# sinamalakouti/CDDMSL

Measured on AMD Instinct MI355X. Metric: images/sec (train step) VOC+Clipart RN50-C4, higher is better.
Workload: dtype bf16

## Files before the change

### cddmsl_amd/csrc/conv_fwd256.hip

```cpp
#include "gemm_common.h"
#include <type_traits>

namespace {

__device__ __forceinline__ unsigned pack4_e4m3(float a, float b, float c, float d) {
  a = __builtin_amdgcn_fmed3f(a, -448.f, 448.f); b = __builtin_amdgcn_fmed3f(b, -448.f, 448.f);
  c = __builtin_amdgcn_fmed3f(c, -448.f, 448.f); d = __builtin_amdgcn_fmed3f(d, -448.f, 448.f);
  int w = __builtin_amdgcn_cvt_pk_fp8_f32(a, b, 0, false);
  w = __builtin_amdgcn_cvt_pk_fp8_f32(c, d, w, true);
  return (unsigned)w;
}

struct fp8e4 { unsigned char v; };
template <> struct Mma<fp8e4> {
  static constexpr int ES = 2;
  __device__ static __forceinline__ void step2(f32x16& acc, const u32x4& a0, const u32x4& a1, const u32x4& b0, const u32x4& b1) {
    const i32x8 a = {(int)a0[0], (int)a0[1], (int)a0[2], (int)a0[3], (int)a1[0], (int)a1[1], (int)a1[2], (int)a1[3]};
    const i32x8 b = {(int)b0[0], (int)b0[1], (int)b0[2], (int)b0[3], (int)b1[0], (int)b1[1], (int)b1[2], (int)b1[3]};
    acc = __builtin_amdgcn_mfma_scale_f32_32x32x64_f8f6f4(a, b, acc, 0, 0, 0, 0x7f7f7f7f, 0, 0x7f7f7f7f);
  }
};
template <typename T> struct MmaQuad {
  __device__ static __forceinline__ void run(f32x16& c0, f32x16& c1, const u32x4 (*fa)[4], const u32x4* fb) {
#pragma unroll
// ... 172 lines not shown
        const u32x2 o8 = {pack4_e4m3(v[0] * q8s, v[1] * q8s, v[2] * q8s, v[3] * q8s), pack4_e4m3(v[4] * q8s, v[5] * q8s, v[6] * q8s, v[7] * q8s)};
        __builtin_amdgcn_raw_buffer_store_b64(o8, ry8, vy8, (unsigned)((a * 32 + 8 * i) * p.ldy), CDDMSL_STORE_AUX);
        asm volatile("s_nop 4" ::: "memory");
        asm volatile("" :: "v"(o8));
      }
      if (f32out) {
        const u32x4 o0 = {__builtin_bit_cast(unsigned, v[0]), __builtin_bit_cast(unsigned, v[1]), __builtin_bit_cast(unsigned, v[2]), __builtin_bit_cast(unsigned, v[3])};
        const u32x4 o1 = {__builtin_bit_cast(unsigned, v[4]), __builtin_bit_cast(unsigned, v[5]), __builtin_bit_cast(unsigned, v[6]), __builtin_bit_cast(unsigned, v[7])};
        __builtin_amdgcn_raw_buffer_store_b128(o0, ry, vy, so, CDDMSL_STORE_AUX);
        __builtin_amdgcn_raw_buffer_store_b128(o1, ry, vy, so + 16, CDDMSL_STORE_AUX);
        asm volatile("s_nop 4" ::: "memory");
        asm volatile("" :: "v"(o0), "v"(o1));
      } else {
        const u32x4 o = {pack2bf(v[0], v[1]), pack2bf(v[2], v[3]), pack2bf(v[4], v[5]), pack2bf(v[6], v[7])};
        if (p.nt_out) __builtin_amdgcn_raw_buffer_store_b128(o, ry, vy, so, CDDMSL_STORE_AUX);
        else __builtin_amdgcn_raw_buffer_store_b128(o, ry, vy, so, 0);
        asm volatile("s_nop 4" ::: "memory");
        asm volatile("" :: "v"(o));
      }
    }
    if (DEPTH == 2 && a + 2 < 4 && !rf32) fetch(a + 2, rresb[a % DEPTH], rmskb[a % DEPTH]);
  };
  put(std::integral_constant<int, 0>{});
  pass(std::integral_constant<int, 0>{});
  pass(std::integral_constant<int, 1>{});
  pass(std::integral_constant<int, 2>{});
  pass(std::integral_constant<int, 3>{});
  if (emit8 && p.amax8) {
    am8 = wave_max_u(am8);
    if (lane == 0) atomicMax(p.amax8 + (blockIdx.x & 63), am8);
  }
}

template <typename T, bool TAPS, bool RPOOL = false, int EPI = -1, bool PERSIST = false, bool SPLITK = false>
__global__ __launch_bounds__(512) void k_conv_fwd256(ConvArgs p) {
  __shared__ __attribute__((aligned(16))) u32x4 lds[2 * 2 * 2 * 128 * KCH];
  const int t_in = threadIdx.x;
  p.x += (long)blockIdx.y * p.bx; p.w += (long)blockIdx.y * p.bw; p.y += (long)blockIdx.y * p.by;
  const int ntn = p.Cout >> 8;
  const int ntiles = PERSIST ? (p.tile_limit ? p.tile_limit : ntn * ((p.M + 255) >> 8)) : 0;
  int lbid = PERSIST ? (int)((blockIdx.x & 7) * (gridDim.x >> 3) + (blockIdx.x >> 3))
           : SPLITK ? p.tile0 + (int)(blockIdx.x / (unsigned)p.ksplits) : xcd_remap(blockIdx.x, gridDim.x);
  const int kt0 = SPLITK ? (int)(blockIdx.x % (unsigned)p.ksplits) * p.kper : 0;
  if (PERSIST && lbid >= ntiles) return;
  for (;;) {
  int t = t_in;
  if (PERSIST) asm volatile("" : "+v"(t));
  const int lane = t & 63;
#ifdef CDDMSL_TILE_STAMPS
  const unsigned long long ts_entry = __builtin_amdgcn_s_memrealtime();
#endif
  const int wvu = __builtin_amdgcn_readfirstlane(t >> 6);
  const int wr = wvu >> 2, wc = wvu & 3;
  const int tile_n = lbid % ntn, tile_m = lbid / ntn;
  const int m0 = tile_m * 256, n0 = tile_n * 256;
  const int cl = (t & 7) ^ ((t >> 4) & 7);
  const int nkt = SPLITK ? min(p.kper, (p.Kc >> 3) - kt0) : (p.Kc >> 3);
  const int tpt = p.cpp >> 3;

  auto rowoff = [&](int m, int& iy0, int& ix0) {
    const unsigned tq = fdiv((unsigned)m, p.dWo), ox = m - tq * p.Wo;
    const unsigned img = fdiv(tq, p.dHo), oy = tq - img * p.Ho;
    iy0 = (int)oy * p.stride - p.pad; ix0 = (int)ox * p.stride - p.pad;
    return (((long)img * p.Hi + iy0) * p.Wi + ix0) * p.xrs * 16;
  };
  int iyb, ixb;
  const long base_a = rowoff(m0, iyb, ixb);
  const __amdgpu_buffer_rsrc_t ra_rsrc = __builtin_amdgcn_make_buffer_rsrc((void*)(p.x + base_a), 0, 0x7fffffff, 0x00020000);
  const __amdgpu_buffer_rsrc_t rb_rsrc = __builtin_amdgcn_make_buffer_rsrc((void*)(p.w + (long)n0 * p.wrs * 16), 0, 0x7fffffff, 0x00020000);
  unsigned va[2][2], vinv[2][2], vb[2][2];
  int iy0[2][2], ix0[2][2];
#pragma unroll
  for (int h = 0; h < 2; ++h)
#pragma unroll
    for (int i = 0; i < 2; ++i) {
      const int m = m0 + i * 128 + h * 64 + (t >> 3);
      const bool vm = m < p.M;
      const long ro = rowoff(vm ? m : m0, iy0[h][i], ix0[h][i]);
      va[h][i] = (unsigned)(ro - base_a) + cl * 16;
      if (!vm) { iy0[h][i] = -(1 << 20); if (!TAPS) va[h][i] |= 0x80000000u; }
      vinv[h][i] = 0;
      vb[h][i] = (unsigned)(((2 * i + (t >> 8)) * 64 + h * 32 + ((t >> 3) & 31)) * p.wrs + cl) * 16;
    }
  if (TAPS) {
    unsigned xm[2][2] = {{0, 0}, {0, 0}};
    for (int kx = 0; kx < p.KW; ++kx)
#pragma unroll
      for (int h = 0; h < 2; ++h)
#pragma unroll
        for (int i = 0; i < 2; ++i) xm[h][i] |= ((unsigned)(ix0[h][i] + kx) >= (unsigned)p.Wi ? 1u : 0u) << kx;
    const unsigned full = (1u << p.KW) - 1u;
    for (int ky = 0; ky < p.KH; ++ky)
#pragma unroll
      for (int h = 0; h < 2; ++h)
#pragma unroll
        for (int i = 0; i < 2; ++i) vinv[h][i] |= ((unsigned)(iy0[h][i] + ky) >= (unsigned)p.Hi ? full : xm[h][i]) << (ky * p.KW);
  }
  const int step_col = (p.xrs - (p.cpp - KCH)) * 16;
  const int step_row = ((p.Wi - (p.KW - 1)) * p.xrs - (p.cpp - KCH)) * 16;
  int left[2] = {tpt, tpt}, tap[2] = {0, 0}, kxs[2] = {0, 0};
  unsigned soa[2] = {0, 0}, sob[2] = {0, 0};
  if (SPLITK) {
    const int tap0 = TAPS ? kt0 / tpt : 0, within = TAPS ? kt0 - tap0 * tpt : kt0;
    const int ky0 = TAPS ? tap0 / p.KW : 0, kx0 = tap0 - ky0 * p.KW;
#pragma unroll
    for (int h = 0; h < 2; ++h) {
      left[h] = tpt - (TAPS ? within : 0); tap[h] = tap0; kxs[h] = kx0;
      soa[h] = (unsigned)((ky0 * p.Wi + kx0) * p.xrs * 16 + within * KCH * 16);
      sob[h] = (unsigned)(kt0 * KCH * 16);
    }
  }

  char* const L = (char*)lds;
  auto stageA = [&](auto H, int buf) {
    constexpr int h = decltype(H)::value;
    char* dst = L + (buf << 16) + (h << 14) + wvu * 1024;
#pragma unroll
    for (int i = 0; i < 2; ++i) {
      unsigned v = va[h][i];
      if (TAPS) v |= __builtin_amdgcn_ubfe(vinv[h][i], (unsigned)tap[h], 1u) << 31;
      blds16(ra_rsrc, v, soa[h], dst + i * 8192);
    }
    if (TAPS) {
      int step = KCH * 16;
      if (--left[h] == 0) {
        left[h] = tpt; ++tap[h];
        if (++kxs[h] == p.KW) { kxs[h] = 0; step = step_row; } else step = step_col;
      }
      soa[h] += step;
    } else soa[h] += KCH * 16;
  };
  auto stageB = [&](auto J, int buf) {
    constexpr int j = decltype(J)::value;
    char* dst = L + (buf << 16) + (1 << 15) + (j << 14) + wvu * 1024;
#pragma unroll
    for (int i = 0; i < 2; ++i) blds16(rb_rsrc, vb[j][i], sob[j], dst + i * 8192);
    sob[j] += KCH * 16;
  };
  using I0 = std::integral_constant<int, 0>;
  using I1 = std::integral_constant<int, 1>;

  f32x16 acc[4][2];
#pragma unroll
  for (int a = 0; a < 4; ++a)
#pragma unroll
    for (int b = 0; b < 2; ++b)
#pragma unroll
      for (int r = 0; r < 16; ++r) acc[a][b][r] = 0.f;

  const int r32 = lane & 31, hh = lane >> 5, sw = (r32 >> 1) & 7;
  unsigned ada[4], adb[4];
#pragma unroll
  for (int ks = 0; ks < 4; ++ks) {
    ada[ks] = (unsigned)(((wr * 64 + r32) * KCH + ((2 * ks + hh) ^ sw)) * 16);
    adb[ks] = (unsigned)(((wc * 32 + r32) * KCH + ((2 * ks + hh) ^ sw)) * 16 + (1 << 15));
  }
  u32x4 fa0[2][4], fa1[2][4], fb0[4], fb1[4];
  auto readA = [&](auto I, u32x4 (*fa)[4]) {
    constexpr int i = decltype(I)::value;
#pragma unroll
    for (int rt = 0; rt < 2; ++rt)
#pragma unroll
      for (int ks = 0; ks < 4; ++ks) fa[rt][ks] = *(const u32x4*)(L + ada[ks] + ((i << 14) + rt * 32 * KCH * 16));
  };
  auto readB = [&](auto J, u32x4* fb) {
    constexpr int j = decltype(J)::value;
#pragma unroll
    for (int ks = 0; ks < 4; ++ks) fb[ks] = *(const u32x4*)(L + adb[ks] + (j << 14));
  };
  auto flipA = [&]() {
// ... 313 lines not shown
    case 2: launch(std::integral_constant<int, 2>()); break;
    default: launch(std::integral_constant<int, 3>()); break;
  }
}

template <typename T, bool TAPS> void launch_fwd2(const ConvArgs& a, dim3 grid, hipStream_t st) {
  const int epi = epi_of(a);
  if constexpr (sizeof(T) == 2) {
    if (epi >= 0) {
      with_epi(epi, [&](auto e) { hipLaunchKernelGGL((k_conv_fwd2<T, TAPS, decltype(e)::value>), grid, dim3(256), 0, st, a); });
      return;
    }
  }
  hipLaunchKernelGGL((k_conv_fwd2<T, TAPS, -1>), grid, dim3(256), 0, st, a);
}

struct TailSplit { int rem, splits, kper; };
constexpr int TAIL_FRAC_DEFAULT = 8;
static TailSplit plan_tail_split(int tiles, int ncu, int nktot, long ws_bytes) {
  const int rem = ncu > 0 ? tiles % ncu : 0;
  long frac = env_int("CDDMSL_TAIL_FRAC", TAIL_FRAC_DEFAULT);
  if (frac <= 0) frac = 8;
  if (env_int("CDDMSL_TAIL_SPLIT", 1) == 0 || tiles <= ncu || rem <= 0 || rem * frac > ncu || nktot < 16) return {};
  long S = ncu / rem;
  if (S > nktot / 2) S = nktot / 2;
  const long maxs = env_int("CDDMSL_TAIL_MAXS", S);
  if (S > maxs) S = maxs;
  const int kper = (int)((nktot + S - 1) / S);
  S = (nktot + kper - 1) / kper;
  if (S < 2 || rem * S * 65536 * 4 > ws_bytes) return {};
  return {rem, (int)S, kper};
}

template <typename T, bool TAPS> void launch256_main(const ConvArgs& a, dim3 grid, hipStream_t st, int epi) {
  if constexpr (std::is_same<T, __bf16>::value && !TAPS) {
    const int nb = persistent_blocks();
    if (nb > 0 && grid.y == 1 && (int)grid.x > nb && (a.Kc >> 3) <= env_int("CDDMSL_PERSIST_MAXKT", 8)) {
      with_epi(epi, [&](auto e) { hipLaunchKernelGGL((k_conv_fwd256<T, false, false, decltype(e)::value, true>), dim3(nb), dim3(512), 0, st, a); });
      return;
    }
  }
  with_epi(epi, [&](auto e) { hipLaunchKernelGGL((k_conv_fwd256<T, TAPS, false, decltype(e)::value>), grid, dim3(512), 0, st, a); });
}

template <typename T, bool TAPS> void launch256(const ConvArgs& a, dim3 grid, hipStream_t st, void* ws, long ws_bytes) {
  const int epi = epi_of(a);
  if (sizeof(T) == 4 || epi < 0) { hipLaunchKernelGGL((k_conv_fwd256<T, TAPS, false, -1>), grid, dim3(512), 0, st, a); return; }
  if constexpr (sizeof(T) != 4) {
    if constexpr (std::is_same<T, __bf16>::value) {
      const int tiles = (int)grid.x;
      const TailSplit ts = grid.y == 1 ? plan_tail_split(tiles, persistent_blocks_raw(), a.Kc >> 3, ws ? ws_bytes : 0) : TailSplit{};
      if (ts.splits) {
        ConvArgs m = a, t = a;
        m.tile_limit = tiles - ts.rem;
        launch256_main<T, TAPS>(m, dim3((unsigned)(tiles - ts.rem), 1), st, epi);
        t.partial = (float*)ws; t.tile0 = tiles - ts.rem; t.ksplits = ts.splits; t.kper = ts.kper;
        hipLaunchKernelGGL((k_conv_fwd256<T, TAPS, false, -1, false, true>), dim3((unsigned)(ts.rem * ts.splits)), dim3(512), 0, st, t);
        hipLaunchKernelGGL(k_conv_split_reduce, dim3((unsigned)(ts.rem * 64)), dim3(256), 0, st, t);
        return;
      }
    }
    launch256_main<T, TAPS>(a, grid, st, epi);
  }
}

template <typename T> void launch_tile256(const ConvArgs& a, const Plan& p, hipStream_t st, void* ws, long ws_bytes) {
  const dim3 grid(p.gx, p.gy);
  const bool taps = !(a.KH == 1 && a.KW == 1 && a.pad == 0);
  if constexpr (std::is_same<T, fp8e4>::value) {
    if (taps) launch256<T, true>(a, grid, st, ws, ws_bytes);
    else launch256<T, false>(a, grid, st, ws, ws_bytes);
  } else if (p.kernel == 11) {
    if (taps) launch_fwd2<T, true>(a, grid, st);
    else launch_fwd2<T, false>(a, grid, st);
  } else {
    if (a.res_pool) hipLaunchKernelGGL((k_conv_fwd256<T, false, true>), grid, dim3(512), 0, st, a);
    else if (taps) launch256<T, true>(a, grid, st, ws, ws_bytes);
    else launch256<T, false>(a, grid, st, ws, ws_bytes);
  }
}

}

void launch_fwd_tile256(const ConvArgs& a, const Plan& p, Operand op, hipStream_t st, void* ws, long ws_bytes) {
  if (op == OP_BF16) launch_tile256<__bf16>(a, p, st, ws, ws_bytes);
  else if (op == OP_F32) launch_tile256<float>(a, p, st, ws, ws_bytes);
  else launch_tile256<fp8e4>(a, p, st, ws, ws_bytes);
}
```

### cddmsl_amd/csrc/conv_wgrad.hip

```cpp
#include "gemm_common.h"

namespace {

template <typename T> struct TrFrag;
template <> struct TrFrag<__bf16> {
  __device__ static __forceinline__ u32x4 read(const u32x4* base, int mrow0, int col0, int lane) {
    int g = lane >> 4, li = lane & 15, q = li >> 2, pp = li & 3;
    int hh = g >> 1;
    int col = col0 + 16 * (g & 1) + 4 * pp;
    const char* b = (const char*)base;
    const char* a0 = b + (long)(mrow0 + 8 * hh + q) * (WROW * 16) + col * 2;
    const char* a1 = a0 + 4 * (WROW * 16);
    i16x4 v0 = __builtin_amdgcn_ds_read_tr16_b64_v4i16((__attribute__((address_space(3))) i16x4*)a0);
    i16x4 v1 = __builtin_amdgcn_ds_read_tr16_b64_v4i16((__attribute__((address_space(3))) i16x4*)a1);
    u32x2 p0 = __builtin_bit_cast(u32x2, v0), p1 = __builtin_bit_cast(u32x2, v1);
    u32x4 r = {p0[0], p0[1], p1[0], p1[1]};
    return r;
  }
  static constexpr int MSTEP = 16;
};
template <> struct TrFrag<float> {
  __device__ static __forceinline__ u32x4 read(const u32x4* base, int mrow0, int col0, int lane) {
    int r = lane & 31, hh = lane >> 5;
    const char* b = (const char*)base;
// ... 170 lines not shown
  __shared__ __attribute__((aligned(16))) u32x4 lds[2][2][WM * 16];
  const int t = threadIdx.x, lane = t & 63, wv = t >> 6;
  p.x += (long)blockIdx.y * p.bx; p.dy += (long)blockIdx.y * p.bd;
  char* outp = (char*)p.dw + (long)blockIdx.y * p.bo;
  const int wvu = __builtin_amdgcn_readfirstlane(t >> 6);
  const int ntn = (p.Cout + COLS - 1) / COLS, ntk = (p.K + COLS - 1) / COLS;
  int bid = xcd_remap(blockIdx.x, gridDim.x);
  const int tile_k = bid % ntk; bid /= ntk;
  const int tile_n = bid % ntn; bid /= ntn;
  const int split = bid;
  const int n0 = tile_n * COLS, k0 = tile_k * COLS;
  const int mt0 = split * p.mtiles_per_split;
  const int total_mt = (p.M + WM - 1) / WM;
  const int mt1 = min(mt0 + p.mtiles_per_split, total_mt);

  const int cc = t & 15, rb = t >> 4;
  const int cl = cc ^ fsw(rb);
  const int kc = k0 * ES / 16 + cl;
  const bool vk = kc < p.Kc;
  const int pp = vk ? kc / p.cpp : 0, coff = vk ? kc - pp * p.cpp : 0;
  const int ky = pp / p.KW, kx = pp - ky * p.KW;
  const int nc = n0 * ES / 16 + cl;
  const bool vn = nc < p.ncc;
  const bool taps = !(p.KH == 1 && p.KW == 1);
  const char* zp = (const char*)g_zero_page;

  int m[4];
  const char* pd[4];
  const char* px[4];
#pragma unroll
  for (int i = 0; i < 4; ++i) {
    m[i] = mt0 * WM + rb + 16 * i;
    pd[i] = p.dy + ((long)m[i] * p.ldd) * ES + (long)nc * 16;
    px[i] = p.x + (((long)m[i] + (long)(ky - p.pad) * p.Wi + (kx - p.pad)) * p.xrs) * 16 + (long)coff * 16;
  }
  const long dstep = (long)WM * p.ldd * ES, xstep = (long)WM * p.xrs * 16;

  auto stage = [&](int buf) {
#pragma unroll
    for (int i = 0; i < 4; ++i) {
      bool vmm = m[i] < p.M;
      glds16((vmm && vn) ? pd[i] : zp, &lds[buf][0][(4 * wvu + 16 * i) * 16]);
    }
#pragma unroll
    for (int i = 0; i < 4; ++i) {
      bool ok = (m[i] < p.M) & vk;
      if (taps) {
        unsigned mm = min((unsigned)m[i], (unsigned)(p.M - 1));
        unsigned tq = fdiv(mm, p.dWo);
        unsigned ox = mm - tq * p.Wo;
        unsigned oy = tq - fdiv(tq, p.dHo) * p.Ho;
        ok = ok & ((unsigned)((int)oy - p.pad + ky) < (unsigned)p.Hi) & ((unsigned)((int)ox - p.pad + kx) < (unsigned)p.Wi);
      }
      glds16(ok ? px[i] : zp, &lds[buf][1][(4 * wvu + 16 * i) * 16]);
    }
#pragma unroll
    for (int i = 0; i < 4; ++i) { m[i] += WM; pd[i] += dstep; px[i] += xstep; }
  };

  constexpr int WT = COLS / 2;
  constexpr int NT = WT / 32;
  const int wn = wv >> 1, wk = wv & 1;
  f32x16 acc[NT][NT];
#pragma unroll
  for (int a = 0; a < NT; ++a)
#pragma unroll
    for (int b = 0; b < NT; ++b)
#pragma unroll
      for (int r = 0; r < 16; ++r) acc[a][b][r] = 0.f;

  typename TrFragS<T>::Off offa[NT], offb[NT];
#pragma unroll
  for (int i = 0; i < NT; ++i) {
    offa[i] = TrFragS<T>::prep(wn * WT + i * 32, lane);
    offb[i] = TrFragS<T>::prep(wk * WT + i * 32, lane);
  }

  if (mt0 < mt1) stage(0);
  for (int mt = mt0; mt < mt1; ++mt) {
    const int cur = (mt - mt0) & 1;
    if (mt + 1 < mt1) {
      stage(cur ^ 1);
      asm volatile("s_waitcnt vmcnt(8)" ::: "memory");
    } else {
      asm volatile("s_waitcnt vmcnt(0)" ::: "memory");
// ... 315 lines not shown
#pragma unroll
    for (int a = 0; a < NTN; ++a)
#pragma unroll
      for (int g = 0; g < 16; ++g) {
        if (a * 4 + (g >> 2) < NG) {
          const int n = a * 32 + (g & 3) + 8 * (g >> 2) + 4 * h;
          const float v = acc[a][g];
          const long o = (long)n * p.ldo + k;
          if (MODE == 0) atomicAdd((float*)outp + o, v);
          else if (MODE == 1) ((float*)outp)[o] = v;
          else Mma<__bf16>::store(outp + o * 2, v);
        }
        acc[a][g] = 0.f;
      }
  };
  {
    int it = 0;
    for (; it + 2 < nit; ++it) item(it, std::integral_constant<int, 2>{});
    if (it + 1 < nit) { item(it, std::integral_constant<int, 1>{}); ++it; }
    if (it < nit) item(it, std::integral_constant<int, 0>{});
  }
  if (MODE == 3 && p.gpos) {
    const int k = k0 + wvu * 32 + r;
#pragma unroll
    for (int a = 0; a < NTN; ++a)
#pragma unroll
      for (int g = 0; g < 16; ++g) {
        const int n = a * 32 + (g & 3) + 8 * (g >> 2) + 4 * h;
        if (a * 4 + (g >> 2) < NG && n <= P) atomicAdd(p.gpos + (long)n * p.K + k, gacc[a][g]);
      }
  }
}

__global__ __launch_bounds__(512) void k_wgrad256(WgradArgs p) {
  __shared__ __attribute__((aligned(16))) u32x4 lds[2 * 2 * 2 * 64 * 16];
  const int t = threadIdx.x, lane = t & 63;
#ifdef CDDMSL_TILE_STAMPS
  const unsigned long long ts_entry = __builtin_amdgcn_s_memrealtime();
  unsigned long long ts_loop = ts_entry;
#endif
  p.x += (long)blockIdx.y * p.bx; p.dy += (long)blockIdx.y * p.bd;
  char* outp = (char*)p.dw + (long)blockIdx.y * p.bo;
  const int wvu = __builtin_amdgcn_readfirstlane(t >> 6);
  const int wn = wvu >> 2, wk = wvu & 3;
  const int ntn = p.Cout >> 8, ntk = p.K >> 8;
  int bid = xcd_remap(blockIdx.x, gridDim.x);
  const int tile_k = bid % ntk; bid /= ntk;
  const int tile_n = bid % ntn; bid /= ntn;
  const int n0 = tile_n * 256, k0 = tile_k * 256;
  const int mt0 = bid * p.mtiles_per_split;
  const int nmt = min(p.mtiles_per_split, (p.M + WM - 1) / WM - mt0);
  const bool taps = !(p.KH == 1 && p.KW == 1);

  const int rb = t >> 4, cl = (t & 15) ^ fsw(rb);
  const int gd = (cl >> 3) * 16 + (cl & 7);
  const int gx = (cl >> 2) * 8 + (cl & 3);
  const int kc = (k0 >> 3) + gx;
  const int pp = kc / p.cpp, coff = kc - pp * p.cpp;
  const int ky = pp / p.KW, kx = pp - ky * p.KW;
  unsigned vd[2], vx[2];
#pragma unroll
  for (int i = 0; i < 2; ++i) {
    vd[i] = (unsigned)((i * 32 + rb) * p.ldd * 2 + gd * 16);
    vx[i] = (unsigned)((((i * 32 + rb) + ky * p.Wi + kx) * p.xrs + coff) * 16);
  }
  const __amdgpu_buffer_rsrc_t rd = __builtin_amdgcn_make_buffer_rsrc((void*)(p.dy + ((long)mt0 * WM * p.ldd + n0) * 2), 0, 0x80000000u, 0x00020000);
  const __amdgpu_buffer_rsrc_t rx = __builtin_amdgcn_make_buffer_rsrc((void*)(p.x + ((long)mt0 * WM - p.pad * p.Wi - p.pad) * p.xrs * 16), 0, 0x80000000u, 0x00020000);
  const unsigned dstep = (unsigned)(WM * p.ldd * 2), xstep = (unsigned)(WM * p.xrs * 16);
  const int mrow = mt0 * WM + rb;

  char* const L = (char*)lds;
  auto stageD = [&](auto H, int buf, int T) {
    constexpr int h = decltype(H)::value;
    char* dst = L + (buf << 16) + (h << 14) + wvu * 1024;
#pragma unroll
    for (int i = 0; i < 2; ++i) {
      const unsigned inv = (mrow + T * WM + i * 32 < p.M) ? 0u : 0x80000000u;
      __builtin_amdgcn_raw_ptr_buffer_load_lds(rd, (__attribute__((address_space(3))) void*)(dst + i * 8192 - h * 128), 16,
                                               (int)(vd[i] | inv), (int)(T * dstep), h * 128, 0);
    }
  };
  unsigned xinv[2];
  auto validX = [&](int T) {
#pragma unroll
    for (int i = 0; i < 2; ++i) {
      const int m = mrow + T * WM + i * 32;
      bool ok = m < p.M;
      if (taps) {
        const unsigned mm = min((unsigned)m, (unsigned)(p.M - 1));
        const unsigned tq = fdiv(mm, p.dWo);
        const unsigned ox = mm - tq * p.Wo;
        const unsigned oy = tq - fdiv(tq, p.dHo) * p.Ho;
        ok = ok & ((unsigned)((int)oy - p.pad + ky) < (unsigned)p.Hi) & ((unsigned)((int)ox - p.pad + kx) < (unsigned)p.Wi);
      }
      xinv[i] = ok ? 0u : 0x80000000u;
    }
  };
  auto stageX = [&](auto J, int buf, int T) {
    constexpr int j = decltype(J)::value;
    char* dst = L + (buf << 16) + (1 << 15) + (j << 14) + wvu * 1024;
#pragma unroll
    for (int i = 0; i < 2; ++i)
      __builtin_amdgcn_raw_ptr_buffer_load_lds(rx, (__attribute__((address_space(3))) void*)(dst + i * 8192 - j * 64), 16,
                                               (int)(vx[i] | xinv[i]), (int)(T * xstep), j * 64, 0);
  };
  using I0 = std::integral_constant<int, 0>;
  using I1 = std::integral_constant<int, 1>;

  f32x16 acc[4][2];
#pragma unroll
  for (int a = 0; a < 4; ++a)
#pragma unroll
    for (int b = 0; b < 2; ++b)
#pragma unroll
      for (int r = 0; r < 16; ++r) acc[a][b][r] = 0.f;

  const unsigned lbase = (unsigned)(size_t)(__attribute__((address_space(3))) char*)L;
  unsigned adA[2][2], adB[2];
  {
#pragma unroll
    for (int a = 0; a < 2; ++a) {
      const TrFragS<__bf16>::Off o = TrFragS<__bf16>::prep(wn * 64 + a * 32, lane);
      adA[a][0] = lbase + o.o0; adA[a][1] = lbase + o.o1;
    }
    const TrFragS<__bf16>::Off o = TrFragS<__bf16>::prep(wk * 32, lane);
    adB[0] = lbase + (1u << 15) + o.o0; adB[1] = lbase + (1u << 15) + o.o1;
  }
  u32x4 fa0[2][4], fa1[2][4], fb0[4], fb1[4];
#define CDDMSL_TR2(DST, A0, A1, IMM)                                                             \
// ... 5 lines not shown
  _Pragma("unroll") for (int a = 0; a < 2; ++a) {                                                \
    CDDMSL_TR2(FA[a][0], adA[a][0], adA[a][1], ((HALF) << 14) + 0 * 4096)                        \
    CDDMSL_TR2(FA[a][1], adA[a][0], adA[a][1], ((HALF) << 14) + 1 * 4096)                        \
    CDDMSL_TR2(FA[a][2], adA[a][0], adA[a][1], ((HALF) << 14) + 2 * 4096)                        \
    CDDMSL_TR2(FA[a][3], adA[a][0], adA[a][1], ((HALF) << 14) + 3 * 4096) }
#define CDDMSL_READ_B(HALF, FB)                                                                  \
  CDDMSL_TR2(FB[0], adB[0], adB[1], ((HALF) << 14) + 0 * 4096)                                   \
  CDDMSL_TR2(FB[1], adB[0], adB[1], ((HALF) << 14) + 1 * 4096)                                   \
  CDDMSL_TR2(FB[2], adB[0], adB[1], ((HALF) << 14) + 2 * 4096)                                   \
  CDDMSL_TR2(FB[3], adB[0], adB[1], ((HALF) << 14) + 3 * 4096)
#define CDDMSL_FLIP_A() { adA[0][0] ^= 1u << 16; adA[0][1] ^= 1u << 16; adA[1][0] ^= 1u << 16; adA[1][1] ^= 1u << 16; }
#define CDDMSL_FLIP_B() { adB[0] ^= 1u << 16; adB[1] ^= 1u << 16; }
#define CDDMSL_MMA_QUAD(I, J, FA, FB)                                               \
  _Pragma("unroll") for (int ms = 0; ms < 4; ++ms) {                                \
    Mma<__bf16>::step(acc[2 * (I)][J], FA[0][ms], FB[ms]);                          \
    Mma<__bf16>::step(acc[2 * (I) + 1][J], FA[1][ms], FB[ms]);                      \
  }
#define CDDMSL_WAIT4(F) asm volatile("s_waitcnt lgkmcnt(0)" : "+v"(F[0]), "+v"(F[1]), "+v"(F[2]), "+v"(F[3]) :: "memory");
#define CDDMSL_WAIT8(F) asm volatile("s_waitcnt lgkmcnt(0)" : "+v"(F[0][0]), "+v"(F[0][1]), "+v"(F[0][2]), "+v"(F[0][3]), \
                                     "+v"(F[1][0]), "+v"(F[1][1]), "+v"(F[1][2]), "+v"(F[1][3]) :: "memory");
#define CDDMSL_PHASE_SYNC_IN(WAIT)                                                  \
  __builtin_amdgcn_sched_barrier(0);                                                \
  __builtin_amdgcn_s_barrier();                                                     \
  WAIT                                                                              \
  __builtin_amdgcn_sched_barrier(0);                                                \
  __builtin_amdgcn_s_setprio(1);
#define CDDMSL_PHASE_SYNC_OUT(I, J)                                                 \
  asm volatile("" : "+v"(acc[2 * (I)][J]), "+v"(acc[2 * (I) + 1][J]));              \
  __builtin_amdgcn_s_setprio(0);                                                    \
  __builtin_amdgcn_sched_barrier(0);                                                \
  __builtin_amdgcn_s_barrier();                                                     \
  __builtin_amdgcn_sched_barrier(0);

  if (nmt > 0) {
    validX(0);
    stageD(I0{}, 0, 0); stageD(I1{}, 0, 0); stageX(I0{}, 0, 0); stageX(I1{}, 0, 0);
    if (nmt > 1) {
      validX(1);
      stageD(I0{}, 1, 1); stageX(I0{}, 1, 1); stageX(I1{}, 1, 1);
      asm volatile("s_waitcnt vmcnt(6)" ::: "memory");
    } else {
      asm volatile("s_waitcnt vmcnt(0)" ::: "memory");
    }
    __builtin_amdgcn_s_barrier();
    __builtin_amdgcn_sched_barrier(0);
    CDDMSL_READ_A(0, fa0)
    CDDMSL_WAIT8(fa0)
    if (wn == 1) __builtin_amdgcn_s_barrier();
    __builtin_amdgcn_sched_barrier(0);
#ifdef CDDMSL_TILE_STAMPS
    ts_loop = __builtin_amdgcn_s_memrealtime();
#endif

    for (int kt = 0; kt < nmt; ++kt) {
      const int d = kt & 1;
      const bool more1 = kt + 1 < nmt, more2 = kt + 2 < nmt;
      CDDMSL_READ_B(0, fb0)
      if (more1) stageD(I1{}, d ^ 1, kt + 1);
      CDDMSL_PHASE_SYNC_IN(CDDMSL_WAIT4(fb0))
      CDDMSL_MMA_QUAD(0, 0, fa0, fb0);
      CDDMSL_PHASE_SYNC_OUT(0, 0)
      CDDMSL_READ_B(1, fb1)
      CDDMSL_FLIP_B()
      if (more2) { stageD(I0{}, d, kt + 2); validX(kt + 2); }
      CDDMSL_PHASE_SYNC_IN(CDDMSL_WAIT4(fb1))
      CDDMSL_MMA_QUAD(0, 1, fa0, fb1);
      CDDMSL_PHASE_SYNC_OUT(0, 1)
      CDDMSL_READ_A(1, fa1)
      CDDMSL_FLIP_A()
      if (more2) {
        stageX(I0{}, d, kt + 2);
        asm volatile("s_waitcnt vmcnt(4)" ::: "memory");
      } else {
        asm volatile("s_waitcnt vmcnt(0)" ::: "memory");
      }
      CDDMSL_PHASE_SYNC_IN(CDDMSL_WAIT8(fa1))
      CDDMSL_MMA_QUAD(1, 1, fa1, fb1);
      CDDMSL_PHASE_SYNC_OUT(1, 1)
      if (more1) { CDDMSL_READ_A(0, fa0) }
      if (more2) stageX(I1{}, d, kt + 2);
      CDDMSL_PHASE_SYNC_IN(CDDMSL_WAIT8(fa0))
      CDDMSL_MMA_QUAD(1, 0, fa1, fb0);
      CDDMSL_PHASE_SYNC_OUT(1, 0)
    }
    if (wn == 0) __builtin_amdgcn_s_barrier();
  }
#undef CDDMSL_TR2
#undef CDDMSL_WAIT4
#undef CDDMSL_WAIT8
#undef CDDMSL_READ_A
#undef CDDMSL_READ_B
#undef CDDMSL_FLIP_A
#undef CDDMSL_FLIP_B
#undef CDDMSL_MMA_QUAD
#undef CDDMSL_PHASE_SYNC_IN
#undef CDDMSL_PHASE_SYNC_OUT

#ifdef CDDMSL_TILE_STAMPS
  const unsigned long long ts_epi = __builtin_amdgcn_s_memrealtime();
#endif
  const int r = lane & 31, h = lane >> 5;
  if (p.ws) {
    store_frags((f32x4*)p.ws + ((long)(bid * ntn + tile_n) * ntk + tile_k) * (8 * 32 * 64) + (wvu * 32) * 64 + lane, acc);
  } else
#pragma unroll
  for (int a = 0; a < 4; ++a)
#pragma unroll
    for (int b = 0; b < 2; ++b) {
      const int k = k0 + wk * 64 + b * 32 + r;
#pragma unroll
      for (int g = 0; g < 16; ++g) {
        const int n = n0 + wn * 128 + a * 32 + (g & 3) + 8 * (g >> 2) + 4 * h;
        const float v = acc[a][b][g] * (p.scale ? p.scale[n] : 1.f);
// ... 201 lines not shown
  }
  for (; s < splits; ++s) sum += src[s * ntiles * SLOTS];
  const int wv = q / (FR * 64), j = (q / 64) % FR, lane = q & 63, r = lane & 31, h = lane >> 5, g4 = j & 3;
  int a, b, wn, wk;
  if (WAVES == 8) { a = j >> 3; b = (j >> 2) & 1; wn = wv >> 2; wk = wv & 3; }
  else { a = j >> 3; b = (j >> 2) & 1; wn = wv >> 1; wk = wv & 1; }
  const int n = tile_n * TN + wn * (WAVES == 8 ? 128 : 64) + a * 32 + 8 * g4 + 4 * h;
  const int k = tile_k * TN + wk * 64 + b * 32 + r;
  if (k >= K) return;
#pragma unroll
  for (int e = 0; e < 4; ++e)
    if (n + e < Cout) dw[(long)(n + e) * ldo + k] += sum[e] * (scale ? scale[n + e] : 1.f);
}

static bool use_workspace(long blocks, long tile_floats, void* ws, long ws_bytes) {
  if (env_int("CDDMSL_WGRAD_WS", 1) == 0) return false;
  return ws != nullptr && blocks * tile_floats * 4 <= ws_bytes;
}

template <int WAVES, int FR>
static void launch_wgrad_split(void (*kernel)(WgradArgs), WgradArgs& a, const Plan& p, hipStream_t st, void* wsp, long ws_bytes) {
  constexpr int TN = WAVES == 8 ? 256 : 128, SLOTS = WAVES * FR * 64;
  const int ntn = (a.Cout + TN - 1) / TN, ntk = (a.K + TN - 1) / TN;
  const bool ws = p.splits > 1 && use_workspace((long)p.gx, SLOTS * 4, wsp, ws_bytes);
  if (ws) a.ws = (float*)wsp;
  hipLaunchKernelGGL(kernel, dim3(p.gx), dim3(WAVES * 64), 0, st, a);
  if (ws) hipLaunchKernelGGL((k_wgrad_reduce<WAVES, FR>), dim3((unsigned)(ntn * ntk * (SLOTS / 256))), dim3(256), 0, st, (const f32x4*)wsp, a.dw, a.scale,
                             ntn, ntk, p.splits, a.Cout, a.K, a.ldo);
}

void launch_wgrad(WgradArgs& a, const Plan& p, Operand op, hipStream_t st, void* ws, long ws_bytes) {
  switch (p.kernel) {
    case 12: launch_wgrad_split<8, 32>(k_wgrad256_f8, a, p, st, ws, ws_bytes); break;
    case 6: launch_wgrad_split<8, 32>(k_wgrad256, a, p, st, ws, ws_bytes); break;
    case 5:
      if (op == OP_BF16) launch_wgrad_split<4, 16>(k_conv_wgrad_dma<__bf16>, a, p, st, ws, ws_bytes);
      else hipLaunchKernelGGL(k_conv_wgrad_dma<float>, dim3(p.gx), dim3(256), 0, st, a);
      break;
    default:
      if (op == OP_BF16) hipLaunchKernelGGL(k_conv_wgrad<__bf16>, dim3(p.gx), dim3(256), 0, st, a);
      else hipLaunchKernelGGL(k_conv_wgrad<float>, dim3(p.gx), dim3(256), 0, st, a);
  }
}

void launch_gemm_tn(const WgradArgs& p, Operand op, const Plan& pl, int batch, int mode, hipStream_t st) {
  const dim3 grid(pl.gx, pl.gy);
  if (pl.kernel == 9) {
#define CDDMSL_TNS(NG)                                                                                              \
  case NG:                                                                                                          \
    if (mode == 0) hipLaunchKernelGGL((k_gemm_tn_small<NG, 0>), grid, dim3(256), 0, st, p, batch, pl.bpb);      \
    else if (mode == 1) hipLaunchKernelGGL((k_gemm_tn_small<NG, 1>), grid, dim3(256), 0, st, p, batch, pl.bpb); \
    else hipLaunchKernelGGL((k_gemm_tn_small<NG, 2>), grid, dim3(256), 0, st, p, batch, pl.bpb);                \
    break;
    switch (p.Cout / 8) { CDDMSL_TNS(1) CDDMSL_TNS(2) CDDMSL_TNS(3) CDDMSL_TNS(4) CDDMSL_TNS(5) CDDMSL_TNS(6) CDDMSL_TNS(7) CDDMSL_TNS(8) }
#undef CDDMSL_TNS
  } else if (pl.kernel == 7) {
    if (op == OP_BF16) hipLaunchKernelGGL(k_gemm_tn_stream<__bf16>, grid, dim3(256), 0, st, p, batch, pl.bpb);
    else hipLaunchKernelGGL(k_gemm_tn_stream<float>, grid, dim3(256), 0, st, p, batch, pl.bpb);
  } else {
    if (op == OP_BF16) hipLaunchKernelGGL(k_conv_wgrad_dma<__bf16>, grid, dim3(256), 0, st, p);
    else hipLaunchKernelGGL(k_conv_wgrad_dma<float>, grid, dim3(256), 0, st, p);
  }
}

void launch_attnpool_dx(const WgradArgs& p, unsigned gx, unsigned gy, int nbatch, int bpb, hipStream_t st) {
  hipLaunchKernelGGL((k_gemm_tn_small<7, 3, 49>), dim3(gx, gy), dim3(256), 0, st, p, nbatch, bpb);
}
// ... 1 lines not shown
```

### cddmsl_amd/csrc/elementwise.hip

```cpp
#include "common.h"
#include <stdlib.h>

namespace {

template <typename T> struct Elt;
template <> struct Elt<__bf16> {
  static constexpr int ES = 2, VEC = 8;
  __device__ static __forceinline__ void unpack(const u32x4& v, float* f) {
#pragma unroll
    for (int j = 0; j < 4; ++j) { f[2 * j] = bf2f(v[j] & 0xffff); f[2 * j + 1] = bf2f(v[j] >> 16); }
  }
  __device__ static __forceinline__ u32x4 pack(const float* f) {
    u32x4 v;
#pragma unroll
    for (int j = 0; j < 4; ++j) v[j] = pack2bf(f[2 * j], f[2 * j + 1]);
    return v;
  }
  __device__ static __forceinline__ float ld(const char* p) { return bf2f(*(const unsigned short*)p); }
  __device__ static __forceinline__ void st(char* p, float v) { *(unsigned short*)p = f2bf(v); }
};
template <> struct Elt<float> {
  static constexpr int ES = 4, VEC = 4;
  __device__ static __forceinline__ void unpack(const u32x4& v, float* f) {
    const f32x4 x = __builtin_bit_cast(f32x4, v);
// ... 110 lines not shown
    float a0[8], a1[8], a2[8], a3[8], o[8];
    Elt<T>::unpack(b[0], a0); Elt<T>::unpack(b[cch], a1);
    Elt<T>::unpack(b[(long)W * cch], a2); Elt<T>::unpack(b[(long)W * cch + cch], a3);
#pragma unroll
    for (int j = 0; j < Elt<T>::VEC; ++j) o[j] = ((a0[j] + a1[j]) + (a2[j] + a3[j])) * 0.25f;
    ((u32x4*)y)[i] = Elt<T>::pack(o);
  }
}

template <typename T>
__global__ void k_avgpool2_bwd(const char* dy, const char* mask, const char* add, char* dx, int N, int H, int W, int cch) {
  int Ho = H / 2, Wo = W / 2;
  long total = (long)N * H * W * cch;
  for (long i = (long)blockIdx.x * blockDim.x + threadIdx.x; i < total; i += (long)gridDim.x * blockDim.x) {
    int c = i % cch; long q = i / cch;
    int xx = q % W; q /= W;
    int yy = q % H; int n = q / H;
    float g[8], m[8], a[8], o[8];
    bool in = (yy >> 1) < Ho && (xx >> 1) < Wo;
    if (in) Elt<T>::unpack(((const u32x4*)dy)[(((long)n * Ho + (yy >> 1)) * Wo + (xx >> 1)) * cch + c], g);
    if (mask) Elt<T>::unpack(((const u32x4*)mask)[i], m);
    if (add) Elt<T>::unpack(((const u32x4*)add)[i], a);
#pragma unroll
    for (int j = 0; j < Elt<T>::VEC; ++j) {
      float v = in ? g[j] * 0.25f : 0.f;
      if (add) v += a[j];
      if (mask && !(m[j] > 0.f)) v = 0.f;
      o[j] = v;
    }
    ((u32x4*)dx)[i] = Elt<T>::pack(o);
  }
}

__global__ __launch_bounds__(256) void k_avgpool2_bwd_q8(const char* dy, const char* mask, const char* add, char* dx, int N, int H, int W, int cch,
                                                         char* y8, const float* q8, unsigned* amax8) {
  using T = __bf16;
  const int Ho = H / 2, Wo = W / 2;
  const long total = (long)N * H * W * cch;
  const float s = q8[0];
  unsigned mx = 0u;
  for (long i = (long)blockIdx.x * blockDim.x + threadIdx.x; i < total; i += (long)gridDim.x * blockDim.x) {
    int c = i % cch; long q = i / cch;
    int xx = q % W; q /= W;
    int yy = q % H; int n = q / H;
    float g[8], m[8], a[8], o[8];
    bool in = (yy >> 1) < Ho && (xx >> 1) < Wo;
    if (in) Elt<T>::unpack(((const u32x4*)dy)[(((long)n * Ho + (yy >> 1)) * Wo + (xx >> 1)) * cch + c], g);
    if (mask) Elt<T>::unpack(((const u32x4*)mask)[i], m);
    if (add) Elt<T>::unpack(((const u32x4*)add)[i], a);
#pragma unroll
    for (int j = 0; j < 8; ++j) {
      float v = in ? g[j] * 0.25f : 0.f;
      if (add) v += a[j];
      if (mask && !(m[j] > 0.f)) v = 0.f;
      o[j] = v;
      mx = absmax_bits(mx, v);
    }
    ((u32x4*)dx)[i] = Elt<T>::pack(o);
    const u32x2 o8 = {e4m3x4(o[0] * s, o[1] * s, o[2] * s, o[3] * s), e4m3x4(o[4] * s, o[5] * s, o[6] * s, o[7] * s)};
    ((u32x2*)y8)[i] = o8;
  }
  __shared__ unsigned sm[4];
  mx = wave_max_u(mx);
  if ((threadIdx.x & 63) == 0) sm[threadIdx.x >> 6] = mx;
  __syncthreads();
  if (threadIdx.x == 0) {
// ... 416 lines not shown
  hipStream_t st = (hipStream_t)stream;
  for (int n0 = 0; n0 < N; n0 += PRE_MAX) {
    const int c = N - n0 < PRE_MAX ? N - n0 : PRE_MAX;
    PreBatch b;
    for (int j = 0; j < PRE_MAX; ++j) { const int q = j < c ? j : 0; b.img[j] = imgs[n0 + q]; b.h[j] = hs[n0 + q]; b.w[j] = ws[n0 + q]; }
    DISPATCH(dtype, k_preprocess224_batch, <<<dim3((unsigned)((S * S + 255) / 256), (unsigned)c), dim3(256), 0, st>>>(
        b, (char*)out, n0, Hp, Wp, RH, RW, top, left, S, Cp, mean3[0], mean3[1], mean3[2], std3[0], std3[1], std3[2]));
  }
  return launch_status();
}

extern "C" int cddmsl_avgpool2_fwd(const void* x, void* y, int N, int H, int W, int C, int dtype, void* stream) {
  int es = dtype == 0 ? 2 : 4;
  if ((C * es) % 16 || H < 2 || W < 2) return CDDMSL_ERR_ARG;
  int cch = C * es / 16;
  long total = (long)N * (H / 2) * (W / 2) * cch;
  if (total == 0) return CDDMSL_OK;
  DISPATCH(dtype, k_avgpool2_fwd, <<<dim3(gsz(total)), dim3(256), 0, (hipStream_t)stream>>>((const char*)x, (char*)y, N, H, W, cch));
  return launch_status();
}

extern "C" int cddmsl_avgpool2_bwd(const void* dy, const void* mask, const void* add, void* dx, int N, int H, int W,
                                   int C, int dtype, void* stream) {
  int es = dtype == 0 ? 2 : 4;
  if ((C * es) % 16 || H < 2 || W < 2) return CDDMSL_ERR_ARG;
  int cch = C * es / 16;
  long total = (long)N * H * W * cch;
  if (total == 0) return CDDMSL_OK;
  DISPATCH(dtype, k_avgpool2_bwd, <<<dim3(gsz(total)), dim3(256), 0, (hipStream_t)stream>>>(
      (const char*)dy, (const char*)mask, (const char*)add, (char*)dx, N, H, W, cch));
  return launch_status();
}

extern "C" int cddmsl_avgpool2_bwd_q8(const void* dy, const void* mask, const void* add, void* dx, int N, int H, int W, int C, void* y8,
                                      const float* q8, float* amax8, void* stream) {
  if ((C * 2) % 16 || !y8 || !q8 || !amax8) return CDDMSL_ERR_ARG;
  const int cch = C * 2 / 16;
  const long total = (long)N * H * W * cch;
  if (total == 0) return CDDMSL_OK;
  hipLaunchKernelGGL(k_avgpool2_bwd_q8, dim3(gsz(total, 256, 8192)), dim3(256), 0, (hipStream_t)stream, (const char*)dy, (const char*)mask, (const char*)add,
                     (char*)dx, N, H, W, cch, (char*)y8, q8, (unsigned*)amax8);
  return launch_status();
}

extern "C" int cddmsl_maxpool3s2_fwd(const void* x, void* y, int N, int H, int W, int C, int dtype, void* stream) {
  int es = dtype == 0 ? 2 : 4;
  if ((C * es) % 16 || H < 1 || W < 1) return CDDMSL_ERR_ARG;
  int cch = C * es / 16, Ho = (H - 1) / 2 + 1, Wo = (W - 1) / 2 + 1;
  long total = (long)N * Ho * Wo * cch;
  if (total == 0) return CDDMSL_OK;
  DISPATCH(dtype, k_maxpool3s2, <<<dim3(gsz(total)), dim3(256), 0, (hipStream_t)stream>>>((const char*)x, (char*)y, N, H, W, Ho, Wo, cch));
  return launch_status();
}
extern "C" int cddmsl_upsample_zero2(const void* t, const void* mask, const void* add, void* dx, int N, int H, int W, int C,
                                     int dtype, void* stream) {
  int es = dtype == 0 ? 2 : 4;
  if ((C * es) % 16 || H < 1 || W < 1) return CDDMSL_ERR_ARG;
  int cch = C * es / 16, Ho = (H - 1) / 2 + 1, Wo = (W - 1) / 2 + 1;
  long total = (long)N * H * W * cch;
  if (total == 0) return CDDMSL_OK;
  DISPATCH(dtype, k_upsample_zero2, <<<dim3(gsz(total)), dim3(256), 0, (hipStream_t)stream>>>(
      (const char*)t, (const char*)mask, (const char*)add, (char*)dx, N, H, W, Ho, Wo, cch));
  return launch_status();
}
extern "C" int cddmsl_meanpool_fwd(const void* x, float* y, long K, int P, int C, int dtype, void* stream) {
  if (K < 0 || P <= 0 || C <= 0) return CDDMSL_ERR_ARG;
// ... 122 lines not shown
```

### cddmsl_amd/csrc/gemm_common.h

```cpp
#pragma once
#include "common.h"
#include <cstdlib>

namespace {

constexpr int BM = 128, BN = 128, KCH = 8;

struct FastDiv {
  unsigned mul, shr, d;
};
static inline FastDiv make_fastdiv(unsigned d) {
  FastDiv f;
  f.d = d;
  unsigned s = 0;
  while ((1ull << s) < d) ++s;
  f.shr = s;
  f.mul = (unsigned)(((1ull << 32) * ((1ull << s) - d)) / d + 1);
  return f;
}
__device__ __forceinline__ unsigned fdiv(unsigned n, const FastDiv& f) { return (__umulhi(n, f.mul) + n) >> f.shr; }

template <typename T> __device__ __forceinline__ float affine(float v, float sc, float bi) {
  return sizeof(T) <= 2 ? __builtin_fmaf(v, sc, bi) : v * sc + bi;
}

#ifndef CDDMSL_STORE_AUX
#define CDDMSL_STORE_AUX 2
#endif
#ifndef CDDMSL_LOAD_AUX
#define CDDMSL_LOAD_AUX 0
#endif

struct ConvArgs {
  const char* x;
  const char* w;
  char* y;
  const float* scale;
  const float* bias;
  const char* residual;
  const char* relu_mask;
  int Nimg, Hi, Wi, Cin, Ho, Wo, Cout, KH, KW, stride, pad;
  int ldy, ldr, ldm;
  int relu, out_f32, pool;
  int res_f32;
  int res_pool;
  int M, Kc, cpp;
  FastDiv dWo, dHo, dcpp, dKW;
  int xrs, wrs;
  long bx, bw, by;
  char* y8 = nullptr;
  const float* q8 = nullptr;
  unsigned* amax8 = nullptr;
  float* partial = nullptr;
  int tile0 = 0, ksplits = 1, kper = 0, tile_limit = 0;
  int nt_out = 1;
#ifdef CDDMSL_TILE_STAMPS
  unsigned long long* tstamps = nullptr;
#endif
};

template <typename T> struct Mma;
template <> struct Mma<__bf16> {
  static constexpr int ES = 2;
  __device__ static __forceinline__ void step(f32x16& acc, const u32x4& a, const u32x4& b) {
    acc = __builtin_amdgcn_mfma_f32_32x32x16_bf16(__builtin_bit_cast(bf16x8, a), __builtin_bit_cast(bf16x8, b), acc, 0, 0, 0);
  }
  __device__ static __forceinline__ float load(const char* p) { return bf2f(*(const unsigned short*)p); }
  __device__ static __forceinline__ void store(char* p, float v) { *(unsigned short*)p = f2bf(v); }
};
template <> struct Mma<float> {
  static constexpr int ES = 4;
  __device__ static __forceinline__ void step(f32x16& acc, const u32x4& a, const u32x4& b) {
    const f32x4 fa = __builtin_bit_cast(f32x4, a), fb = __builtin_bit_cast(f32x4, b);
    acc = __builtin_amdgcn_mfma_f32_32x32x2f32(fa[0], fb[0], acc, 0, 0, 0);
    acc = __builtin_amdgcn_mfma_f32_32x32x2f32(fa[1], fb[1], acc, 0, 0, 0);
    acc = __builtin_amdgcn_mfma_f32_32x32x2f32(fa[2], fb[2], acc, 0, 0, 0);
    acc = __builtin_amdgcn_mfma_f32_32x32x2f32(fa[3], fb[3], acc, 0, 0, 0);
  }
  __device__ static __forceinline__ float load(const char* p) { return *(const float*)p; }
  __device__ static __forceinline__ void store(char* p, float v) { *(float*)p = v; }
};
typedef __attribute__((ext_vector_type(8))) int i32x8;

__device__ __forceinline__ int xcd_remap(int bid, int nblk) {
  const int q = nblk >> 3, rem = nblk & 7, x = bid & 7, j = bid >> 3;
  return (x < rem ? x * (q + 1) : rem * (q + 1) + (x - rem) * q) + j;
}

// ... 8 lines not shown
  u32x4 r;
#pragma unroll
  for (int j = 0; j < 4; ++j) {
    float lo = (bf2f(a[j] & 0xffff) + bf2f(b[j] & 0xffff)) + (bf2f(c[j] & 0xffff) + bf2f(d[j] & 0xffff));
    float hi = (bf2f(a[j] >> 16) + bf2f(b[j] >> 16)) + (bf2f(c[j] >> 16) + bf2f(d[j] >> 16));
    r[j] = pack2bf(lo * 0.25f, hi * 0.25f);
  }
  return r;
}

__device__ __attribute__((aligned(16))) unsigned int g_zero_page[4] = {0u, 0u, 0u, 0u};

__device__ __forceinline__ void glds16(const void* g, void* l) {
  __builtin_amdgcn_global_load_lds((const __attribute__((address_space(1))) void*)g,
                                   (__attribute__((address_space(3))) void*)l, 16, 0, 0);
}

struct WgradArgs {
  const char* x;
  const char* dy;
  float* dw;
  const float* scale;
  int Nimg, Hi, Wi, Cin, Ho, Wo, Cout, KH, KW, stride, pad, ldd, pool;
  int M, Kc, cpp, K, ncc;
  int mtiles_per_split;
  FastDiv dWo, dHo;
  int xrs;
  int ldo;
  int direct;
  long bx, bd, bo;
  const float* g0 = nullptr;
  const unsigned long long* mbits = nullptr;
  float* gpos = nullptr;
  float* ws = nullptr;
#ifdef CDDMSL_TILE_STAMPS
  unsigned long long* tstamps = nullptr;
#endif
};

constexpr int WM = 64;
constexpr int WROW = 16 + 4;

__device__ __forceinline__ int fsw(int row) { return ((row & 3) << 2) | ((row >> 2) & 3); }

__device__ __forceinline__ void store_frags(f32x4* dst, const f32x16 (&acc)[4][2]) {
#pragma unroll
  for (int a = 0; a < 4; ++a)
#pragma unroll
    for (int b = 0; b < 2; ++b)
#pragma unroll
      for (int g4 = 0; g4 < 4; ++g4) {
        const f32x4 v = {acc[a][b][4 * g4], acc[a][b][4 * g4 + 1], acc[a][b][4 * g4 + 2], acc[a][b][4 * g4 + 3]};
        dst[((a * 2 + b) * 4 + g4) * 64] = v;
      }
}

static long env_int(const char* name, long dflt, bool* set = nullptr) {
  const char* e = getenv(name);
  if (set) *set = e != nullptr;
  return e ? atol(e) : dflt;
}

enum Operand { OP_BF16 = 0, OP_F32 = 1, OP_FP8 = 2 };
static int elem_size(Operand op) { return op == OP_BF16 ? 2 : op == OP_F32 ? 4 : 1; }

struct Plan {
// ... 28 lines not shown
```

### cddmsl_amd/csrc/gemm_conv.hip

```cpp
#include "gemm_common.h"

namespace {

template <typename T>
__device__ __forceinline__ void weight_prep_body(const float* w, const float* scale, char* wf, char* wd, int Cout, int KH, int KW, int Cin,
                                                 long first, long stride) {
  __shared__ float tile[32][33];
  const int taps = KH * KW, nit = (Cin + 31) / 32, nct = (Cout + 31) / 32;
  const long ntiles = (long)nct * taps * nit;
  const int tx = threadIdx.x & 31, ty = threadIdx.x >> 5;
  constexpr int ES = Mma<T>::ES;
  for (long tl = first; tl < ntiles; tl += stride) {
    const int it = (int)(tl % nit); const long q = tl / nit;
    const int tap = (int)(q % taps), ct = (int)(q / taps);
    const int ky = tap / KW, kx = tap % KW;
    __syncthreads();
#pragma unroll
    for (int r = 0; r < 4; ++r) {
      const int co = ct * 32 + ty + 8 * r, ci = it * 32 + tx;
      float v = 0.f;
      if (co < Cout && ci < Cin) {
        const long i = ((long)co * taps + tap) * Cin + ci;
        v = w[i];
        if (wf) Mma<T>::store(wf + i * ES, v);
// ... 161 lines not shown
extern "C" int cddmsl_conv_fwd(const void* x, const void* w, void* y, const float* scale, const float* bias,
                               const void* residual, const void* relu_mask, int Nimg, int Hi, int Wi, int Cin,
                               int Cout, int KH, int KW, int stride, int pad, int pool, int ldy, int ldr, int ldm,
                               int relu, int out_f32, int dtype, void* stream) {
  if (dtype != 0 && dtype != 1) return CDDMSL_ERR_ARG;
  return conv_fwd_any((Operand)dtype, x, w, y, scale, bias, residual, relu_mask, Nimg, Hi, Wi, Cin, Cout, KH, KW, stride, pad, pool, ldy, ldr, ldm,
                      relu, out_f32, nullptr, nullptr, nullptr, stream);
}

extern "C" int cddmsl_conv_fwd_q8(const void* x, const void* w, void* y, const float* scale, const float* bias,
                                  const void* residual, const void* relu_mask, int Nimg, int Hi, int Wi, int Cin,
                                  int Cout, int KH, int KW, int stride, int pad, int relu, void* y8, const float* q8, float* amax8,
                                  void* stream) {
  if (!y8) return CDDMSL_ERR_ARG;
  return conv_fwd_any(OP_BF16, x, w, y, scale, bias, residual, relu_mask, Nimg, Hi, Wi, Cin, Cout, KH, KW, stride, pad, 0, Cout, Cout, Cout,
                      relu, 0, y8, q8, amax8, stream);
}

extern "C" int cddmsl_conv_fwd_fp8(const void* x, const void* w, void* y, const float* scale, const float* bias,
                                   const void* residual, const void* relu_mask, int Nimg, int Hi, int Wi, int Cin, int Cout, int KH,
                                   int KW, int pad, int relu, int out_f32, void* y8, const float* q8, float* amax8, void* stream) {
  if (Cin % 128 != 0 || (out_f32 & ~1)) return CDDMSL_ERR_ARG;
  return conv_fwd_any(OP_FP8, x, w, y, scale, bias, residual, relu_mask, Nimg, Hi, Wi, Cin, Cout, KH, KW, 1, pad, 0, Cout, Cout, Cout,
                      relu, out_f32, y8, q8, amax8, stream);
}

static bool wgrad256_ok(const WgradArgs& a, int batch) {
  const long mode = env_int("CDDMSL_GEMM256", 1);
  if (mode == 0) return false;
  if ((a.Cout & 255) || (a.K & 255) || (a.cpp & 7) || (a.ldd & 7)) return false;
  if (mode == 2) return true;
  return (long)(a.Cout / 256) * (a.K / 256) * batch * ((a.M + WM - 1) / WM) >= env_int("CDDMSL_WGRAD256_MIN", 4000);
}
static bool wgrad256_span_ok(int mtiles_per_split, int Wi, long row_bytes) {
  return ((long)mtiles_per_split * WM + WM + 2L * Wi + 2) * row_bytes + (1L << 20) < (1L << 31);
}

static int even_split(int total_mt, long* splits) {
  const int mps = (int)((total_mt + *splits - 1) / *splits);
  *splits = (total_mt + mps - 1) / mps;
  return mps;
}

static long split_512_rounds(long tiles, int total_mt, bool taps) {
  bool forced;
  const long target = env_int("CDDMSL_WGRAD_BLOCKS", taps ? 1024 : 512, &forced);
  const long maxs = (total_mt + 7) / 8;
  long splits = 1;
  const long r0 = (target + 511) / 512;
  double best = -1.0;
  for (long r = r0; r <= r0 + 1; ++r) {
    long c = (512 * r) / tiles;
    if (c < 1) c = 1;
    if (c > maxs) c = maxs;
    long real = c;
    even_split(total_mt, &real);
    const long blocks = tiles * real, rounds = (blocks + 511) / 512;
    const double eff = (double)blocks / (512.0 * rounds);
    if (eff > best + 0.03) { best = eff; splits = c; }
    if (c == maxs) break;
  }
  if (forced) { splits = (target + tiles - 1) / tiles; if (splits > maxs) splits = maxs; }
  return splits < 1 ? 1 : splits;
}

static long split_256_rounds(long tiles, int total_mt) {
  const long maxs = (total_mt + 15) / 16;
  long sp = 1;
  double best = -1.0;
  for (int r = 1; r <= 6; ++r) {
    long c = (256L * r) / tiles;
    if (c < 1) continue;
    if (c > maxs) c = maxs;
    const long blocks = tiles * c, rounds = (blocks + 255) / 256;
    const double eff = (double)blocks / (256.0 * rounds);
    if (eff > best + 0.02) { best = eff; sp = c; }
    if (c == maxs) break;
  }
  return sp;
}

static Plan plan_wgrad(const WgradArgs& a, Operand op, int batch) {
  const int es = elem_size(op), total_mt = (a.M + WM - 1) / WM;
  const long tiles256 = (long)(a.Cout / 256) * (a.K / 256);
  const long row_bytes = (long)a.ldd * es > a.xrs * 16L ? (long)a.ldd * es : a.xrs * 16L;
  if (op == OP_FP8) {
    long sp = split_256_rounds(tiles256, total_mt);
    const int mps = even_split(total_mt, &sp);
    if (!wgrad256_span_ok(mps, a.Wi, row_bytes)) return {};
    return {12, (unsigned)(tiles256 * sp), 1, (int)sp, mps};
  }
  const int cols = 256 / es;
  const long tiles = (long)((a.Cout + cols - 1) / cols) * ((a.K + cols - 1) / cols);
  long splits = split_512_rounds(tiles, total_mt, !(a.KH == 1 && a.KW == 1));
  const int mps = even_split(total_mt, &splits);
  if (tiles * splits > 0x7fffffffL) return {};
  const bool same = !a.pool && a.stride == 1 && a.Ho == a.Hi && a.Wo == a.Wi;
  if (same && op == OP_BF16 && wgrad256_ok(a, batch)) {
    bool forced;
    const long want = env_int("CDDMSL_WGRAD256_BLOCKS", 0, &forced);
    const long maxs = (total_mt + 15) / 16;
    long sp = forced ? (want + tiles256 - 1) / tiles256 : split_256_rounds(tiles256, total_mt);
    if (sp > maxs) sp = maxs;
    if (sp < 1) sp = 1;
    const int mps256 = even_split(total_mt, &sp);
    if (wgrad256_span_ok(mps256, a.Wi, row_bytes)) return {6, (unsigned)(tiles256 * sp), 1, (int)sp, mps256};
  }
  return {same ? 5 : 4, (unsigned)(tiles * splits), 1, (int)splits, mps};
}

extern "C" int cddmsl_set_workspace(void* ptr, long bytes) {
  if (bytes < 0 || (ptr == nullptr && bytes != 0) || ((size_t)ptr & 15)) return CDDMSL_ERR_ARG;
  g_ws = ptr; g_ws_bytes = bytes;
  return CDDMSL_OK;
}

static int run_wgrad(WgradArgs& a, Operand op, const Plan& p, void* stream) {
  if (p.kernel == 0) return CDDMSL_ERR_ARG;
  g_last_kernel = p.kernel;
  if (g_plan_only) return CDDMSL_OK;
  a.mtiles_per_split = p.mtiles_per_split;
  launch_wgrad(a, p, op, (hipStream_t)stream, g_ws, g_ws_bytes);
  return launch_status();
}

static int fill_wgrad(WgradArgs& a, Operand op, const void* x, const void* dy, float* dw, const float* scale, int Nimg, int Hi,
                      int Wi, int Cin, int Cout, int KH, int KW, int stride, int pad, int pool, int ldd) {
  const int es = elem_size(op);
  if (Nimg < 0 || Hi <= 0 || Wi <= 0 || Cin <= 0 || Cout <= 0 || KH <= 0 || KW <= 0 || stride <= 0) return CDDMSL_ERR_ARG;
  if ((Cin * es) % 16 != 0 || (Cout * es) % 16 != 0 || (ldd * es) % 16 != 0) return CDDMSL_ERR_ARG;
  if (pool && (KH != 1 || KW != 1 || pad != 0 || stride != 1)) return CDDMSL_ERR_ARG;
  a.x = (const char*)x; a.dy = (const char*)dy; a.dw = dw; a.scale = scale;
  a.Nimg = Nimg; a.Hi = Hi; a.Wi = Wi; a.Cin = Cin; a.Cout = Cout; a.KH = KH; a.KW = KW; a.stride = stride; a.pad = pad;
  a.ldd = ldd; a.pool = pool;
  if (pool) { a.Ho = Hi / 2; a.Wo = Wi / 2; }
  else { a.Ho = (Hi + 2 * pad - KH) / stride + 1; a.Wo = (Wi + 2 * pad - KW) / stride + 1; }
  if (a.Ho <= 0 || a.Wo <= 0) return CDDMSL_ERR_ARG;
  long M = (long)Nimg * a.Ho * a.Wo;
  if (M > 0x7fffff00L) return CDDMSL_ERR_ARG;
  a.M = (int)M; a.cpp = Cin * es / 16; a.Kc = KH * KW * a.cpp; a.K = KH * KW * Cin; a.ncc = Cout * es / 16;
  a.mtiles_per_split = 0;
  a.dWo = make_fastdiv((unsigned)a.Wo); a.dHo = make_fastdiv((unsigned)a.Ho);
  a.xrs = a.cpp; a.ldo = a.K; a.direct = 0; a.bx = a.bd = a.bo = 0;
#ifdef CDDMSL_TILE_STAMPS
  a.tstamps = g_tile_stamps;
#endif
  return CDDMSL_OK;
}

extern "C" int cddmsl_conv_wgrad(const void* x, const void* dy, float* dw, const float* scale, int Nimg, int Hi,
                                 int Wi, int Cin, int Cout, int KH, int KW, int stride, int pad, int pool, int ldd,
                                 int dtype, void* stream) {
  if (dtype != 0 && dtype != 1) return CDDMSL_ERR_ARG;
  WgradArgs a;
  const int st = fill_wgrad(a, (Operand)dtype, x, dy, dw, scale, Nimg, Hi, Wi, Cin, Cout, KH, KW, stride, pad, pool, ldd);
  if (st != CDDMSL_OK || a.M == 0) return st;
  return run_wgrad(a, (Operand)dtype, plan_wgrad(a, (Operand)dtype, 1), stream);
}

extern "C" int cddmsl_conv_wgrad_fp8_ok(int Cin, int Cout, int KH, int KW, int pad, int ldd) {
  return (Cin % 256 == 0 && Cout % 256 == 0 && KH == KW && (KH & 1) && 2 * pad == KH - 1 && ldd % 16 == 0) ? 1 : 0;
}
extern "C" int cddmsl_conv_wgrad_fp8(const void* x8, const void* dy8, float* dw, const float* scale, int Nimg, int Hi, int Wi, int Cin,
                                     int Cout, int KH, int KW, int pad, int ldd, void* stream) {
  if (!cddmsl_conv_wgrad_fp8_ok(Cin, Cout, KH, KW, pad, ldd) || ldd < Cout) return CDDMSL_ERR_ARG;
  WgradArgs a;
  const int st = fill_wgrad(a, OP_FP8, x8, dy8, dw, scale, Nimg, Hi, Wi, Cin, Cout, KH, KW, 1, pad, 0, ldd);
  if (st != CDDMSL_OK || a.M == 0) return st;
  return run_wgrad(a, OP_FP8, plan_wgrad(a, OP_FP8, 1), stream);
}

extern "C" int cddmsl_gemm_nt_batched(const void* a, const void* w, void* c, const float* bias, int M, int N, int K, int lda,
                                      int ldb, int ldc, int batch, long sa, long sw, long sc, int out_f32, int dtype, void* stream) {
  int es = dtype == 0 ? 2 : 4;
  if (dtype != 0 && dtype != 1) return CDDMSL_ERR_ARG;
  if (M < 0 || N <= 0 || K <= 0 || batch < 0 || batch > 65535) return CDDMSL_ERR_ARG;
  if ((K * es) % 16 || (lda * es) % 16 || (ldb * es) % 16 || (sa * es) % 16 || (sw * es) % 16) return CDDMSL_ERR_ARG;
  if (M == 0 || batch == 0) return CDDMSL_OK;
  const Operand op = (Operand)dtype;
  ConvArgs p;
  const int st = fill_conv(p, op, a, w, c, nullptr, bias, nullptr, nullptr, 1, 1, M, K, N, 1, 1, 1, 0, 0, ldc, 0, 0, 0, out_f32 ? 1 : 0,
                           nullptr, nullptr, nullptr);
  if (st != CDDMSL_OK) return st;
  p.xrs = lda * es / 16; p.wrs = ldb * es / 16;
  p.bx = sa * es; p.bw = sw * es; p.by = sc * (out_f32 ? 4 : es);
  p.nt_out = 1;
  return run_fwd(p, op, plan_fwd(p, op, batch), stream);
}

static unsigned tn_small_grid(long kt, long batch, int* bpb) {
  long b = (kt * batch + 4095) / 4096;
  if (b < 8) b = 8;
// ... 89 lines not shown
```

### cddmsl_amd/csrc/roi_align.hip

```cpp
#include "common.h"

namespace {

template <typename T> struct Vec;
template <> struct Vec<__bf16> {
  static constexpr int ES = 2, VEC = 8;
  __device__ static __forceinline__ void unpack(const u32x4& v, float* f) {
#pragma unroll
    for (int j = 0; j < 4; ++j) { f[2 * j] = bf2f(v[j] & 0xffff); f[2 * j + 1] = bf2f(v[j] >> 16); }
  }
  __device__ static __forceinline__ u32x4 pack(const float* f) {
    u32x4 v;
#pragma unroll
    for (int j = 0; j < 4; ++j) v[j] = pack2bf(f[2 * j], f[2 * j + 1]);
    return v;
  }
};
template <> struct Vec<float> {
  static constexpr int ES = 4, VEC = 4;
  __device__ static __forceinline__ void unpack(const u32x4& v, float* f) {
    const f32x4 x = __builtin_bit_cast(f32x4, v);
    f[0] = x[0]; f[1] = x[1]; f[2] = x[2]; f[3] = x[3];
  }
  __device__ static __forceinline__ u32x4 pack(const float* f) {
// ... 150 lines not shown
    if (RP == 2) {
      float a0[8], a1[8], a2[8], a3[8], o[8];
      Vec<T>::unpack(outp[0][0], a0); Vec<T>::unpack(outp[0][RP - 1], a1);
      Vec<T>::unpack(outp[RP - 1][0], a2); Vec<T>::unpack(outp[RP - 1][RP - 1], a3);
#pragma unroll
      for (int q = 0; q < VEC; ++q) o[q] = ((a0[q] + a1[q]) + (a2[q] + a3[q])) * 0.25f;
      if (esc && !y) {
#pragma unroll
        for (int q = 0; q < VEC; ++q) {
          const float sq = esc[c * VEC + q], bq = ebi[c * VEC + q];
          o[q] = sizeof(T) == 2 ? __builtin_fmaf(o[q], sq, bq) : o[q] * sq + bq;
        }
      }
      ((u32x4*)yp)[(((long)k * (ph / 2) + i0 / 2) * (pw / 2) + j0 / 2) * cch + c] = Vec<T>::pack(o);
    }
  }
  }
  if (sizeof(T) == 2 && y8 && amax8) {
    __shared__ unsigned sm8[4];
    am8 = wave_max_u(am8);
    if ((threadIdx.x & 63) == 0) sm8[threadIdx.x >> 6] = am8;
    __syncthreads();
    if (threadIdx.x == 0) {
      unsigned m = sm8[0];
      for (int wv = 1; wv < (int)(blockDim.x >> 6); ++wv) m = sm8[wv] > m ? sm8[wv] : m;
      atomicMax(amax8 + (blockIdx.x & 63), m);
    }
  }
}

constexpr int ROW_MAXY = 32;
template <int RP>
__global__ __launch_bounds__(256) void k_roi_align_fwd_rows(const char* x, const float* rois, char* y, int N, int H, int W, int cch, int ph, int pw,
                                                            float scale, int sampling_ratio, int aligned, const float* esc, const float* ebi, int relu) {
  const int nrb = ph / RP;
  const int i0 = (blockIdx.x % nrb) * RP, k = blockIdx.x / nrb;
  const RoiGeom g = roi_geom(rois + 5 * (long)k, scale, ph, pw, sampling_ratio, aligned);
  __shared__ int s_xl[ROI_MAXS], s_py[ROW_MAXY], s_n[2];
  __shared__ float s_xwl[ROI_MAXS], s_xwh[ROI_MAXS], s_wy[ROW_MAXY];
  __shared__ int s_ylo[ROW_MAXY], s_yhi[ROW_MAXY];
  __shared__ float s_ywl[ROW_MAXY], s_ywh[ROW_MAXY];
  const int ny = RP * g.gh, nx = pw * g.gw;
  const int opw = pw / RP;
  const int c = blockIdx.y * blockDim.x + threadIdx.x;
  const bool inb = g.b >= 0 && g.b < N;
  float sq[8], bq[8];
#pragma unroll
  for (int q = 0; q < 8; ++q) { sq[q] = 1.f; bq[q] = 0.f; }
  if (esc) {
    const int cl = min(c, cch - 1);
#pragma unroll
    for (int q = 0; q < 8; ++q) { sq[q] = esc[cl * 8 + q]; bq[q] = ebi[cl * 8 + q]; }
  }
  if (nx > ROI_MAXS || 2 * ny > ROW_MAXY || g.bw < 0.f) {
    if (c >= cch) return;
    const u32x4* xb = (const u32x4*)x + (long)(inb ? g.b : 0) * H * W * cch + c;
    const float inv = 1.0f / ((float)max(g.gh * g.gw, 1) * (float)(RP * RP));
    for (int jo = 0; jo < opw; ++jo) {
      float acc[8] = {0, 0, 0, 0, 0, 0, 0, 0};
      for (int rr = 0; rr < RP && inb; ++rr)
        for (int cc = 0; cc < RP; ++cc)
          for (int iy = 0; iy < g.gh; ++iy) {
            int yl, yh; float wyl, wyh;
            const float yy = g.y0 + (float)(i0 + rr) * g.bh + ((float)iy + 0.5f) * g.bh / (float)g.gh;
            if (!axis_tap(yy, H, yl, yh, wyl, wyh)) continue;
            for (int ix = 0; ix < g.gw; ++ix) {
              int xl, xh; float wxl, wxh;
              const float xx = g.x0 + (float)(jo * RP + cc) * g.bw + ((float)ix + 0.5f) * g.bw / (float)g.gw;
              if (!axis_tap(xx, W, xl, xh, wxl, wxh)) continue;
              float v1[8], v2[8], v3[8], v4[8];
              Vec<__bf16>::unpack(xb[((long)yl * W + xl) * cch], v1); Vec<__bf16>::unpack(xb[((long)yl * W + xh) * cch], v2);
              Vec<__bf16>::unpack(xb[((long)yh * W + xl) * cch], v3); Vec<__bf16>::unpack(xb[((long)yh * W + xh) * cch], v4);
#pragma unroll
              for (int q = 0; q < 8; ++q) acc[q] += wyl * (wxl * v1[q] + wxh * v2[q]) + wyh * (wxl * v3[q] + wxh * v4[q]);
            }
          }
      float o[8];
#pragma unroll
      for (int q = 0; q < 8; ++q) {
        o[q] = acc[q] * inv;
        if (esc) { o[q] = __builtin_fmaf(o[q], sq[q], bq[q]); if (relu) o[q] = fmaxf(o[q], 0.f); }
      }
      ((u32x4*)y)[(((long)k * nrb + i0 / RP) * opw + jo) * cch + c] = Vec<__bf16>::pack(o);
    }
    return;
  }
  for (int s = threadIdx.x; s < ny + nx; s += blockDim.x) {
    int lo = -1, hi = -1; float wl = 0.f, wh = 0.f;
    if (s < ny) {
      const int rr = s / g.gh, iy = s - rr * g.gh;
      const float yy = g.y0 + (float)(i0 + rr) * g.bh + ((float)iy + 0.5f) * g.bh / (float)g.gh;
      if (!axis_tap(yy, H, lo, hi, wl, wh)) lo = -1;
      s_ylo[s] = lo; s_yhi[s] = hi; s_ywl[s] = wl; s_ywh[s] = wh;
    } else {
      const int sx = s - ny, j = sx / g.gw, ix = sx - j * g.gw;
      const float xx = g.x0 + (float)j * g.bw + ((float)ix + 0.5f) * g.bw / (float)g.gw;
      if (!axis_tap(xx, W, lo, hi, wl, wh)) lo = -1;
      s_xl[sx] = lo; s_xwl[sx] = wl; s_xwh[sx] = wh;
    }
  }
  __syncthreads();
  if (threadIdx.x == 0) {
    int n = 0;
    for (int s = 0; s < ny; ++s) {
      if (s_ylo[s] < 0) continue;
      const int r2[2] = {s_ylo[s], s_yhi[s]};
      const float w2[2] = {s_ywl[s], s_ywh[s]};
      for (int e = 0; e < 2; ++e) {
        int f = -1;
        for (int q = 0; q < n; ++q) if (s_py[q] == r2[e]) f = q;
        if (f < 0) { f = n++; s_py[f] = r2[e]; s_wy[f] = 0.f; }
        s_wy[f] += w2[e];
      }
    }
    int first = -1;
    for (int s = 0; s < nx && first < 0; ++s) if (s_xl[s] >= 0) first = s_xl[s];
// ... 32 lines not shown
  for (int q = 0; q < 8; ++q) { R0[q] = R1[q] = acc[q] = 0.f; }
  int cur = first;
  const bool any = inb && nrow > 0 && first >= 0;
  constexpr int PF = 4;
  const bool ahead = nrow <= PF;
  int pyr[PF]; float wyr[PF];
#pragma unroll
  for (int e = 0; e < PF; ++e) {
    pyr[e] = __builtin_amdgcn_readfirstlane(s_py[e < nrow ? e : 0]);
    wyr[e] = e < nrow ? __builtin_bit_cast(float, __builtin_amdgcn_readfirstlane(__builtin_bit_cast(int, s_wy[e]))) : 0.f;
  }
  u32x4 raw[PF];
  auto issue = [&](int px) {
#pragma unroll
    for (int e = 0; e < PF; ++e) if (e < nrow) raw[e] = xb[((long)pyr[e] * W + px) * cch];
  };
  auto finish = [&](float* R) {
#pragma unroll
    for (int q = 0; q < 8; ++q) R[q] = 0.f;
#pragma unroll
    for (int e = 0; e < PF; ++e) if (e < nrow) {
      float v[8];
      Vec<__bf16>::unpack(raw[e], v);
#pragma unroll
      for (int q = 0; q < 8; ++q) R[q] = __builtin_fmaf(wyr[e], v[q], R[q]);
    }
  };
  __builtin_amdgcn_s_waitcnt(0x0F70);
  if (any) {
    rload(cur, R0); rload(min(cur + 1, W - 1), R1);
    if (ahead) issue(min(cur + 2, W - 1));
  }
  const int spo = RP * g.gw;
  u32x4* yo = (u32x4*)y + ((long)k * nrb + i0 / RP) * opw * cch + c;
  if (nx == 0) {
    float o[8];
#pragma unroll
    for (int q = 0; q < 8; ++q) { o[q] = 0.f; if (esc) { o[q] = bq[q]; if (relu) o[q] = fmaxf(o[q], 0.f); } }
    for (int jo = 0; jo < opw; ++jo) yo[(long)jo * cch] = Vec<__bf16>::pack(o);
    return;
  }
  int left = spo, j = 0;
#pragma unroll
  for (int q = 0; q < ROI_MAXS / 64; ++q) {
  const int lim = min(64, nx - q * 64);
  for (int l = 0; l < lim; ++l) {
    const int xl = __builtin_amdgcn_readlane(xlr[q], l);
    if (any && xl >= 0) {
      while (cur < xl) {
        ++cur;
#pragma unroll
        for (int q = 0; q < 8; ++q) R0[q] = R1[q];
        if (ahead) { finish(R1); issue(min(cur + 2, W - 1)); }
        else rload(min(cur + 1, W - 1), R1);
      }
      const float wl = __builtin_bit_cast(float, __builtin_amdgcn_readlane(xwlr[q], l));
      const float wh = __builtin_bit_cast(float, __builtin_amdgcn_readlane(xwhr[q], l));
#pragma unroll
      for (int q = 0; q < 8; ++q) acc[q] = __builtin_fmaf(wl, R0[q], __builtin_fmaf(wh, R1[q], acc[q]));
    }
    if (--left == 0) {
      float o[8];
#pragma unroll
      for (int q = 0; q < 8; ++q) { o[q] = acc[q] * inv; acc[q] = 0.f; }
      if (esc) {
#pragma unroll
        for (int q = 0; q < 8; ++q) o[q] = __builtin_fmaf(o[q], sq[q], bq[q]);
        if (relu) {
#pragma unroll
          for (int q = 0; q < 8; ++q) o[q] = fmaxf(o[q], 0.f);
        }
      }
      __builtin_nontemporal_store(Vec<__bf16>::pack(o), &yo[(long)j * cch]);
      ++j; left = spo;
    }
  }
  }
}

__global__ void k_roi_tables(const float* rois, float* ay, float* ax, int* fp, int K, int H, int W, int ph, int pw,
                             float scale, int sampling_ratio, int aligned, int fold) {
  int k = blockIdx.x;
  RoiGeom g = roi_geom(rois + 5 * (long)k, scale, ph * fold, pw * fold, sampling_ratio, aligned);
  float* ayk = ay + (long)k * H * ph;
  float* axk = ax + (long)k * W * pw;
  for (int i = threadIdx.x; i < H * ph; i += blockDim.x) ayk[i] = 0.f;
  for (int i = threadIdx.x; i < W * pw; i += blockDim.x) axk[i] = 0.f;
  __shared__ int lim[4];
  if (threadIdx.x == 0) { lim[0] = H; lim[1] = -1; lim[2] = W; lim[3] = -1; }
  __syncthreads();
  const float fw = 1.0f / (float)fold;
  if (threadIdx.x < ph) {
    int lo_min = H, hi_max = -1;
    for (int i = threadIdx.x * fold; i < (threadIdx.x + 1) * fold; ++i)
    for (int iy = 0; iy < g.gh; ++iy) {
      float yy = g.y0 + (float)i * g.bh + ((float)iy + 0.5f) * g.bh / (float)g.gh;
      int yl, yh; float wl, wh;
      if (!axis_tap(yy, H, yl, yh, wl, wh)) continue;
      ayk[yl * ph + threadIdx.x] += fw * (wl / (float)g.gh);
      ayk[yh * ph + threadIdx.x] += fw * (wh / (float)g.gh);
      lo_min = min(lo_min, yl); hi_max = max(hi_max, yh);
    }
    atomicMin(&lim[0], lo_min); atomicMax(&lim[1], hi_max);
  } else if (threadIdx.x >= 64 && threadIdx.x < 64 + pw) {
    const int jc = threadIdx.x - 64;
    int lo_min = W, hi_max = -1;
    for (int j = jc * fold; j < (jc + 1) * fold; ++j)
    for (int ix = 0; ix < g.gw; ++ix) {
      float xx = g.x0 + (float)j * g.bw + ((float)ix + 0.5f) * g.bw / (float)g.gw;
      int xl, xh; float wl, wh;
      if (!axis_tap(xx, W, xl, xh, wl, wh)) continue;
      axk[xl * pw + jc] += fw * (wl / (float)g.gw);
      axk[xh * pw + jc] += fw * (wh / (float)g.gw);
      lo_min = min(lo_min, xl); hi_max = max(hi_max, xh);
    }
    atomicMin(&lim[2], lo_min); atomicMax(&lim[3], hi_max);
  }
  __syncthreads();
  if (threadIdx.x == 0) {
    bool ok = g.b >= 0;
    fp[4 * k] = ok ? lim[0] : 1; fp[4 * k + 1] = ok ? lim[1] : 0; fp[4 * k + 2] = lim[2]; fp[4 * k + 3] = lim[3];
  }
}

constexpr int MAXP = 16;
template <typename T, int NC, int TS>
__global__ __launch_bounds__(256) void k_roi_align_bwd(const char* dy, const float* ay, const float* ax, const int* fp, const int* roi_start,
                                char* dx, int H, int W, int cch, int ph, int pw) {
  const int tiles_x = (W + TS - 1) / TS, tiles_y = (H + TS - 1) / TS;
  const long tile = blockIdx.x;
  const int tx = tile % tiles_x, ty = (tile / tiles_x) % tiles_y, n = tile / ((long)tiles_x * tiles_y);
  const int py0 = TS * ty, px0 = TS * tx;
  const int k0 = roi_start[n], k1 = roi_start[n + 1];
  constexpr int VEC = Vec<T>::VEC;
  float acc[NC][TS * TS][8];
#pragma unroll
  for (int u = 0; u < NC; ++u)
#pragma unroll
    for (int q4 = 0; q4 < TS * TS; ++q4)
#pragma unroll
      for (int q = 0; q < 8; ++q) acc[u][q4][q] = 0.f;
  const int lane_ = threadIdx.x & 63;
  for (int kb = k0; kb < k1; kb += 64) {
    bool hit = false;
    if (kb + lane_ < k1) {
      const int* f = fp + 4 * (kb + lane_);
      hit = !(py0 + TS - 1 < f[0] || py0 > f[1] || px0 + TS - 1 < f[2] || px0 > f[3]);
    }
    unsigned long long hits = __ballot(hit);
  while (hits) {
    const int k = kb + __builtin_ctzll(hits);
    hits &= hits - 1;
    const float* ayr = ay + ((long)k * H + py0) * ph;
    const float* axr = ax + ((long)k * W + px0) * pw;
    const int lane = threadIdx.x & 63;
    float wyv[TS], wxv[TS];
    bool nzy = false, nzx = false;
#pragma unroll
    for (int a = 0; a < TS; ++a) {
      wyv[a] = (lane < ph && py0 + a < H) ? ayr[a * ph + lane] : 0.f;
      wxv[a] = (lane < pw && px0 + a < W) ? axr[a * pw + lane] : 0.f;
      nzy |= wyv[a] != 0.f; nzx |= wxv[a] != 0.f;
    }
    unsigned long long ym = __ballot(nzy);
    const unsigned long long xm0 = __ballot(nzx);
    if (xm0 == 0ull) continue;
    while (ym) {
      const int i = __builtin_ctzll(ym);
      ym &= ym - 1;
      float wyi[TS];
#pragma unroll
      for (int a = 0; a < TS; ++a) wyi[a] = __builtin_bit_cast(float, __builtin_amdgcn_readlane(__builtin_bit_cast(int, wyv[a]), i));
      unsigned long long xm = xm0;
      while (xm) {
        const int j = __builtin_ctzll(xm);
        xm &= xm - 1;
        float wxj[TS];
#pragma unroll
        for (int a = 0; a < TS; ++a) wxj[a] = __builtin_bit_cast(float, __builtin_amdgcn_readlane(__builtin_bit_cast(int, wxv[a]), j));
        const u32x4* src = (const u32x4*)dy + (((long)k * ph + i) * pw + j) * cch;
        float v[NC][8];
#pragma unroll
        for (int u = 0; u < NC; ++u) {
          const int c = threadIdx.x + u * blockDim.x;
          if (c < cch) Vec<T>::unpack(src[c], v[u]);
        }
#pragma unroll
        for (int a = 0; a < TS; ++a)
#pragma unroll
          for (int b = 0; b < TS; ++b) {
            const float w = wyi[a] * wxj[b];
            if (w == 0.f) continue;
#pragma unroll
            for (int u = 0; u < NC; ++u)
#pragma unroll
              for (int q = 0; q < VEC; ++q) acc[u][a * TS + b][q] += w * v[u][q];
          }
      }
    }
  }
  }
#pragma unroll
  for (int u = 0; u < NC; ++u) {
    const int c = threadIdx.x + u * blockDim.x;
    if (c < cch) {
#pragma unroll
      for (int a = 0; a < TS; ++a)
#pragma unroll
        for (int b = 0; b < TS; ++b)
          if (py0 + a < H && px0 + b < W) ((u32x4*)dx)[(((long)n * H + py0 + a) * W + px0 + b) * cch + c] = Vec<T>::pack(acc[u][a * TS + b]);
    }
  }
}

}

static int roi_align_forward_impl(const void* x, const float* rois, void* y, void* y_pooled, int* dbg_grid, const float* esc,
                                  const float* ebi, int relu, int N, int C, int H, int W, int K, int ph, int pw, float spatial_scale,
                                  int sampling_ratio, int aligned, int dtype, void* stream, void* y8 = nullptr, const float* q8 = nullptr,
                                  float* amax8 = nullptr) {
  int es = dtype == 0 ? 2 : 4;
  if ((dtype != 0 && dtype != 1) || (C * es) % 16 || H <= 0 || W <= 0 || ph <= 0 || pw <= 0 || K < 0 || N < 0)
    return CDDMSL_ERR_ARG;
  if ((esc == nullptr) != (ebi == nullptr)) return CDDMSL_ERR_ARG;
  if (!y && y_pooled && relu) return CDDMSL_ERR_ARG;
  if (K == 0) return CDDMSL_OK;
  if (!y && !y_pooled) return CDDMSL_ERR_ARG;
  if (y8 && (dtype != 0 || !y)) return CDDMSL_ERR_ARG;
  int cch = C * es / 16;
  if (y_pooled && ((ph & 1) || (pw & 1))) return CDDMSL_ERR_ARG;
  long grid = (long)K * (y_pooled ? ph / 2 : ph);
  if (grid > 0x7fffffffL) return CDDMSL_ERR_ARG;
  int threads = cch >= 256 ? 256 : ((cch + 63) / 64) * 64;
  hipStream_t st = (hipStream_t)stream;
  const char* rows_env = getenv("CDDMSL_ROI_ROWS");
  const bool rows_off = rows_env && rows_env[0] == '0';
  if (dtype == 0 && !y8 && !dbg_grid && ((y != nullptr) != (y_pooled != nullptr)) && cch <= 256 && !rows_off) {
    const int rthreads = 64;
    const unsigned gy = (unsigned)((cch + rthreads - 1) / rthreads);
    if (y) k_roi_align_fwd_rows<1><<<dim3((unsigned)((long)K * ph), gy), dim3(rthreads), 0, st>>>((const char*)x, rois, (char*)y, N, H, W, cch, ph, pw, spatial_scale, sampling_ratio, aligned, esc, ebi, relu);
    else k_roi_align_fwd_rows<2><<<dim3((unsigned)((long)K * (ph / 2)), gy), dim3(rthreads), 0, st>>>((const char*)x, rois, (char*)y_pooled, N, H, W, cch, ph, pw, spatial_scale, sampling_ratio, aligned, esc, ebi, relu);
    return launch_status();
  }
#define CDDMSL_RAF(TT, RPP) k_roi_align_fwd<TT, RPP><<<dim3((unsigned)grid), dim3(threads), 0, st>>>((const char*)x, rois, (char*)y, (char*)y_pooled, dbg_grid, N, H, W, cch, ph, pw, spatial_scale, sampling_ratio, aligned, esc, ebi, relu, (char*)y8, q8, (unsigned*)amax8)
  if (dtype == 0) { if (y_pooled) CDDMSL_RAF(__bf16, 2); else CDDMSL_RAF(__bf16, 1); }
  else { if (y_pooled) CDDMSL_RAF(float, 2); else CDDMSL_RAF(float, 1); }
#undef CDDMSL_RAF
  return launch_status();
}

extern "C" int cddmsl_roi_align_forward(const void* x, const float* rois, void* y, void* y_pooled, int* dbg_grid, int N, int C,
                                        int H, int W, int K, int ph, int pw, float spatial_scale, int sampling_ratio,
                                        int aligned, int dtype, void* stream) {
  if (!y && K > 0) return CDDMSL_ERR_ARG;
  return roi_align_forward_impl(x, rois, y, y_pooled, dbg_grid, nullptr, nullptr, 0, N, C, H, W, K, ph, pw, spatial_scale,
                                sampling_ratio, aligned, dtype, stream);
}

extern "C" int cddmsl_roi_align_forward_affine(const void* x, const float* rois, void* y, void* y_pooled, const float* scale,
                                               const float* bias, int relu, int N, int C, int H, int W, int K, int ph, int pw,
                                               float spatial_scale, int sampling_ratio, int aligned, int dtype, void* y8,
                                               const float* q8, float* amax8, void* stream) {
  return roi_align_forward_impl(x, rois, y, y_pooled, nullptr, scale, bias, relu, N, C, H, W, K, ph, pw, spatial_scale,
                                sampling_ratio, aligned, dtype, stream, y8, q8, amax8);
}

static int roi_align_backward_impl(const void* dy, const float* rois, const int* roi_start, void* dx, float* ws_ay,
                                   float* ws_ax, int* ws_fp, int N, int C, int H, int W, int K, int ph, int pw,
                                   float spatial_scale, int sampling_ratio, int aligned, int dtype, int fold, void* stream) {
  int es = dtype == 0 ? 2 : 4;
  if ((dtype != 0 && dtype != 1) || (C * es) % 16 || H <= 0 || W <= 0 || ph <= 0 || pw <= 0 || K < 0 || N < 0)
    return CDDMSL_ERR_ARG;
  if (ph > MAXP || pw > MAXP || ph > 64 || pw > 64) return CDDMSL_ERR_ARG;
  int cch = C * es / 16;
  if (cch > 1024) return CDDMSL_ERR_ARG;
  hipStream_t st = (hipStream_t)stream;
  if (N == 0) return CDDMSL_OK;
  if (K > 0) k_roi_tables<<<dim3((unsigned)K), dim3(128), 0, st>>>(rois, ws_ay, ws_ax, ws_fp, K, H, W, ph, pw, spatial_scale, sampling_ratio, aligned, fold);
  int threads = cch >= 256 ? 256 : ((cch + 63) / 64) * 64;
  const int ncpt = (cch + threads - 1) / threads;
  const int ts = 2;
  long grid = (long)N * ((H + ts - 1) / ts) * ((W + ts - 1) / ts);
  if (grid > 0x7fffffffL) return CDDMSL_ERR_ARG;
#define CDDMSL_RAB(TT, NCC, TSS) k_roi_align_bwd<TT, NCC, TSS><<<dim3((unsigned)grid), dim3(threads), 0, st>>>((const char*)dy, ws_ay, ws_ax, ws_fp, roi_start, (char*)dx, H, W, cch, ph, pw)
  if (dtype == 0) { if (ncpt <= 1) CDDMSL_RAB(__bf16, 1, 2); else if (ncpt == 2) CDDMSL_RAB(__bf16, 2, 2); else CDDMSL_RAB(__bf16, 4, 2); }
  else { if (ncpt <= 1) CDDMSL_RAB(float, 1, 2); else if (ncpt == 2) CDDMSL_RAB(float, 2, 2); else CDDMSL_RAB(float, 4, 2); }
#undef CDDMSL_RAB
  return launch_status();
}

extern "C" int cddmsl_roi_align_backward(const void* dy, const float* rois, const int* roi_start, void* dx, float* ws_ay,
                                         float* ws_ax, int* ws_fp, int N, int C, int H, int W, int K, int ph, int pw,
                                         float spatial_scale, int sampling_ratio, int aligned, int dtype, void* stream) {
  return roi_align_backward_impl(dy, rois, roi_start, dx, ws_ay, ws_ax, ws_fp, N, C, H, W, K, ph, pw, spatial_scale,
                                 sampling_ratio, aligned, dtype, 1, stream);
}

extern "C" int cddmsl_roi_align_backward_pooled(const void* dy, const float* rois, const int* roi_start, void* dx, float* ws_ay,
                                                float* ws_ax, int* ws_fp, int N, int C, int H, int W, int K, int ph, int pw,
                                                float spatial_scale, int sampling_ratio, int aligned, int dtype, void* stream) {
  return roi_align_backward_impl(dy, rois, roi_start, dx, ws_ay, ws_ax, ws_fp, N, C, H, W, K, ph, pw, spatial_scale,
                                 sampling_ratio, aligned, dtype, 2, stream);
}

namespace {
template <typename T>
__global__ void k_nchw_to_nhwc(const T* x, T* y, long N, int C, long HW, int Cp) {
  const long i = (long)blockIdx.x * blockDim.x + threadIdx.x;
  if (i >= N * HW * Cp) return;
  const int c = (int)(i % Cp);
  const long p = (i / Cp) % HW, n = i / ((long)Cp * HW);
  y[i] = c < C ? x[(n * C + c) * HW + p] : (T)0.f;
}
template <typename T>
__global__ void k_nhwc_to_nchw(const T* x, T* y, long K, int C, long HW, int Cp, const int* perm) {
  const long i = (long)blockIdx.x * blockDim.x + threadIdx.x;
  if (i >= K * C * HW) return;
  const long p = i % HW, k = i / ((long)C * HW);
  const int c = (int)((i / HW) % C);
  const long ks = perm ? perm[k] : k;
  y[i] = x[(ks * HW + p) * Cp + c];
}
template <typename T>
__global__ void k_nchw_rows_to_ranked_nhwc(const T* x, T* y, long K, int C, long HW, int Cp, const int* rank) {
  const long i = (long)blockIdx.x * blockDim.x + threadIdx.x;
  if (i >= K * HW * Cp) return;
  const int c = (int)(i % Cp);
  const long p = (i / Cp) % HW, k = i / ((long)Cp * HW);
// ... 78 lines not shown
```

### cddmsl_amd/hip.py

```python
import ctypes
import os
from ctypes import c_float, c_int, c_long, c_void_p

import torch

from ._lib import check, lib, ptr, require_cuda, stream_ptr

DT = {torch.bfloat16: 0, torch.float32: 1}

_sigs_done = False


def _L():
    global _sigs_done
    L = lib()
    if not _sigs_done:
        vp, ci, cf = c_void_p, c_int, c_float
        L.cddmsl_last_kernel.argtypes = []
        L.cddmsl_plan_only.argtypes = [ci]
        L.cddmsl_conv_fwd.argtypes = [vp] * 7 + [ci] * 16 + [vp]
        L.cddmsl_bottleneck64_ok.argtypes = [ci] * 4
        L.cddmsl_bottleneck64_fwd.argtypes = [vp] * 17 + [ci] * 4 + [vp]
        L.cddmsl_conv_wgrad.argtypes = [vp] * 4 + [ci] * 12 + [vp]
        L.cddmsl_set_workspace.argtypes = [vp, c_long]
# ... 42 lines not shown
        L.cddmsl_l2norm_bwd.argtypes = [vp, vp, vp, vp, c_long, ci, vp]
        L.cddmsl_cosine_logits_fwd.argtypes = [vp] * 4 + [c_long, ci, ci, cf, cf, vp]
        L.cddmsl_cosine_logits_bwd.argtypes = [vp] * 5 + [c_long, ci, ci, cf, ci, vp]
        L.cddmsl_layernorm_fwd.argtypes = [vp] * 6 + [c_long, ci, cf, ci, vp]
        L.cddmsl_layernorm_bwd.argtypes = [vp] * 6 + [c_long, ci, ci, ci, vp]
        L.cddmsl_focal_ce_fwd.argtypes = [vp] * 4 + [c_long, ci, cf, ci, cf, vp]
        L.cddmsl_focal_ce_bwd.argtypes = [vp] * 5 + [c_long, ci, cf, ci, cf, vp]
        L.cddmsl_attn_small_fwd.argtypes = [vp] * 4 + [ci] * 8 + [cf, ci, vp]
        L.cddmsl_attn_small_bwd.argtypes = [vp] * 7 + [ci] * 8 + [cf, ci, vp]
        L.cddmsl_attn_tokens_fwd_mask.argtypes = [vp] * 4 + [ci] * 5 + [vp]
        L.cddmsl_attnpool_dx.argtypes = [vp] * 6 + [ci] * 6 + [vp]
        L.cddmsl_rpn_losses.argtypes = [vp, vp, vp, ci, vp, ci, vp, vp, vp, vp, c_long, cf, cf, cf, cf, cf, vp, vp, vp, vp, vp]
        L.cddmsl_box_l1.argtypes = [vp, ci, vp, ci, vp, vp, vp, cf, cf, cf, cf, cf, vp, vp, vp, vp]
        L.cddmsl_attn_last_fwd.argtypes = [vp] * 4 + [ci] * 8 + [cf, ci, vp]
        L.cddmsl_attn_last_bwd.argtypes = [vp] * 6 + [ci] * 8 + [cf, ci, vp]
        L.cddmsl_contrastive_fwd.argtypes = [vp] * 4 + [ci, ci, vp]
        L.cddmsl_contrastive_bwd.argtypes = [vp] * 5 + [ci, ci, vp]
        L.cddmsl_instance_boxes.argtypes = [vp] + [ci] * 4 + [vp, ci, vp, vp, vp, vp]
        L.cddmsl_text_embed.argtypes = [vp] * 4 + [c_long, ci, ci, ci, ci, vp]
        L.cddmsl_attn_causal_fwd.argtypes = [vp, vp] + [ci] * 6 + [cf, ci, vp]
        L.cddmsl_quick_gelu.argtypes = [vp, c_long, ci, vp]
        L.cddmsl_text_pool.argtypes = [vp] * 5 + [c_long, ci, ci, ci, cf, ci, vp]
        L.cddmsl_skinny_gemm_workspace.argtypes = [ci] * 3
        L.cddmsl_skinny_gemm.argtypes = [vp] * 6 + [c_long] + [ci] * 4 + [vp]
        L.cddmsl_lm_head_workspace.argtypes = [ci, ci]
        L.cddmsl_lm_head_argmax.argtypes = [vp, vp, vp, ci, vp, vp, c_long, ci, ci, ci, vp]
        L.cddmsl_decode_attn.argtypes = [vp] * 4 + [ci] * 6 + [cf, ci, vp]
        L.cddmsl_pos_embed.argtypes = [vp, ci] + [vp] * 4 + [c_long] + [ci] * 6 + [vp]
        L.cddmsl_gelu_new.argtypes = [vp, c_long, ci, vp]
        L.cddmsl_lm_head_topk_workspace.argtypes = [ci, ci]
        L.cddmsl_lm_head_topk.argtypes = [vp] * 7 + [c_long] + [ci] * 4 + [vp]
        L.cddmsl_beam_step.argtypes = [vp] * 15 + [ci] * 5 + [vp]
        L.cddmsl_decode_attn_beam.argtypes = [vp] * 7 + [ci] * 9 + [cf, ci, vp]
        _sigs_done = True
    return L


class _Profiler:

    def __init__(self):
        self.on = False
        self.only = None
        self.events = []
        self.shapes = []

    def enable(self, only=None):
        self.on, self.only, self.events, self.shapes = True, (set(only) if only else None), [], []

    def begin(self, name=None, plan=None):
        if not self.on:
            return None
        if self.only is not None:
            if name is None and plan is not None:
                L = _L()
                L.cddmsl_plan_only(1)
                try:
                    plan()
                finally:
                    L.cddmsl_plan_only(0)
                name = _CONV_KERNEL.get(L.cddmsl_last_kernel())
            if name not in self.only:
                return None
        e = torch.cuda.Event(enable_timing=True)
        e.record()
        return e

# ... 96 lines not shown
    if residual_pooled:
        assert residual is not None and not res_f32 and residual.dtype == x.dtype and residual.is_contiguous()
        assert tuple(residual.shape) == (N, Ho // 2, Wo // 2, Cout) and pooled_residual_ok(residual), residual.shape
    for v in (residual, relu_mask):
        assert v is None or (v is residual and residual_pooled) or (
            (v.dtype == x.dtype or (v is residual and res_f32)) and v.is_contiguous() and v.numel() == y.numel())
    y8 = None
    if emit8 is not None:
        assert x.dtype == torch.bfloat16 and not out_f32 and not pool and not residual_pooled and not res_f32
        y8 = torch.empty(y.shape, device=x.device, dtype=torch.uint8)

    def launch():
        if y8 is not None:
            return _L().cddmsl_conv_fwd_q8(ptr(x), ptr(w), ptr(y), ptr(scale), ptr(bias), ptr(residual), ptr(relu_mask),
                                           N, H, W, Cin, Cout, KH, KW, stride, pad, int(relu), ptr(y8), ptr(emit8[0]), ptr(emit8[1]), stream_ptr())
        return _L().cddmsl_conv_fwd(ptr(x), ptr(w), ptr(y), ptr(scale), ptr(bias), ptr(residual), ptr(relu_mask),
                                    N, H, W, Cin, Cout, KH, KW, stride, pad, int(pool), Cout, Cout, Cout,
                                    int(relu), int(out_f32) | (2 if res_f32 else 0) | (4 if residual_pooled else 0), _dt(x), stream_ptr())
    e0 = PROFILE.begin(plan=launch) if PROFILE.on else None
    st = launch()
    check(st, "cddmsl_conv_fwd")
    PROFILE.end(e0, _CONV_KERNEL.get(_L().cddmsl_last_kernel(), "conv_fwd") if e0 is not None else "conv_fwd",
                2.0 * N * Ho * Wo * Cout * KH * KW * Cin,
                (N * Ho * Wo, Cout, KH * KW * Cin, KH, int(pool), stride),
                nbytes=float(_conv_input_pixels(N, H, W, Ho, Wo, KH, KW, stride, bool(pool)) * Cin * x.element_size()
                             + w.numel() * w.element_size() + y.numel() * y.element_size()
                             + (residual.numel() * residual.element_size() if residual is not None else 0)
                             + (relu_mask.numel() * relu_mask.element_size() if relu_mask is not None else 0)))
    if y8 is not None:
        y._fp8 = (y8, emit8[0].data_ptr())
    return y


def bottleneck64_ok(o1, w2, w3, wd=None, w1n=None):
    if not (o1.is_cuda and o1.dtype == torch.bfloat16 and o1.dim() == 4 and o1.is_contiguous() and o1.shape[3] == 64):
        return False
    want = ((w2, (64, 3, 3, 64)), (w3, (256, 1, 1, 64)), (wd, (256, 1, 1, 64)), (w1n, (64, 1, 1, 256)))
    if any(w is not None and (tuple(w.shape) != s or w.dtype != torch.bfloat16 or not w.is_contiguous()) for w, s in want):
        return False
    N, H, W, _ = o1.shape
    return N > 0 and bool(_L().cddmsl_bottleneck64_ok(N, H, W, 0))


def bottleneck64_fwd(o1, w2, bn2, w3, bn3, residual=None, x0=None, wd=None, bnd=None, w1n=None, bn1n=None):
    require_cuda(o1, w2, w3, residual, x0, wd, w1n)
    assert bottleneck64_ok(o1, w2, w3, wd, w1n) and (residual is None) != (wd is None)
    N, H, W, _ = o1.shape
    for t, c in ((residual, 256), (x0 if wd is not None else None, 64)):
        assert t is None or (t.dtype == torch.bfloat16 and t.is_contiguous() and tuple(t.shape) == (N, H, W, c))
    for bn, c in ((bn2, 64), (bn3, 256), (bnd, 256), (bn1n, 64)):
        assert bn is None or all(v.dtype == torch.float32 and v.numel() == c and v.is_contiguous() and v.is_cuda for v in bn)
    assert (wd is None) == (bnd is None) and (w1n is None) == (bn1n is None) and (wd is None or x0 is not None)
    out = torch.empty((N, H, W, 256), device=o1.device, dtype=o1.dtype)
    o1n = torch.empty((N, H, W, 64), device=o1.device, dtype=o1.dtype) if w1n is not None else None
    sd, bd = bnd if bnd is not None else (None, None)
    s1n, b1n = bn1n if bn1n is not None else (None, None)
    e0 = PROFILE.begin(name="k_bottleneck64") if PROFILE.on else None
    check(_L().cddmsl_bottleneck64_fwd(ptr(o1), ptr(w2), ptr(bn2[0]), ptr(bn2[1]), ptr(w3), ptr(bn3[0]), ptr(bn3[1]), ptr(residual),
                                       ptr(x0 if wd is not None else None), ptr(wd), ptr(sd), ptr(bd), ptr(w1n), ptr(s1n), ptr(b1n),
                                       ptr(out), ptr(o1n), N, H, W, 0, stream_ptr()), "cddmsl_bottleneck64_fwd")
    M = N * H * W
    kn = 576 * 64 + 64 * 256 + (64 * 256 if wd is not None else 0) + (256 * 64 if w1n is not None else 0)
    PROFILE.end(e0, "k_bottleneck64", 2.0 * M * kn, (M, 256, 576, 3, int(wd is not None), int(w1n is not None)),
                nbytes=float(2 * M * (64 + (64 if wd is not None else 256) + 256 + (64 if w1n is not None else 0)) + 2 * kn))
    return out, o1n

# ... 184 lines not shown
    check(_L().cddmsl_preprocess_batch(ptrs, hs, ws, len(images_u8), ptr(out), Hp, Wp, Cp, m, s, int(div255), DT[dtype], stream_ptr()),
          "cddmsl_preprocess_batch")
    return out


@_timed("preprocess224")
def preprocess224(images_u8, Hp, Wp, mean, std, dtype, size=224, Cp=None):
    require_cuda(*images_u8)
    Cp = Cp or (8 if dtype == torch.bfloat16 else 4)
    if Wp <= Hp:
        RW, RH = size, int(size * Hp / Wp)
    else:
        RH, RW = size, int(size * Wp / Hp)
    top, left = int(round((RH - size) / 2.0)), int(round((RW - size) / 2.0))
    out = torch.empty((len(images_u8), size, size, Cp), device=images_u8[0].device, dtype=dtype)
    m, s = _f3(mean), _f3(std)
    for im in images_u8:
        assert im.dtype == torch.uint8 and im.dim() == 3 and im.is_contiguous()
    ptrs, hs, ws = _image_table(images_u8)
    check(_L().cddmsl_preprocess224_batch(ptrs, hs, ws, len(images_u8), ptr(out), Hp, Wp, RH, RW, top, left, size, Cp,
                                           m, s, DT[dtype], stream_ptr()), "cddmsl_preprocess224_batch")
    return out


@_timed("avgpool2_fwd")
def avgpool2_fwd(x):
    require_cuda(x)
    N, H, W, C = x.shape
    y = torch.empty((N, H // 2, W // 2, C), device=x.device, dtype=x.dtype)
    check(_L().cddmsl_avgpool2_fwd(ptr(x), ptr(y), N, H, W, C, _dt(x), stream_ptr()), "cddmsl_avgpool2_fwd")
    return y


@_timed("avgpool2_bwd")
def avgpool2_bwd(dy, in_shape, mask=None, add=None, emit8=None):
    require_cuda(dy, mask, add)
    N, H, W, C = in_shape
    assert dy.is_contiguous() and tuple(dy.shape) == (N, H // 2, W // 2, C)
    dx = torch.empty(in_shape, device=dy.device, dtype=dy.dtype)
    if emit8 is not None and dy.dtype == torch.bfloat16:
        y8 = torch.empty(in_shape, device=dy.device, dtype=torch.uint8)
        check(_L().cddmsl_avgpool2_bwd_q8(ptr(dy), ptr(mask), ptr(add), ptr(dx), N, H, W, C, ptr(y8), ptr(emit8[0]), ptr(emit8[1]), stream_ptr()),
              "cddmsl_avgpool2_bwd_q8")
        dx._fp8 = (y8, emit8[0].data_ptr())
        return dx
    check(_L().cddmsl_avgpool2_bwd(ptr(dy), ptr(mask), ptr(add), ptr(dx), N, H, W, C, _dt(dy), stream_ptr()), "cddmsl_avgpool2_bwd")
    return dx


@_timed("attn_tokens_fwd")
def attn_tokens_fwd(x, pos, tp=None):
    require_cuda(x, pos)
    K, P, C = x.shape
    tp = tp or P + 1
    assert pos.dtype == torch.float32 and tuple(pos.shape) == (P + 1, C) and x.is_contiguous() and pos.is_contiguous()
    tok = torch.empty((K, tp, C), device=x.device, dtype=x.dtype)
    check(_L().cddmsl_attn_tokens_fwd(ptr(x), ptr(pos), ptr(tok), K, P, tp, C, _dt(x), stream_ptr()), "cddmsl_attn_tokens_fwd")
    return tok


@_timed("attn_tokens_fwd")
def attn_tokens_fwd_mask(x, pos, tp=None):
    require_cuda(x, pos)
    K, P, C = x.shape
    tp = tp or P + 1
    assert pos.dtype == torch.float32 and tuple(pos.shape) == (P + 1, C) and x.is_contiguous() and pos.is_contiguous() and P <= 64
# ... 170 lines not shown
    N, H, W, C = x.shape
    K = rois.shape[0]
    y = torch.empty((K + extra_rows, ph, pw, C), device=x.device, dtype=x.dtype)
    yp = torch.empty((K + extra_rows, ph // 2, pw // 2, C), device=x.device, dtype=x.dtype) if with_pooled else None
    check(_L().cddmsl_roi_align_forward(ptr(x), ptr(rois), ptr(y), ptr(yp), ptr(dbg_grid), N, C, H, W, K, ph, pw, spatial_scale,
                                         sampling_ratio, int(aligned), _dt(x), stream_ptr()), "cddmsl_roi_align_forward")
    return (y, yp) if with_pooled else y


@_timed("roi_align_forward")
def roi_align_forward_affine(x, rois, ph, pw, spatial_scale, sampling_ratio, aligned, scale=None, bias=None, relu=False,
                             pooled_only=False, extra_rows=0, emit8=None):
    require_cuda(x, rois)
    assert rois.dim() == 2 and rois.size(1) == 5 and rois.dtype == torch.float32 and rois.is_contiguous()
    assert (scale is None) == (bias is None)
    N, H, W, C = x.shape
    K = rois.shape[0]
    if pooled_only:
        y, yp = None, torch.empty((K + extra_rows, ph // 2, pw // 2, C), device=x.device, dtype=x.dtype)
    else:
        y, yp = torch.empty((K + extra_rows, ph, pw, C), device=x.device, dtype=x.dtype), None
    assert scale is None or (scale.dtype == torch.float32 and scale.numel() == C and bias.numel() == C and scale.is_contiguous() and bias.is_contiguous())
    y8 = None
    if emit8 is not None:
        assert not pooled_only and x.dtype == torch.bfloat16
        y8 = torch.empty(y.shape, device=x.device, dtype=torch.uint8)
    check(_L().cddmsl_roi_align_forward_affine(ptr(x), ptr(rois), ptr(y), ptr(yp), ptr(scale), ptr(bias), int(relu), N, C, H, W, K,
                                                ph, pw, spatial_scale, sampling_ratio, int(aligned), _dt(x), ptr(y8),
                                                ptr(emit8[0]) if emit8 else c_void_p(0), ptr(emit8[1]) if emit8 else c_void_p(0), stream_ptr()),
          "cddmsl_roi_align_forward_affine")
    if y8 is not None:
        y._fp8 = (y8, emit8[0].data_ptr())
    return yp if pooled_only else y


@_timed("roi_align_backward")
def roi_align_backward(dy, rois, roi_start, in_shape, spatial_scale, sampling_ratio, aligned, pooled=False):
    require_cuda(dy, rois, roi_start)
    N, H, W, C = in_shape
    K, ph, pw, _ = dy.shape
    assert roi_start.dtype == torch.int32 and roi_start.numel() == N + 1 and dy.is_contiguous()
    dx = torch.empty(in_shape, device=dy.device, dtype=dy.dtype)
    ay = workspace("roi_ay", max(K, 1) * H * ph * 4, dy.device)
    ax = workspace("roi_ax", max(K, 1) * W * pw * 4, dy.device)
    fp = workspace("roi_fp", max(K, 1) * 16, dy.device)
    fn = _L().cddmsl_roi_align_backward_pooled if pooled else _L().cddmsl_roi_align_backward
    check(fn(ptr(dy), ptr(rois), ptr(roi_start), ptr(dx), ptr(ay), ptr(ax), ptr(fp), N, C, H, W, K,
             ph, pw, spatial_scale, sampling_ratio, int(aligned), _dt(dy), stream_ptr()), "cddmsl_roi_align_backward")
    return dx


def roi_align_nchw(input, rois, output_size, spatial_scale, sampling_ratio, aligned):
    require_cuda(input, rois)
    assert rois.dim() == 2 and rois.size(1) == 5 and rois.dtype == torch.float32 and rois.is_contiguous() and input.is_contiguous()
    N, C, H, W = input.shape
    ph, pw = (output_size, output_size) if isinstance(output_size, int) else output_size
    K = rois.shape[0]
    out = torch.zeros((K, C, ph, pw), device=input.device, dtype=input.dtype)
    nbytes = ctypes.c_size_t(0)
    args = (N, C, H, W, K, ph, pw, spatial_scale, sampling_ratio, int(aligned), _dt(input))
    check(_L().cddmsl_roi_align_nchw_anyorder(ptr(input), ptr(rois), ptr(out), *args, None, ctypes.byref(nbytes), stream_ptr()), "cddmsl_roi_align_nchw_anyorder(size)")
    ws = workspace("roi_nchw", max(nbytes.value, 1), input.device)
    check(_L().cddmsl_roi_align_nchw_anyorder(ptr(input), ptr(rois), ptr(out), *args, ptr(ws), ctypes.byref(nbytes), stream_ptr()), "cddmsl_roi_align_nchw_anyorder")
    return out


# ... 610 lines not shown
```

### cddmsl_amd/layers.py

```python
import os
import weakref

import torch

from . import hip

_STEP = [0]


def bump_weight_version():
    _STEP[0] += 1


_LOAD_GEN = [0]


def note_weights_loaded(*_):
    _LOAD_GEN[0] += 1
    _STEP[0] += 1


def load_generation():
    return _LOAD_GEN[0]

# ... 579 lines not shown
class StackHalvesFn(torch.autograd.Function):

    @staticmethod
    def forward(ctx, a, b, full):
        n = a.shape[0]
        assert a.data_ptr() == full.data_ptr() and b.data_ptr() == full[n:].data_ptr() and full.shape[0] == 2 * n and a.shape == b.shape
        ctx.n = n
        return full.view(full.shape)

    @staticmethod
    def backward(ctx, g):
        return g[:ctx.n], g[ctx.n:], None


def stack_halves(a, b, full):
    return StackHalvesFn.apply(a, b, full)


def res_stage_attnpool(x, blocks, frozen, ap):
    fuse = not frozen and torch.is_grad_enabled()
    y = res_stage(x, blocks, frozen, out_grad_premasked=fuse)
    return AttnPoolFn.apply(y, None if ap.frozen else ap.q_w, ap, fuse)


def roi_downsample_on_map(K, out_size, N, H, W):
    if os.environ.get("CDDMSL_ROI_COMMUTE", "1") == "0":
        return False
    v = os.environ.get("CDDMSL_ROI_COMMUTE_DOWN", "")
    if v in ("0", "1"):
        return v == "1"
    return K * (out_size // 2) ** 2 > N * H * W


def _roi_block0_forward(feat, rois, bp, out_size, scale, sr, extra, next_pw=None, on_map=None):
    T = feat.dtype
    (s1, b1), (s2, b2), (s3, b3), bnd = bp.bn
    w1, _ = bp.pw[0].get(T, False)
    f8 = bp.fp8
    K, E = rois.shape[0], (0 if extra is None else extra.shape[0])
    N, H, W, _ = feat.shape
    z = hip.conv_fwd(feat, w1)
    o1_shape = (K + E, out_size, out_size, z.shape[-1])
    e8 = fp8_emit_for(bp.pw[1], o1_shape, 1, f8) if E == 0 else None
    o1 = hip.roi_align_forward_affine(z, rois, out_size, out_size, scale, sr, True, s1, b1, relu=True, extra_rows=E, emit8=e8)
    del z
    if on_map is None:
        on_map = roi_downsample_on_map(K, out_size, N, H, W)
    if on_map:
        wd, _ = bp.pw[3].get(T, False)
        zd = hip.conv_fwd(feat, wd)
        idn = hip.roi_align_forward_affine(zd, rois, out_size, out_size, scale, sr, True, bnd[0], bnd[1], pooled_only=True, extra_rows=E)
        del zd
        px = None
        if E:
            px = hip.avgpool2_fwd(extra)
            idn[K:].copy_(hip.conv_fwd(px, wd, bnd[0], bnd[1]))
    else:
        px = hip.roi_align_forward_affine(feat, rois, out_size, out_size, scale, sr, True, pooled_only=True, extra_rows=E)
        idn = None
    if E:
        o1[K:].copy_(hip.conv_fwd(extra, w1, s1, b1, relu=True))
        if idn is None:
            px[K:].copy_(hip.avgpool2_fwd(extra))
    o2 = conv_fwd_auto(o1, bp.pw[1], s2, b2, f8, relu=True, pad=1)
    p2 = hip.avgpool2_fwd(o2)
    if idn is None:
        idn = conv_fwd_auto(px, bp.pw[3], bnd[0], bnd[1], f8)
    out_shape = (p2.shape[0], p2.shape[1], p2.shape[2], _ohwi(bp.w[2]).shape[0])
    out = conv_fwd_auto(p2, bp.pw[2], s3, b3, f8, emit8=fp8_emit_for(next_pw, out_shape, 0, f8), residual=idn, relu=True)
    return o1, o2, p2, px, out, (_fp8_made_for(o1, bp.pw[1]) if f8 else None)


class RoIStageFn(torch.autograd.Function):

    @staticmethod
    def forward(ctx, feat, anchor, rois, roi_start, blocks, out_size, scale, sr, out_grad_premasked, extra):
        feat = feat.contiguous()
        nxt = lambda i: blocks[i + 1].pw[0] if i + 1 < len(blocks) else None
        on_map = roi_downsample_on_map(rois.shape[0], out_size, feat.shape[0], feat.shape[1], feat.shape[2])
        o1, o2, p2, px, cur, o1_8 = _roi_block0_forward(feat, rois, blocks[0], out_size, scale, sr, extra, nxt(0), on_map)
        saved, o1_8s = [feat, rois, roi_start, extra, o1, o2, p2, px, cur], [None, o1_8, None]
        for bi, bp in enumerate(blocks[1:], start=1):
            cur, mids = _block_forward(cur, bp, True, None, nxt(bi))
            saved += [mids[0], mids[1], mids[2], mids[3], cur]
            o1_8s += list(mids[4])
        ctx.blocks, ctx.meta = blocks, (out_size, scale, sr, out_grad_premasked, on_map)
        ctx.save_for_backward(*saved, *o1_8s)
        return cur

    @staticmethod
    def backward(ctx, g):
        blocks = ctx.blocks
        saved, o1_8s = ctx.saved_tensors[:-3 * len(blocks)], ctx.saved_tensors[-3 * len(blocks):]
        out_size, scale, sr, premasked, on_map = ctx.meta
        feat, rois, roi_start, extra = saved[:4]
        st = saved[4:]
        gs = g.contiguous() if premasked else hip.relu_bwd(g.contiguous(), st[-1])
        for i in range(len(blocks) - 1, 0, -1):
            o1, o2, p2, px = st[5 * i: 5 * i + 4]
            gs = _block_backward(gs, st[5 * i - 1], o1, o2, p2, px, blocks[i], True, mask_x=True, prev_bp=blocks[i - 1], c8=tuple(o1_8s[3 * i: 3 * i + 3]))
        bp = blocks[0]
        o1, o2, p2, px = st[0:4]
        T = o1.dtype
        (s1, _), (s2, _), (s3, _), bnd = bp.bn
        w1p, w2p, w3p, wdp = bp.w
        shp = lambda w: _ohwi(w).shape
        K, E = rois.shape[0], (0 if extra is None else extra.shape[0])
        f8 = bp.fp8 and T == torch.bfloat16
        gs_slot = fp8_slot_of(bp, "_fp8_gs") if f8 else None
        d2_slot = fp8_slot_of(bp.pw[1], "_fp8_g") if f8 else None
        hip.conv_wgrad(p2, gs, shp(w3p), s3, out=_ohwi(_grad_buf(w3p)))
        e8 = d2_slot.emit() if f8 and _fp8_dgrad_wanted(bp.pw[1], o2.shape, 1, f8) else None
        dpre2 = hip.avgpool2_bwd(dgrad_auto(gs, bp.pw[2], f8, gs_slot), tuple(o2.shape), mask=o2, emit8=e8)
        dpre1 = dgrad_auto(dpre2, bp.pw[1], f8, d2_slot, pad=1, relu_mask=o1)
        wgrad_auto(o1, dpre2, bp.pw[1], s2, 1, _ohwi(_grad_buf(w2p)), f8, o1_8s[1], d2_slot)
        N, H, W, C = feat.shape
        _, w1d = bp.pw[0].get(T, True)
        dfeat = dextra = dzd = wdd = None
        if on_map:
            _, wdd = bp.pw[3].get(T, True)
            dzd = hip.roi_align_backward(gs[:K], rois, roi_start, (N, H, W, gs.shape[-1]), scale, sr, True, pooled=True)
            hip.conv_wgrad(feat, dzd, shp(wdp), bnd[0], out=_ohwi(_grad_buf(wdp)))
            if E:
                hip.conv_wgrad(px, gs[K:], shp(wdp), bnd[0], out=_ohwi(_grad_buf(wdp)))
        else:
            hip.conv_wgrad(px, gs, shp(wdp), bnd[0], out=_ohwi(_grad_buf(wdp)))
            dxb = dgrad_auto(gs, bp.pw[3], f8, gs_slot)
        dz = hip.roi_align_backward(dpre1[:K], rois, roi_start, (N, H, W, dpre1.shape[-1]), scale, sr, True)
        hip.conv_wgrad(feat, dz, shp(w1p), s1, out=_ohwi(_grad_buf(w1p)))
        if E:
            hip.conv_wgrad(extra, dpre1[K:], shp(w1p), s1, out=_ohwi(_grad_buf(w1p)))
            if ctx.needs_input_grad[9]:
                dxe = hip.conv_fwd(gs[K:], wdd) if on_map else dxb[K:].contiguous()
                dextra = hip.conv_fwd(dpre1[K:], w1d, residual=hip.avgpool2_bwd(dxe, tuple(extra.shape)))
        if ctx.needs_input_grad[0]:
            r = hip.conv_fwd(dzd, wdd) if on_map else hip.roi_align_backward(dxb[:K], rois, roi_start, (N, H, W, C), scale, sr, True, pooled=True)
            dfeat = hip.conv_fwd(dz, w1d, residual=r)
        return dfeat, None, None, None, None, None, None, None, None, dextra


def roi_stage_supported(blocks):
    bp = blocks[0]
    return bp.stride == 2 and bp.w[3] is not None and tuple(bp.w[0].shape[2:]) == (1, 1) and tuple(bp.w[3].shape[2:]) == (1, 1)


def roi_stage(feat, rois, roi_start, blocks, frozen, out_size, scale, sr, extra=None, out_grad_premasked=False):
    assert rois.dim() == 2 and rois.size(1) == 5 and out_size % 2 == 0
    assert extra is None or tuple(extra.shape[1:]) == (out_size, out_size, feat.shape[3])
    if frozen or not torch.is_grad_enabled():
        nxt = lambda i: blocks[i + 1].pw[0] if i + 1 < len(blocks) else None
        cur = _roi_block0_forward(feat.contiguous(), rois, blocks[0], out_size, scale, sr, extra, nxt(0))[4]
        for bi, bp in enumerate(blocks[1:], start=1):
            cur, _ = _block_forward(cur, bp, False, None, nxt(bi))
        return cur
    return RoIStageFn.apply(feat, blocks[0].w[0], rois, roi_start, blocks, out_size, scale, sr, out_grad_premasked, extra)


def roi_stage_attnpool(feat, rois, roi_start, blocks, frozen, ap, out_size, scale, sr, extra=None):
    fuse = not frozen and torch.is_grad_enabled()
    y = roi_stage(feat, rois, roi_start, blocks, frozen, out_size, scale, sr, extra, out_grad_premasked=fuse)
    return AttnPoolFn.apply(y, None if ap.frozen else ap.q_w, ap, fuse)


class RoIAlignFn(torch.autograd.Function):
    @staticmethod
    def forward(ctx, x, rois, roi_start, out_size, scale, sampling_ratio, aligned, with_pooled=False, extra=None):
        K, E = rois.shape[0], (0 if extra is None else extra.shape[0])
# ... 419 lines not shown
```

### include/cddmsl_hip.h

```cpp
#ifndef CDDMSL_HIP_H
#define CDDMSL_HIP_H
#include <stddef.h>

#ifdef __cplusplus
extern "C" {
#endif

int cddmsl_abi_version(void);

int cddmsl_conv_fwd(const void* x, const void* w, void* y, const float* scale, const float* bias, const void* residual,
                    const void* relu_mask, int Nimg, int Hi, int Wi, int Cin, int Cout, int KH, int KW, int stride, int pad,
                    int pool, int ldy, int ldr, int ldm, int relu, int out_f32, int dtype, void* stream);
int cddmsl_bottleneck64_ok(int Nimg, int H, int W, int dtype);
int cddmsl_bottleneck64_fwd(const void* o1, const void* w2, const float* s2, const float* b2, const void* w3, const float* s3,
                            const float* b3, const void* residual, const void* x0, const void* wd, const float* sd,
                            const float* bd, const void* w1n, const float* s1n, const float* b1n, void* out, void* o1n,
                            int Nimg, int H, int W, int dtype, void* stream);
int cddmsl_set_workspace(void* ptr, long bytes);
int cddmsl_conv_wgrad(const void* x, const void* dy, float* dw, const float* scale, int Nimg, int Hi, int Wi, int Cin,
                      int Cout, int KH, int KW, int stride, int pad, int pool, int ldd, int dtype, void* stream);
int cddmsl_gemm_nt_batched(const void* a, const void* w, void* c, const float* bias, int M, int N, int K, int lda, int ldb, int ldc,
                           int batch, long sa, long sw, long sc, int out_f32, int dtype, void* stream);
int cddmsl_gemm_tn_batched(const void* a, const void* b, void* out, int M, int N, int K, int lda, int ldb, int ldo, int batch, long sa,
                           long sb, long so, int mode, int dtype, void* stream);
int cddmsl_last_kernel(void);
int cddmsl_plan_only(int on);
int cddmsl_weight_prep(const float* w, const float* scale, void* w_fwd, void* w_dgrad, int Cout, int KH, int KW, int Cin,
                       int dtype, void* stream);
int cddmsl_weight_prep_multi(const long long* table, int count, int dtype, void* stream);

int cddmsl_quantize_fp8(const void* x, void* y, const float* scale, float* amax, long numel, int src_dtype, void* stream);
int cddmsl_conv_fwd_fp8(const void* x, const void* w, void* y, const float* scale, const float* bias, const void* residual,
                        const void* relu_mask, int Nimg, int Hi, int Wi, int Cin, int Cout, int KH, int KW, int pad, int relu,
                        int out_f32, void* y8, const float* q8, float* amax8, void* stream);
int cddmsl_conv_fwd_q8(const void* x, const void* w, void* y, const float* scale, const float* bias, const void* residual,
                       const void* relu_mask, int Nimg, int Hi, int Wi, int Cin, int Cout, int KH, int KW, int stride, int pad,
                       int relu, void* y8, const float* q8, float* amax8, void* stream);
int cddmsl_fp8_dot_nt(const void* a, const void* b, float* c, const float* alpha, int R, int N, int K, int ldc, void* stream);
int cddmsl_conv_wgrad_fp8_ok(int Cin, int Cout, int KH, int KW, int pad, int ldd);
int cddmsl_conv_wgrad_fp8(const void* x8, const void* dy8, float* dw, const float* scale, int Nimg, int Hi, int Wi, int Cin, int Cout,
                          int KH, int KW, int pad, int ldd, void* stream);

int cddmsl_roi_align_forward(const void* x, const float* rois, void* y, void* y_pooled, int* dbg_grid, int N, int C, int H, int W,
                             int K, int ph, int pw, float spatial_scale, int sampling_ratio, int aligned, int dtype, void* stream);
int cddmsl_roi_align_backward(const void* dy, const float* rois, const int* roi_start, void* dx, float* ws_ay, float* ws_ax,
                              int* ws_fp, int N, int C, int H, int W, int K, int ph, int pw, float spatial_scale,
                              int sampling_ratio, int aligned, int dtype, void* stream);
int cddmsl_roi_align_forward_affine(const void* x, const float* rois, void* y, void* y_pooled, const float* scale,
                                    const float* bias, int relu, int N, int C, int H, int W, int K, int ph, int pw,
                                    float spatial_scale, int sampling_ratio, int aligned, int dtype, void* y8, const float* q8,
                                    float* amax8, void* stream);
int cddmsl_roi_align_backward_pooled(const void* dy, const float* rois, const int* roi_start, void* dx, float* ws_ay,
                                     float* ws_ax, int* ws_fp, int N, int C, int H, int W, int K, int ph, int pw,
                                     float spatial_scale, int sampling_ratio, int aligned, int dtype, void* stream);
int cddmsl_roi_align_nchw_anyorder(const void* input, const float* rois, void* output, int N, int C, int H, int W, int K, int ph, int pw,
                                   float spatial_scale, int sampling_ratio, int aligned, int dtype, void* temp, size_t* temp_bytes,
                                   void* stream);
int cddmsl_roi_align_backward_nchw_anyorder(const void* grad, const float* rois, void* grad_input, int N, int C, int H, int W, int K,
                                            int ph, int pw, float spatial_scale, int sampling_ratio, int aligned, int dtype, void* temp,
                                            size_t* temp_bytes, void* stream);

int cddmsl_anchors(const float* cell, float* out, int Hf, int Wf, int A, float stride, float offset, void* stream);
int cddmsl_sort_desc(const float* keys_in, float* keys_out, int* idx_scratch, int* order_out, const int* offsets, int N,
                     int total, void* temp, size_t* temp_bytes, void* stream);
int cddmsl_rpn_decode(const int* order, const float* deltas, const float* cell, const int* img_hw, float* boxes,
                      unsigned char* valid, int N, int Hf, int Wf, int A, int topk, float stride, float offset, float wx,
                      float wy, float ww, float wh, float scale_clamp, float min_size, void* stream);
int cddmsl_nms(const float* boxes, const unsigned char* valid, unsigned long long* mask_ws, int* keep, int* nkeep, int N,
               int n, float thr, int max_keep, void* stream);
int cddmsl_nms_anyorder(const float* boxes, const float* scores, long* keep, int* nkeep, int K, float iou_threshold, void* temp,
                        size_t* temp_bytes, void* stream);
int cddmsl_iou_match(const float* gt, int G, const float* preds, int P, long* matches, signed char* labels,
                     unsigned int* best_ws, int nthr, float t0, float t1, int l0, int l1, int l2, int allow_low_quality,
                     void* stream);

int cddmsl_iou_match_batched(const float* gt, const int* gt_off, const float* preds, const int* pred_off, long* matches,
                             signed char* labels, unsigned int* best_ws, int N, int P, int maxG, int totalG, int nthr, float t0,
                             float t1, int l0, int l1, int l2, int allow_low_quality, void* stream);

int cddmsl_attn_tokens_fwd(const void* x, const float* pos, void* tok, int K, int P, int TP, int C, int dtype, void* stream);
int cddmsl_attn_tokens_fwd_mask(const void* x, const float* pos, void* tok, unsigned long long* mbits, int K, int P, int TP, int C,
                                int dtype, void* stream);
int cddmsl_attnpool_dx(const void* pds, const void* zu, const float* g0, const unsigned long long* mbits, void* dx, float* gpos, int K,
                       int H2, int P, int TP, int C, int dtype, void* stream);
int cddmsl_attn_tokens_bwd(const void* dtok, const void* relu_mask, void* dx, float* gpos, int K, int P, int TP, int C, int dtype,
                           void* stream);
// ... 43 lines not shown
int cddmsl_l2norm_bwd(const float* dy, const float* y, const float* inv, float* dx, long R, int D, void* stream);
int cddmsl_cosine_logits_fwd(const float* x, const float* wn, float* scores, float* inv, long R, int D, int Kc,
                             float temperature, float eps, void* stream);
int cddmsl_cosine_logits_bwd(const float* ds, const float* x, const float* wn, const float* inv, float* dx, long R, int D,
                             int Kc, float temperature, int accumulate, void* stream);
int cddmsl_layernorm_fwd(const float* x, const float* gamma, const float* beta, void* y, float* mean, float* rstd, long R, int D,
                         float eps, int dtype, void* stream);
int cddmsl_layernorm_bwd(const void* dy, const float* x, const float* gamma, const float* mean, const float* rstd, float* dx,
                         long R, int D, int accumulate, int dtype, void* stream);
int cddmsl_focal_ce_fwd(const float* logits, const long* target, float* row_loss, float* probs, long R, int C, float gamma,
                        int bg_class, float bg_weight, void* stream);
int cddmsl_focal_ce_bwd(const float* logits, const long* target, const float* probs, const float* gscale, float* dlogits, long R,
                        int C, float gamma, int bg_class, float bg_weight, void* stream);
int cddmsl_contrastive_fwd(const float* S, float* rlse, float* clse, float* loss, int n, int ld, void* stream);
int cddmsl_contrastive_bwd(const float* S, const float* rlse, const float* clse, const float* gloss, float* dS, int n, int ld,
                           void* stream);
int cddmsl_rpn_losses(const float* logits, const float* deltas, const long* pos, int npos, const long* neg, int nneg, const long* midx,
                      const float* gt, const long* gt_off, const float* anchors, long A, float wx, float wy, float ww, float wh, float inv_norm,
                      float* out2, const float* gout2, float* dlogits, float* ddeltas, void* stream);
int cddmsl_box_l1(const float* deltas, int ld, const long* fg, int nfg, const long* cls, const float* src, const float* tgt, float wx, float wy,
                  float ww, float wh, float inv_norm, float* out1, const float* gout1, float* ddeltas, void* stream);

int cddmsl_preprocess(const unsigned char* img, void* out, int n, int h, int w, int Hp, int Wp, int Cp, const float* mean3,
                      const float* std3, int div255, int dtype, void* stream);
int cddmsl_preprocess224(const unsigned char* img, void* out, int n, int h, int w, int Hp, int Wp, int RH, int RW, int top,
                         int left, int S, int Cp, const float* mean3, const float* std3, int dtype, void* stream);
int cddmsl_preprocess_batch(const unsigned char* const* imgs, const int* hs, const int* ws, int N, void* out, int Hp, int Wp, int Cp,
                            const float* mean3, const float* std3, int div255, int dtype, void* stream);
int cddmsl_preprocess224_batch(const unsigned char* const* imgs, const int* hs, const int* ws, int N, void* out, int Hp, int Wp, int RH,
                               int RW, int top, int left, int S, int Cp, const float* mean3, const float* std3, int dtype, void* stream);
int cddmsl_avgpool2_fwd(const void* x, void* y, int N, int H, int W, int C, int dtype, void* stream);
int cddmsl_avgpool2_bwd(const void* dy, const void* mask, const void* add, void* dx, int N, int H, int W, int C, int dtype,
                        void* stream);
int cddmsl_avgpool2_bwd_q8(const void* dy, const void* mask, const void* add, void* dx, int N, int H, int W, int C, void* y8,
                           const float* q8, float* amax8, void* stream);
int cddmsl_maxpool3s2_fwd(const void* x, void* y, int N, int H, int W, int C, int dtype, void* stream);
int cddmsl_upsample_zero2(const void* t, const void* mask, const void* add, void* dx, int N, int H, int W, int C, int dtype,
                          void* stream);
int cddmsl_meanpool_fwd(const void* x, float* y, long K, int P, int C, int dtype, void* stream);
int cddmsl_meanpool_bwd(const float* dy, void* dx, long K, int P, int C, int dtype, void* stream);
int cddmsl_relu_bwd(const void* g, const void* y, void* dx, long numel, int g_f32, int dtype, void* stream);
int cddmsl_colsum(const void* x, float* out, long rows, int cols, int period, int dtype, void* stream);
int cddmsl_sgd_clip_step(float** params, const float** grads, float** moms, const long* sizes, int count, float* norm_ws,
                         float lr, float momentum, float wd, float clip, int first_step, void* stream);

int cddmsl_instance_boxes(const void* maps, int B, int H, int W, int dtype, int* records, int max_records, int* counts, void* ws,
                          size_t* ws_bytes, void* stream);

#ifdef __cplusplus
}
#endif
#endif
```

Baseline: 167.9.

## Add planar ROI-head layout path with dilated conv kernels and tap skipping

Introduces a 'planes' layout for the ROI head's first block, where pooled ROI features are stored position-major across all ROIs, so the 3x3 conv runs as a dilated conv over a wide plane instead of a batch of tiny images. The forward and wgrad kernels gain a dilation template path, and the forward path skips taps that are fully out of bounds for the whole tile. Matching avgpool, ROI-align forward/backward and wgrad plane kernels and the Python dispatch are added. The aim is to cut per-ROI tiling overhead and wasted padding work on small 7x7/14x14 maps. In exchange it adds extra permute copies and runs the fp8 paths in bf16 only when planes are used.

```diff
diff --git a/cddmsl_amd/csrc/conv_fwd256.hip b/cddmsl_amd/csrc/conv_fwd256.hip
--- a/cddmsl_amd/csrc/conv_fwd256.hip
+++ b/cddmsl_amd/csrc/conv_fwd256.hip
@@ -228,7 +228,7 @@
   }
 }
 
-template <typename T, bool TAPS, bool RPOOL = false, int EPI = -1, bool PERSIST = false, bool SPLITK = false>
+template <typename T, bool TAPS, bool RPOOL = false, int EPI = -1, bool PERSIST = false, bool SPLITK = false, bool DIL = false>
 __global__ __launch_bounds__(512) void k_conv_fwd256(ConvArgs p) {
   __shared__ __attribute__((aligned(16))) u32x4 lds[2 * 2 * 2 * 128 * KCH];
   const int t_in = threadIdx.x;
@@ -251,13 +251,14 @@
   const int tile_n = lbid % ntn, tile_m = lbid / ntn;
   const int m0 = tile_m * 256, n0 = tile_n * 256;
   const int cl = (t & 7) ^ ((t >> 4) & 7);
-  const int nkt = SPLITK ? min(p.kper, (p.Kc >> 3) - kt0) : (p.Kc >> 3);
+  int nkt = SPLITK ? min(p.kper, (p.Kc >> 3) - kt0) : (p.Kc >> 3);
   const int tpt = p.cpp >> 3;
+  const int dil = DIL ? p.dil : 1;
 
   auto rowoff = [&](int m, int& iy0, int& ix0) {
     const unsigned tq = fdiv((unsigned)m, p.dWo), ox = m - tq * p.Wo;
     const unsigned img = fdiv(tq, p.dHo), oy = tq - img * p.Ho;
-    iy0 = (int)oy * p.stride - p.pad; ix0 = (int)ox * p.stride - p.pad;
+    iy0 = (int)oy * p.stride - p.pad; ix0 = (int)ox * p.stride - p.pad * dil;
     return (((long)img * p.Hi + iy0) * p.Wi + ix0) * p.xrs * 16;
   };
   int iyb, ixb;
@@ -284,7 +285,7 @@
 #pragma unroll
       for (int h = 0; h < 2; ++h)
 #pragma unroll
-        for (int i = 0; i < 2; ++i) xm[h][i] |= ((unsigned)(ix0[h][i] + kx) >= (unsigned)p.Wi ? 1u : 0u) << kx;
+        for (int i = 0; i < 2; ++i) xm[h][i] |= ((unsigned)(ix0[h][i] + kx * dil) >= (unsigned)p.Wi ? 1u : 0u) << kx;
     const unsigned full = (1u << p.KW) - 1u;
     for (int ky = 0; ky < p.KH; ++ky)
 #pragma unroll
@@ -296,13 +297,42 @@
   const int step_row = ((p.Wi - (p.KW - 1)) * p.xrs - (p.cpp - KCH)) * 16;
   int left[2] = {tpt, tpt}, tap[2] = {0, 0}, kxs[2] = {0, 0};
   unsigned soa[2] = {0, 0}, sob[2] = {0, 0};
+  unsigned keep = (1u << (p.KH * p.KW)) - 1u;
+  int leftb[2] = {tpt, tpt}, tapb[2] = {0, 0};
+  auto tap_off = [&](int tp) {
+    const unsigned ky = fdiv((unsigned)tp, p.dKW), kx = (unsigned)tp - ky * p.KW;
+    return (unsigned)((ky * p.Wi + kx * dil) * p.xrs * 16);
+  };
+  auto next_tap = [&](int tp) {
+    const unsigned r = keep >> (tp + 1);
+    return tp + 1 + (r ? __builtin_ctz(r) : 0);
+  };
+  if (DIL && !SPLITK) {
+    unsigned inv = vinv[0][0] & vinv[0][1] & vinv[1][0] & vinv[1][1];
+#pragma unroll
+    for (int o = 32; o > 0; o >>= 1) inv &= (unsigned)__shfl_xor((int)inv, o);
+    unsigned* red = (unsigned*)lds;
+    if (lane == 0) red[wvu] = inv;
+    __syncthreads();
+    unsigned all = red[0];
+#pragma unroll
+    for (int w = 1; w < 8; ++w) all &= red[w];
+    __syncthreads();
+    keep &= ~(unsigned)__builtin_amdgcn_readfirstlane((int)all);
+    if (keep == 0) keep = 1u;
+    nkt = __builtin_popcount(keep) * tpt;
+    const int t0 = __builtin_ctz(keep);
+#pragma unroll
+    for (int h = 0; h < 2; ++h) { tap[h] = tapb[h] = t0; soa[h] = tap_off(t0); sob[h] = (unsigned)(t0 * p.cpp * 16); }
+  }
   if (SPLITK) {
     const int tap0 = TAPS ? kt0 / tpt : 0, within = TAPS ? kt0 - tap0 * tpt : kt0;
     const int ky0 = TAPS ? tap0 / p.KW : 0, kx0 = tap0 - ky0 * p.KW;
 #pragma unroll
     for (int h = 0; h < 2; ++h) {
       left[h] = tpt - (TAPS ? within : 0); tap[h] = tap0; kxs[h] = kx0;
-      soa[h] = (unsigned)((ky0 * p.Wi + kx0) * p.xrs * 16 + within * KCH * 16);
+      leftb[h] = left[h]; tapb[h] = tap0;
+      soa[h] = (unsigned)((ky0 * p.Wi + kx0 * dil) * p.xrs * 16 + within * KCH * 16);
       sob[h] = (unsigned)(kt0 * KCH * 16);
     }
   }
@@ -317,7 +347,10 @@
       if (TAPS) v |= __builtin_amdgcn_ubfe(vinv[h][i], (unsigned)tap[h], 1u) << 31;
       blds16(ra_rsrc, v, soa[h], dst + i * 8192);
     }
-    if (TAPS) {
+    if (DIL) {
+      soa[h] += KCH * 16;
+      if (--left[h] == 0) { left[h] = tpt; tap[h] = next_tap(tap[h]); soa[h] = tap_off(tap[h]); }
+    } else if (TAPS) {
       int step = KCH * 16;
       if (--left[h] == 0) {
         left[h] = tpt; ++tap[h];
@@ -332,6 +365,9 @@
 #pragma unroll
     for (int i = 0; i < 2; ++i) blds16(rb_rsrc, vb[j][i], sob[j], dst + i * 8192);
     sob[j] += KCH * 16;
+    if (DIL) {
+      if (--leftb[j] == 0) { leftb[j] = tpt; tapb[j] = next_tap(tapb[j]); sob[j] = (unsigned)(tapb[j] * p.cpp * 16); }
+    }
   };
   using I0 = std::integral_constant<int, 0>;
   using I1 = std::integral_constant<int, 1>;
@@ -711,7 +747,7 @@
   return {rem, (int)S, kper};
 }
 
-template <typename T, bool TAPS> void launch256_main(const ConvArgs& a, dim3 grid, hipStream_t st, int epi) {
+template <typename T, bool TAPS, bool DIL = false> void launch256_main(const ConvArgs& a, dim3 grid, hipStream_t st, int epi) {
   if constexpr (std::is_same<T, __bf16>::value && !TAPS) {
     const int nb = persistent_blocks();
     if (nb > 0 && grid.y == 1 && (int)grid.x > nb && (a.Kc >> 3) <= env_int("CDDMSL_PERSIST_MAXKT", 8)) {
@@ -719,12 +755,14 @@
       return;
     }
   }
-  with_epi(epi, [&](auto e) { hipLaunchKernelGGL((k_conv_fwd256<T, TAPS, false, decltype(e)::value>), grid, dim3(512), 0, st, a); });
-}
-
-template <typename T, bool TAPS> void launch256(const ConvArgs& a, dim3 grid, hipStream_t st, void* ws, long ws_bytes) {
+  with_epi(epi, [&](auto e) { hipLaunchKernelGGL((k_conv_fwd256<T, TAPS, false, decltype(e)::value, false, false, DIL>), grid, dim3(512), 0, st, a); });
+}
+
+template <typename T, bool TAPS, bool DIL = false> void launch256(const ConvArgs& a, dim3 grid, hipStream_t st, void* ws, long ws_bytes) {
   const int epi = epi_of(a);
-  if (sizeof(T) == 4 || epi < 0) { hipLaunchKernelGGL((k_conv_fwd256<T, TAPS, false, -1>), grid, dim3(512), 0, st, a); return; }
+  if constexpr (!DIL) {
+    if (sizeof(T) == 4 || epi < 0) { hipLaunchKernelGGL((k_conv_fwd256<T, TAPS, false, -1>), grid, dim3(512), 0, st, a); return; }
+  }
   if constexpr (sizeof(T) != 4) {
     if constexpr (std::is_same<T, __bf16>::value) {
       const int tiles = (int)grid.x;
@@ -732,14 +770,14 @@
       if (ts.splits) {
         ConvArgs m = a, t = a;
         m.tile_limit = tiles - ts.rem;
-        launch256_main<T, TAPS>(m, dim3((unsigned)(tiles - ts.rem), 1), st, epi);
+        launch256_main<T, TAPS, DIL>(m, dim3((unsigned)(tiles - ts.rem), 1), st, epi);
         t.partial = (float*)ws; t.tile0 = tiles - ts.rem; t.ksplits = ts.splits; t.kper = ts.kper;
-        hipLaunchKernelGGL((k_conv_fwd256<T, TAPS, false, -1, false, true>), dim3((unsigned)(ts.rem * ts.splits)), dim3(512), 0, st, t);
+        hipLaunchKernelGGL((k_conv_fwd256<T, TAPS, false, -1, false, true, DIL>), dim3((unsigned)(ts.rem * ts.splits)), dim3(512), 0, st, t);
         hipLaunchKernelGGL(k_conv_split_reduce, dim3((unsigned)(ts.rem * 64)), dim3(256), 0, st, t);
         return;
       }
     }
-    launch256_main<T, TAPS>(a, grid, st, epi);
+    launch256_main<T, TAPS, DIL>(a, grid, st, epi);
   }
 }
 
@@ -753,6 +791,9 @@
     if (taps) launch_fwd2<T, true>(a, grid, st);
     else launch_fwd2<T, false>(a, grid, st);
   } else {
+    if constexpr (std::is_same<T, __bf16>::value) {
+      if (a.dil != 1) { launch256<T, true, true>(a, grid, st, ws, ws_bytes); return; }
+    }
     if (a.res_pool) hipLaunchKernelGGL((k_conv_fwd256<T, false, true>), grid, dim3(512), 0, st, a);
     else if (taps) launch256<T, true>(a, grid, st, ws, ws_bytes);
     else launch256<T, false>(a, grid, st, ws, ws_bytes);
diff --git a/cddmsl_amd/csrc/conv_wgrad.hip b/cddmsl_amd/csrc/conv_wgrad.hip
--- a/cddmsl_amd/csrc/conv_wgrad.hip
+++ b/cddmsl_amd/csrc/conv_wgrad.hip
@@ -226,7 +226,7 @@
   for (int i = 0; i < 4; ++i) {
     m[i] = mt0 * WM + rb + 16 * i;
     pd[i] = p.dy + ((long)m[i] * p.ldd) * ES + (long)nc * 16;
-    px[i] = p.x + (((long)m[i] + (long)(ky - p.pad) * p.Wi + (kx - p.pad)) * p.xrs) * 16 + (long)coff * 16;
+    px[i] = p.x + (((long)m[i] + (long)(ky - p.pad) * p.Wi + (long)(kx - p.pad) * p.dil) * p.xrs) * 16 + (long)coff * 16;
   }
   const long dstep = (long)WM * p.ldd * ES, xstep = (long)WM * p.xrs * 16;
 
@@ -244,7 +244,7 @@
         unsigned tq = fdiv(mm, p.dWo);
         unsigned ox = mm - tq * p.Wo;
         unsigned oy = tq - fdiv(tq, p.dHo) * p.Ho;
-        ok = ok & ((unsigned)((int)oy - p.pad + ky) < (unsigned)p.Hi) & ((unsigned)((int)ox - p.pad + kx) < (unsigned)p.Wi);
+        ok = ok & ((unsigned)((int)oy - p.pad + ky) < (unsigned)p.Hi) & ((unsigned)((int)ox + (kx - p.pad) * p.dil) < (unsigned)p.Wi);
       }
       glds16(ok ? px[i] : zp, &lds[buf][1][(4 * wvu + 16 * i) * 16]);
     }
@@ -626,6 +626,7 @@
   }
 }
 
+template <bool DIL>
 __global__ __launch_bounds__(512) void k_wgrad256(WgradArgs p) {
   __shared__ __attribute__((aligned(16))) u32x4 lds[2 * 2 * 2 * 64 * 16];
   const int t = threadIdx.x, lane = t & 63;
@@ -645,6 +646,7 @@
   const int mt0 = bid * p.mtiles_per_split;
   const int nmt = min(p.mtiles_per_split, (p.M + WM - 1) / WM - mt0);
   const bool taps = !(p.KH == 1 && p.KW == 1);
+  const int dil = DIL ? p.dil : 1;
 
   const int rb = t >> 4, cl = (t & 15) ^ fsw(rb);
   const int gd = (cl >> 3) * 16 + (cl & 7);
@@ -656,10 +658,10 @@
 #pragma unroll
   for (int i = 0; i < 2; ++i) {
     vd[i] = (unsigned)((i * 32 + rb) * p.ldd * 2 + gd * 16);
-    vx[i] = (unsigned)((((i * 32 + rb) + ky * p.Wi + kx) * p.xrs + coff) * 16);
+    vx[i] = (unsigned)((((i * 32 + rb) + ky * p.Wi + kx * dil) * p.xrs + coff) * 16);
   }
   const __amdgpu_buffer_rsrc_t rd = __builtin_amdgcn_make_buffer_rsrc((void*)(p.dy + ((long)mt0 * WM * p.ldd + n0) * 2), 0, 0x80000000u, 0x00020000);
-  const __amdgpu_buffer_rsrc_t rx = __builtin_amdgcn_make_buffer_rsrc((void*)(p.x + ((long)mt0 * WM - p.pad * p.Wi - p.pad) * p.xrs * 16), 0, 0x80000000u, 0x00020000);
+  const __amdgpu_buffer_rsrc_t rx = __builtin_amdgcn_make_buffer_rsrc((void*)(p.x + ((long)mt0 * WM - p.pad * p.Wi - p.pad * dil) * p.xrs * 16), 0, 0x80000000u, 0x00020000);
   const unsigned dstep = (unsigned)(WM * p.ldd * 2), xstep = (unsigned)(WM * p.xrs * 16);
   const int mrow = mt0 * WM + rb;
 
@@ -685,10 +687,28 @@
         const unsigned tq = fdiv(mm, p.dWo);
         const unsigned ox = mm - tq * p.Wo;
         const unsigned oy = tq - fdiv(tq, p.dHo) * p.Ho;
-        ok = ok & ((unsigned)((int)oy - p.pad + ky) < (unsigned)p.Hi) & ((unsigned)((int)ox - p.pad + kx) < (unsigned)p.Wi);
+        ok = ok & ((unsigned)((int)oy - p.pad + ky) < (unsigned)p.Hi) & ((unsigned)((int)ox + (kx - p.pad) * dil) < (unsigned)p.Wi);
       }
       xinv[i] = ok ? 0u : 0x80000000u;
     }
+  };
+  const int btap = __builtin_amdgcn_readfirstlane((k0 >> 3) / p.cpp);
+  const int bky = btap / p.KW, bkx = btap - bky * p.KW;
+  auto next_tile = [&](int T) {
+    if (!DIL) return T;
+    while (T < nmt) {
+      const unsigned mlo = (unsigned)(mt0 + T) * WM, mhi = min(mlo + WM - 1, (unsigned)(p.M - 1));
+      const unsigned qlo = fdiv(mlo, p.dWo), qhi = fdiv(mhi, p.dWo);
+      if (qlo != qhi) break;
+      const int oxlo = (int)(mlo - qlo * p.Wo), oxhi = (int)(mhi - qlo * p.Wo);
+      const int oy = (int)(qlo - fdiv(qlo, p.dHo) * p.Ho), dxo = (bkx - p.pad) * dil;
+      unsigned mend;
+      if ((unsigned)(oy - p.pad + bky) >= (unsigned)p.Hi || (dxo > 0 && oxlo + dxo >= p.Wi)) mend = (qlo + 1) * p.Wo;
+      else if (dxo < 0 && oxhi + dxo < 0) mend = qlo * p.Wo + (unsigned)(-dxo);
+      else break;
+      T = max(T + 1, (int)(mend / WM) - mt0);
+    }
+    return T;
   };
   auto stageX = [&](auto J, int buf, int T) {
     constexpr int j = decltype(J)::value;
@@ -760,12 +780,13 @@
   __builtin_amdgcn_s_barrier();                                                     \
   __builtin_amdgcn_sched_barrier(0);
 
-  if (nmt > 0) {
-    validX(0);
-    stageD(I0{}, 0, 0); stageD(I1{}, 0, 0); stageX(I0{}, 0, 0); stageX(I1{}, 0, 0);
-    if (nmt > 1) {
-      validX(1);
-      stageD(I0{}, 1, 1); stageX(I0{}, 1, 1); stageX(I1{}, 1, 1);
+  int Tc = next_tile(0), T1 = next_tile(Tc + 1), T2 = next_tile(T1 + 1);
+  if (Tc < nmt) {
+    validX(Tc);
+    stageD(I0{}, 0, Tc); stageD(I1{}, 0, Tc); stageX(I0{}, 0, Tc); stageX(I1{}, 0, Tc);
+    if (T1 < nmt) {
+      validX(T1);
+      stageD(I0{}, 1, T1); stageX(I0{}, 1, T1); stageX(I1{}, 1, T1);
       asm volatile("s_waitcnt vmcnt(6)" ::: "memory");
     } else {
       asm volatile("s_waitcnt vmcnt(0)" ::: "memory");
@@ -780,24 +801,24 @@
     ts_loop = __builtin_amdgcn_s_memrealtime();
 #endif
 
-    for (int kt = 0; kt < nmt; ++kt) {
+    for (int kt = 0; Tc < nmt; ++kt, Tc = T1, T1 = T2, T2 = next_tile(T2 + 1)) {
       const int d = kt & 1;
-      const bool more1 = kt + 1 < nmt, more2 = kt + 2 < nmt;
+      const bool more1 = T1 < nmt, more2 = T2 < nmt;
       CDDMSL_READ_B(0, fb0)
-      if (more1) stageD(I1{}, d ^ 1, kt + 1);
+      if (more1) stageD(I1{}, d ^ 1, T1);
       CDDMSL_PHASE_SYNC_IN(CDDMSL_WAIT4(fb0))
       CDDMSL_MMA_QUAD(0, 0, fa0, fb0);
       CDDMSL_PHASE_SYNC_OUT(0, 0)
       CDDMSL_READ_B(1, fb1)
       CDDMSL_FLIP_B()
-      if (more2) { stageD(I0{}, d, kt + 2); validX(kt + 2); }
+      if (more2) { stageD(I0{}, d, T2); validX(T2); }
       CDDMSL_PHASE_SYNC_IN(CDDMSL_WAIT4(fb1))
       CDDMSL_MMA_QUAD(0, 1, fa0, fb1);
       CDDMSL_PHASE_SYNC_OUT(0, 1)
       CDDMSL_READ_A(1, fa1)
       CDDMSL_FLIP_A()
       if (more2) {
-        stageX(I0{}, d, kt + 2);
+        stageX(I0{}, d, T2);
         asm volatile("s_waitcnt vmcnt(4)" ::: "memory");
       } else {
         asm volatile("s_waitcnt vmcnt(0)" ::: "memory");
@@ -806,7 +827,7 @@
       CDDMSL_MMA_QUAD(1, 1, fa1, fb1);
       CDDMSL_PHASE_SYNC_OUT(1, 1)
       if (more1) { CDDMSL_READ_A(0, fa0) }
-      if (more2) stageX(I1{}, d, kt + 2);
+      if (more2) stageX(I1{}, d, T2);
       CDDMSL_PHASE_SYNC_IN(CDDMSL_WAIT8(fa0))
       CDDMSL_MMA_QUAD(1, 0, fa1, fb0);
       CDDMSL_PHASE_SYNC_OUT(1, 0)
@@ -1074,7 +1095,7 @@
 void launch_wgrad(WgradArgs& a, const Plan& p, Operand op, hipStream_t st, void* ws, long ws_bytes) {
   switch (p.kernel) {
     case 12: launch_wgrad_split<8, 32>(k_wgrad256_f8, a, p, st, ws, ws_bytes); break;
-    case 6: launch_wgrad_split<8, 32>(k_wgrad256, a, p, st, ws, ws_bytes); break;
+    case 6: launch_wgrad_split<8, 32>(a.dil != 1 ? k_wgrad256<true> : k_wgrad256<false>, a, p, st, ws, ws_bytes); break;
     case 5:
       if (op == OP_BF16) launch_wgrad_split<4, 16>(k_conv_wgrad_dma<__bf16>, a, p, st, ws, ws_bytes);
       else hipLaunchKernelGGL(k_conv_wgrad_dma<float>, dim3(p.gx), dim3(256), 0, st, a);
diff --git a/cddmsl_amd/csrc/elementwise.hip b/cddmsl_amd/csrc/elementwise.hip
--- a/cddmsl_amd/csrc/elementwise.hip
+++ b/cddmsl_amd/csrc/elementwise.hip
@@ -166,6 +166,46 @@
   }
 }
 
+template <typename T>
+__global__ void k_avgpool2_fwd_planes(const char* x, char* y, int N, int H, int W, int cch) {
+  int Ho = H / 2, Wo = W / 2;
+  long total = (long)N * Ho * Wo * cch;
+  const long px = (long)N * cch;
+  for (long i = (long)blockIdx.x * blockDim.x + threadIdx.x; i < total; i += (long)gridDim.x * blockDim.x) {
+    int c = i % cch; long q = i / cch;
+    int ox = q % Wo; q /= Wo;
+    int oy = q % Ho; int n = q / Ho;
+    const u32x4* b = (const u32x4*)x + ((long)(2 * oy) * W + 2 * ox) * px + (long)n * cch + c;
+    float a0[8], a1[8], a2[8], a3[8], o[8];
+    Elt<T>::unpack(b[0], a0); Elt<T>::unpack(b[px], a1);
+    Elt<T>::unpack(b[(long)W * px], a2); Elt<T>::unpack(b[(long)W * px + px], a3);
+#pragma unroll
+    for (int j = 0; j < Elt<T>::VEC; ++j) o[j] = ((a0[j] + a1[j]) + (a2[j] + a3[j])) * 0.25f;
+    ((u32x4*)y)[i] = Elt<T>::pack(o);
+  }
+}
+template <typename T>
+__global__ void k_avgpool2_bwd_planes(const char* dy, const char* mask, char* dx, int N, int H, int W, int cch) {
+  int Ho = H / 2, Wo = W / 2;
+  long total = (long)N * H * W * cch;
+  for (long i = (long)blockIdx.x * blockDim.x + threadIdx.x; i < total; i += (long)gridDim.x * blockDim.x) {
+    int c = i % cch; long q = i / cch;
+    int n = q % N; q /= N;
+    int xx = q % W; int yy = q / W;
+    float g[8], m[8], o[8];
+    bool in = (yy >> 1) < Ho && (xx >> 1) < Wo;
+    if (in) Elt<T>::unpack(((const u32x4*)dy)[(((long)n * Ho + (yy >> 1)) * Wo + (xx >> 1)) * cch + c], g);
+    if (mask) Elt<T>::unpack(((const u32x4*)mask)[i], m);
+#pragma unroll
+    for (int j = 0; j < Elt<T>::VEC; ++j) {
+      float v = in ? g[j] * 0.25f : 0.f;
+      if (mask && !(m[j] > 0.f)) v = 0.f;
+      o[j] = v;
+    }
+    ((u32x4*)dx)[i] = Elt<T>::pack(o);
+  }
+}
+
 __global__ __launch_bounds__(256) void k_avgpool2_bwd_q8(const char* dy, const char* mask, const char* add, char* dx, int N, int H, int W, int cch,
                                                          char* y8, const float* q8, unsigned* amax8) {
   using T = __bf16;
@@ -648,6 +688,27 @@
   return launch_status();
 }
 
+extern "C" int cddmsl_avgpool2_fwd_planes(const void* x, void* y, int N, int H, int W, int C, int dtype, void* stream) {
+  int es = dtype == 0 ? 2 : 4;
+  if ((C * es) % 16 || H < 2 || W < 2 || N < 0) return CDDMSL_ERR_ARG;
+  int cch = C * es / 16;
+  long total = (long)N * (H / 2) * (W / 2) * cch;
+  if (total == 0) return CDDMSL_OK;
+  DISPATCH(dtype, k_avgpool2_fwd_planes, <<<dim3(gsz(total)), dim3(256), 0, (hipStream_t)stream>>>((const char*)x, (char*)y, N, H, W, cch));
+  return launch_status();
+}
+
+extern "C" int cddmsl_avgpool2_bwd_planes(const void* dy, const void* mask, void* dx, int N, int H, int W, int C, int dtype, void* stream) {
+  int es = dtype == 0 ? 2 : 4;
+  if ((C * es) % 16 || H < 2 || W < 2 || N < 0) return CDDMSL_ERR_ARG;
+  int cch = C * es / 16;
+  long total = (long)N * H * W * cch;
+  if (total == 0) return CDDMSL_OK;
+  DISPATCH(dtype, k_avgpool2_bwd_planes, <<<dim3(gsz(total)), dim3(256), 0, (hipStream_t)stream>>>(
+      (const char*)dy, (const char*)mask, (char*)dx, N, H, W, cch));
+  return launch_status();
+}
+
 extern "C" int cddmsl_avgpool2_bwd_q8(const void* dy, const void* mask, const void* add, void* dx, int N, int H, int W, int C, void* y8,
                                       const float* q8, float* amax8, void* stream) {
   if ((C * 2) % 16 || !y8 || !q8 || !amax8) return CDDMSL_ERR_ARG;
diff --git a/cddmsl_amd/csrc/gemm_common.h b/cddmsl_amd/csrc/gemm_common.h
--- a/cddmsl_amd/csrc/gemm_common.h
+++ b/cddmsl_amd/csrc/gemm_common.h
@@ -54,6 +54,7 @@
   float* partial = nullptr;
   int tile0 = 0, ksplits = 1, kper = 0, tile_limit = 0;
   int nt_out = 1;
+  int dil = 1;
 #ifdef CDDMSL_TILE_STAMPS
   unsigned long long* tstamps = nullptr;
 #endif
@@ -128,6 +129,7 @@
   const float* g0 = nullptr;
   const unsigned long long* mbits = nullptr;
   float* gpos = nullptr;
+  int dil = 1;
   float* ws = nullptr;
 #ifdef CDDMSL_TILE_STAMPS
   unsigned long long* tstamps = nullptr;
diff --git a/cddmsl_amd/csrc/gemm_conv.hip b/cddmsl_amd/csrc/gemm_conv.hip
--- a/cddmsl_amd/csrc/gemm_conv.hip
+++ b/cddmsl_amd/csrc/gemm_conv.hip
@@ -217,8 +217,8 @@
   if (mode == 2) return true;
   return (long)(a.Cout / 256) * (a.K / 256) * batch * ((a.M + WM - 1) / WM) >= env_int("CDDMSL_WGRAD256_MIN", 4000);
 }
-static bool wgrad256_span_ok(int mtiles_per_split, int Wi, long row_bytes) {
-  return ((long)mtiles_per_split * WM + WM + 2L * Wi + 2) * row_bytes + (1L << 20) < (1L << 31);
+static bool wgrad256_span_ok(int mtiles_per_split, int Wi, int dil, long row_bytes) {
+  return ((long)mtiles_per_split * WM + WM + 2L * Wi + 2L * dil) * row_bytes + (1L << 20) < (1L << 31);
 }
 
 static int even_split(int total_mt, long* splits) {
@@ -272,7 +272,7 @@
   if (op == OP_FP8) {
     long sp = split_256_rounds(tiles256, total_mt);
     const int mps = even_split(total_mt, &sp);
-    if (!wgrad256_span_ok(mps, a.Wi, row_bytes)) return {};
+    if (!wgrad256_span_ok(mps, a.Wi, 1, row_bytes)) return {};
     return {12, (unsigned)(tiles256 * sp), 1, (int)sp, mps};
   }
   const int cols = 256 / es;
@@ -289,7 +289,7 @@
     if (sp > maxs) sp = maxs;
     if (sp < 1) sp = 1;
     const int mps256 = even_split(total_mt, &sp);
-    if (wgrad256_span_ok(mps256, a.Wi, row_bytes)) return {6, (unsigned)(tiles256 * sp), 1, (int)sp, mps256};
+    if (wgrad256_span_ok(mps256, a.Wi, a.dil, row_bytes)) return {6, (unsigned)(tiles256 * sp), 1, (int)sp, mps256};
   }
   return {same ? 5 : 4, (unsigned)(tiles * splits), 1, (int)splits, mps};
 }
@@ -343,6 +343,46 @@
   return run_wgrad(a, (Operand)dtype, plan_wgrad(a, (Operand)dtype, 1), stream);
 }
 
+static int fill_conv_planes(ConvArgs& a, const void* x, const void* w, void* y, const float* scale, const float* bias, const void* residual,
+                            const void* relu_mask, int ph, int pw, int Kr, int Cin, int Cout, int KH, int KW, int pad, int relu) {
+  if (ph <= 0 || pw <= 0 || Kr <= 0 || KH != KW || 2 * pad != KH - 1 || (long)pw * Kr > 0x7fffffffL) return CDDMSL_ERR_ARG;
+  const int st = fill_conv(a, OP_BF16, x, w, y, scale, bias, residual, relu_mask, 1, ph, pw * Kr, Cin, Cout, KH, KW, 1, pad, 0, Cout, Cout, Cout,
+                           relu, 0, nullptr, nullptr, nullptr);
+  if (st != CDDMSL_OK) return st;
+  a.dil = Kr;
+  if (env_int("CDDMSL_GEMM256", 1) == 0 || !gemm256_legal(a)) return CDDMSL_ERR_ARG;
+  if ((((long)(KH - 1) * a.Wi + (long)(KW - 1) * Kr + 256) * a.xrs + a.cpp) * 16 >= (1L << 31)) return CDDMSL_ERR_ARG;
+  return CDDMSL_OK;
+}
+static Plan plan_fwd_planes(const ConvArgs& a) { return {3, (unsigned)((a.Cout / 256) * ((a.M + 255) / 256)), 1}; }
+
+extern "C" int cddmsl_conv_planes_ok(int ph, int pw, int Kr, int Cin, int Cout, int KH, int KW, int pad) {
+  ConvArgs a;
+  if (Cin <= 0 || Cin % 8 != 0) return 0;
+  return fill_conv_planes(a, nullptr, nullptr, nullptr, nullptr, nullptr, nullptr, nullptr, ph, pw, Kr, Cin, Cout, KH, KW, pad, 0) == CDDMSL_OK ? 1 : 0;
+}
+
+extern "C" int cddmsl_conv_fwd_planes(const void* x, const void* w, void* y, const float* scale, const float* bias, const void* residual,
+                                      const void* relu_mask, int ph, int pw, int Kr, int Cin, int Cout, int KH, int KW, int pad, int relu,
+                                      void* stream) {
+  ConvArgs a;
+  const int st = fill_conv_planes(a, x, w, y, scale, bias, residual, relu_mask, ph, pw, Kr, Cin, Cout, KH, KW, pad, relu);
+  if (st != CDDMSL_OK) return st;
+  return run_fwd(a, OP_BF16, plan_fwd_planes(a), stream);
+}
+
+extern "C" int cddmsl_conv_wgrad_planes(const void* x, const void* dy, float* dw, const float* scale, int ph, int pw, int Kr, int Cin,
+                                        int Cout, int KH, int KW, int pad, void* stream) {
+  if (ph <= 0 || pw <= 0 || Kr <= 0 || KH != KW || 2 * pad != KH - 1 || (long)pw * Kr > 0x7fffffffL) return CDDMSL_ERR_ARG;
+  WgradArgs a;
+  const int st = fill_wgrad(a, OP_BF16, x, dy, dw, scale, 1, ph, pw * Kr, Cin, Cout, KH, KW, 1, pad, 0, Cout);
+  if (st != CDDMSL_OK || a.M == 0) return st;
+  a.dil = Kr;
+  const Plan p = plan_wgrad(a, OP_BF16, 1);
+  if (p.kernel != 5 && p.kernel != 6) return CDDMSL_ERR_ARG;
+  return run_wgrad(a, OP_BF16, p, stream);
+}
+
 extern "C" int cddmsl_conv_wgrad_fp8_ok(int Cin, int Cout, int KH, int KW, int pad, int ldd) {
   return (Cin % 256 == 0 && Cout % 256 == 0 && KH == KW && (KH & 1) && 2 * pad == KH - 1 && ldd % 16 == 0) ? 1 : 0;
 }
diff --git a/cddmsl_amd/csrc/roi_align.hip b/cddmsl_amd/csrc/roi_align.hip
--- a/cddmsl_amd/csrc/roi_align.hip
+++ b/cddmsl_amd/csrc/roi_align.hip
@@ -206,7 +206,8 @@
 constexpr int ROW_MAXY = 32;
 template <int RP>
 __global__ __launch_bounds__(256) void k_roi_align_fwd_rows(const char* x, const float* rois, char* y, int N, int H, int W, int cch, int ph, int pw,
-                                                            float scale, int sampling_ratio, int aligned, const float* esc, const float* ebi, int relu) {
+                                                            float scale, int sampling_ratio, int aligned, const float* esc, const float* ebi, int relu,
+                                                            long sk, long si, long sj) {
   const int nrb = ph / RP;
   const int i0 = (blockIdx.x % nrb) * RP, k = blockIdx.x / nrb;
   const RoiGeom g = roi_geom(rois + 5 * (long)k, scale, ph, pw, sampling_ratio, aligned);
@@ -255,7 +256,7 @@
         o[q] = acc[q] * inv;
         if (esc) { o[q] = __builtin_fmaf(o[q], sq[q], bq[q]); if (relu) o[q] = fmaxf(o[q], 0.f); }
       }
-      ((u32x4*)y)[(((long)k * nrb + i0 / RP) * opw + jo) * cch + c] = Vec<__bf16>::pack(o);
+      ((u32x4*)y)[(long)k * sk + (long)(i0 / RP) * si + (long)jo * sj + c] = Vec<__bf16>::pack(o);
     }
     return;
   }
@@ -354,12 +355,12 @@
     if (ahead) issue(min(cur + 2, W - 1));
   }
   const int spo = RP * g.gw;
-  u32x4* yo = (u32x4*)y + ((long)k * nrb + i0 / RP) * opw * cch + c;
+  u32x4* yo = (u32x4*)y + (long)k * sk + (long)(i0 / RP) * si + c;
   if (nx == 0) {
     float o[8];
 #pragma unroll
     for (int q = 0; q < 8; ++q) { o[q] = 0.f; if (esc) { o[q] = bq[q]; if (relu) o[q] = fmaxf(o[q], 0.f); } }
-    for (int jo = 0; jo < opw; ++jo) yo[(long)jo * cch] = Vec<__bf16>::pack(o);
+    for (int jo = 0; jo < opw; ++jo) yo[(long)jo * sj] = Vec<__bf16>::pack(o);
     return;
   }
   int left = spo, j = 0;
@@ -393,7 +394,7 @@
           for (int q = 0; q < 8; ++q) o[q] = fmaxf(o[q], 0.f);
         }
       }
-      __builtin_nontemporal_store(Vec<__bf16>::pack(o), &yo[(long)j * cch]);
+      __builtin_nontemporal_store(Vec<__bf16>::pack(o), &yo[(long)j * sj]);
       ++j; left = spo;
     }
   }
@@ -448,7 +449,7 @@
 constexpr int MAXP = 16;
 template <typename T, int NC, int TS>
 __global__ __launch_bounds__(256) void k_roi_align_bwd(const char* dy, const float* ay, const float* ax, const int* fp, const int* roi_start,
-                                char* dx, int H, int W, int cch, int ph, int pw) {
+                                char* dx, int H, int W, int cch, int ph, int pw, long sk, long si, long sj) {
   const int tiles_x = (W + TS - 1) / TS, tiles_y = (H + TS - 1) / TS;
   const long tile = blockIdx.x;
   const int tx = tile % tiles_x, ty = (tile / tiles_x) % tiles_y, n = tile / ((long)tiles_x * tiles_y);
@@ -500,7 +501,7 @@
         float wxj[TS];
 #pragma unroll
         for (int a = 0; a < TS; ++a) wxj[a] = __builtin_bit_cast(float, __builtin_amdgcn_readlane(__builtin_bit_cast(int, wxv[a]), j));
-        const u32x4* src = (const u32x4*)dy + (((long)k * ph + i) * pw + j) * cch;
+        const u32x4* src = (const u32x4*)dy + ((long)k * sk + (long)i * si + (long)j * sj);
         float v[NC][8];
 #pragma unroll
         for (int u = 0; u < NC; ++u) {
@@ -540,7 +541,7 @@
 static int roi_align_forward_impl(const void* x, const float* rois, void* y, void* y_pooled, int* dbg_grid, const float* esc,
                                   const float* ebi, int relu, int N, int C, int H, int W, int K, int ph, int pw, float spatial_scale,
                                   int sampling_ratio, int aligned, int dtype, void* stream, void* y8 = nullptr, const float* q8 = nullptr,
-                                  float* amax8 = nullptr) {
+                                  float* amax8 = nullptr, int Kr = 0) {
   int es = dtype == 0 ? 2 : 4;
   if ((dtype != 0 && dtype != 1) || (C * es) % 16 || H <= 0 || W <= 0 || ph <= 0 || pw <= 0 || K < 0 || N < 0)
     return CDDMSL_ERR_ARG;
@@ -549,6 +550,7 @@
   if (K == 0) return CDDMSL_OK;
   if (!y && !y_pooled) return CDDMSL_ERR_ARG;
   if (y8 && (dtype != 0 || !y)) return CDDMSL_ERR_ARG;
+  if (Kr && (Kr < K || !y || y_pooled)) return CDDMSL_ERR_ARG;
   int cch = C * es / 16;
   if (y_pooled && ((ph & 1) || (pw & 1))) return CDDMSL_ERR_ARG;
   long grid = (long)K * (y_pooled ? ph / 2 : ph);
@@ -560,10 +562,13 @@
   if (dtype == 0 && !y8 && !dbg_grid && ((y != nullptr) != (y_pooled != nullptr)) && cch <= 256 && !rows_off) {
     const int rthreads = 64;
     const unsigned gy = (unsigned)((cch + rthreads - 1) / rthreads);
-    if (y) k_roi_align_fwd_rows<1><<<dim3((unsigned)((long)K * ph), gy), dim3(rthreads), 0, st>>>((const char*)x, rois, (char*)y, N, H, W, cch, ph, pw, spatial_scale, sampling_ratio, aligned, esc, ebi, relu);
-    else k_roi_align_fwd_rows<2><<<dim3((unsigned)((long)K * (ph / 2)), gy), dim3(rthreads), 0, st>>>((const char*)x, rois, (char*)y_pooled, N, H, W, cch, ph, pw, spatial_scale, sampling_ratio, aligned, esc, ebi, relu);
+    const long rs = (long)(y ? pw : pw / 2) * cch;
+    if (Kr) k_roi_align_fwd_rows<1><<<dim3((unsigned)((long)K * ph), gy), dim3(rthreads), 0, st>>>((const char*)x, rois, (char*)y, N, H, W, cch, ph, pw, spatial_scale, sampling_ratio, aligned, esc, ebi, relu, (long)cch, rs * Kr, (long)Kr * cch);
+    else if (y) k_roi_align_fwd_rows<1><<<dim3((unsigned)((long)K * ph), gy), dim3(rthreads), 0, st>>>((const char*)x, rois, (char*)y, N, H, W, cch, ph, pw, spatial_scale, sampling_ratio, aligned, esc, ebi, relu, rs * ph, rs, (long)cch);
+    else k_roi_align_fwd_rows<2><<<dim3((unsigned)((long)K * (ph / 2)), gy), dim3(rthreads), 0, st>>>((const char*)x, rois, (char*)y_pooled, N, H, W, cch, ph, pw, spatial_scale, sampling_ratio, aligned, esc, ebi, relu, rs * (ph / 2), rs, (long)cch);
     return launch_status();
   }
+  if (Kr) return CDDMSL_ERR_ARG;
 #define CDDMSL_RAF(TT, RPP) k_roi_align_fwd<TT, RPP><<<dim3((unsigned)grid), dim3(threads), 0, st>>>((const char*)x, rois, (char*)y, (char*)y_pooled, dbg_grid, N, H, W, cch, ph, pw, spatial_scale, sampling_ratio, aligned, esc, ebi, relu, (char*)y8, q8, (unsigned*)amax8)
   if (dtype == 0) { if (y_pooled) CDDMSL_RAF(__bf16, 2); else CDDMSL_RAF(__bf16, 1); }
   else { if (y_pooled) CDDMSL_RAF(float, 2); else CDDMSL_RAF(float, 1); }
@@ -587,10 +592,19 @@
                                 sampling_ratio, aligned, dtype, stream, y8, q8, amax8);
 }
 
+extern "C" int cddmsl_roi_align_forward_affine_planes(const void* x, const float* rois, void* y, const float* scale, const float* bias,
+                                                      int relu, int N, int C, int H, int W, int K, int ph, int pw, int Kr,
+                                                      float spatial_scale, int sampling_ratio, int aligned, void* stream) {
+  if (Kr <= 0 || !y) return CDDMSL_ERR_ARG;
+  return roi_align_forward_impl(x, rois, y, nullptr, nullptr, scale, bias, relu, N, C, H, W, K, ph, pw, spatial_scale, sampling_ratio,
+                                aligned, 0, stream, nullptr, nullptr, nullptr, Kr);
+}
+
 static int roi_align_backward_impl(const void* dy, const float* rois, const int* roi_start, void* dx, float* ws_ay,
                                    float* ws_ax, int* ws_fp, int N, int C, int H, int W, int K, int ph, int pw,
-                                   float spatial_scale, int sampling_ratio, int aligned, int dtype, int fold, void* stream) {
+                                   float spatial_scale, int sampling_ratio, int aligned, int dtype, int fold, void* stream, int Kr = 0) {
   int es = dtype == 0 ? 2 : 4;
+  if (Kr && Kr < K) return CDDMSL_ERR_ARG;
   if ((dtype != 0 && dtype != 1) || (C * es) % 16 || H <= 0 || W <= 0 || ph <= 0 || pw <= 0 || K < 0 || N < 0)
     return CDDMSL_ERR_ARG;
   if (ph > MAXP || pw > MAXP || ph > 64 || pw > 64) return CDDMSL_ERR_ARG;
@@ -604,7 +618,8 @@
   const int ts = 2;
   long grid = (long)N * ((H + ts - 1) / ts) * ((W + ts - 1) / ts);
   if (grid > 0x7fffffffL) return CDDMSL_ERR_ARG;
-#define CDDMSL_RAB(TT, NCC, TSS) k_roi_align_bwd<TT, NCC, TSS><<<dim3((unsigned)grid), dim3(threads), 0, st>>>((const char*)dy, ws_ay, ws_ax, ws_fp, roi_start, (char*)dx, H, W, cch, ph, pw)
+  const long sk = Kr ? cch : (long)ph * pw * cch, si = Kr ? (long)pw * Kr * cch : (long)pw * cch, sj = Kr ? (long)Kr * cch : cch;
+#define CDDMSL_RAB(TT, NCC, TSS) k_roi_align_bwd<TT, NCC, TSS><<<dim3((unsigned)grid), dim3(threads), 0, st>>>((const char*)dy, ws_ay, ws_ax, ws_fp, roi_start, (char*)dx, H, W, cch, ph, pw, sk, si, sj)
   if (dtype == 0) { if (ncpt <= 1) CDDMSL_RAB(__bf16, 1, 2); else if (ncpt == 2) CDDMSL_RAB(__bf16, 2, 2); else CDDMSL_RAB(__bf16, 4, 2); }
   else { if (ncpt <= 1) CDDMSL_RAB(float, 1, 2); else if (ncpt == 2) CDDMSL_RAB(float, 2, 2); else CDDMSL_RAB(float, 4, 2); }
 #undef CDDMSL_RAB
@@ -616,6 +631,14 @@
                                          float spatial_scale, int sampling_ratio, int aligned, int dtype, void* stream) {
   return roi_align_backward_impl(dy, rois, roi_start, dx, ws_ay, ws_ax, ws_fp, N, C, H, W, K, ph, pw, spatial_scale,
                                  sampling_ratio, aligned, dtype, 1, stream);
+}
+
+extern "C" int cddmsl_roi_align_backward_planes(const void* dy, const float* rois, const int* roi_start, void* dx, float* ws_ay,
+                                                float* ws_ax, int* ws_fp, int N, int C, int H, int W, int K, int ph, int pw, int Kr,
+                                                float spatial_scale, int sampling_ratio, int aligned, int dtype, void* stream) {
+  if (Kr <= 0) return CDDMSL_ERR_ARG;
+  return roi_align_backward_impl(dy, rois, roi_start, dx, ws_ay, ws_ax, ws_fp, N, C, H, W, K, ph, pw, spatial_scale,
+                                 sampling_ratio, aligned, dtype, 1, stream, Kr);
 }
 
 extern "C" int cddmsl_roi_align_backward_pooled(const void* dy, const float* rois, const int* roi_start, void* dx, float* ws_ay,
diff --git a/cddmsl_amd/hip.py b/cddmsl_amd/hip.py
--- a/cddmsl_amd/hip.py
+++ b/cddmsl_amd/hip.py
@@ -98,6 +98,13 @@
         L.cddmsl_lm_head_topk.argtypes = [vp] * 7 + [c_long] + [ci] * 4 + [vp]
         L.cddmsl_beam_step.argtypes = [vp] * 15 + [ci] * 5 + [vp]
         L.cddmsl_decode_attn_beam.argtypes = [vp] * 7 + [ci] * 9 + [cf, ci, vp]
+        L.cddmsl_conv_planes_ok.argtypes = [ci] * 8
+        L.cddmsl_conv_fwd_planes.argtypes = [vp] * 7 + [ci] * 9 + [vp]
+        L.cddmsl_conv_wgrad_planes.argtypes = [vp] * 4 + [ci] * 8 + [vp]
+        L.cddmsl_roi_align_forward_affine_planes.argtypes = [vp] * 5 + [ci] * 9 + [cf, ci, ci, vp]
+        L.cddmsl_roi_align_backward_planes.argtypes = [vp] * 7 + [ci] * 8 + [cf, ci, ci, ci, vp]
+        L.cddmsl_avgpool2_fwd_planes.argtypes = [vp, vp] + [ci] * 5 + [vp]
+        L.cddmsl_avgpool2_bwd_planes.argtypes = [vp] * 3 + [ci] * 5 + [vp]
         _sigs_done = True
     return L
 
@@ -260,6 +267,55 @@
     return y
 
 
+def conv_planes_ok(ph, pw, Kr, Cin, Cout, KH, KW, pad):
+    return bool(_L().cddmsl_conv_planes_ok(ph, pw, Kr, Cin, Cout, KH, KW, pad))
+
+
+def conv_fwd_planes(x, w, scale=None, bias=None, residual=None, relu=False, relu_mask=None, pad=0):
+    require_cuda(x, w, scale, bias, residual, relu_mask)
+    ensure_workspace(x.device)
+    assert x.dim() == 4 and w.dim() == 4 and x.is_contiguous() and w.is_contiguous() and x.dtype == w.dtype == torch.bfloat16
+    ph, pw, Kr, Cin = x.shape
+    Cout, KH, KW, Cin2 = w.shape
+    assert Cin == Cin2, (x.shape, w.shape)
+    y = torch.empty((ph, pw, Kr, Cout), device=x.device, dtype=x.dtype)
+    for v in (scale, bias):
+        assert v is None or (v.dtype == torch.float32 and v.numel() == Cout and v.is_contiguous())
+    for v in (residual, relu_mask):
+        assert v is None or (v.dtype == x.dtype and v.is_contiguous() and tuple(v.shape) == tuple(y.shape))
+    name = _CONV_KERNEL[3]
+    e0 = PROFILE.begin(name)
+    check(_L().cddmsl_conv_fwd_planes(ptr(x), ptr(w), ptr(y), ptr(scale), ptr(bias), ptr(residual), ptr(relu_mask), ph, pw, Kr, Cin, Cout,
+                                      KH, KW, pad, int(relu), stream_ptr()), "cddmsl_conv_fwd_planes")
+    M = ph * pw * Kr
+    PROFILE.end(e0, name, 2.0 * M * Cout * KH * KW * Cin, (M, Cout, KH * KW * Cin, KH, 0, 1),
+                nbytes=float(x.numel() * 2 + w.numel() * 2 + y.numel() * 2 + (residual.numel() * 2 if residual is not None else 0)
+                             + (relu_mask.numel() * 2 if relu_mask is not None else 0)))
+    return y
+
+
+def conv_wgrad_planes(x, dy, w_shape, scale=None, pad=0, out=None):
+    require_cuda(x, dy, scale, out)
+    Cout, KH, KW, Cin = w_shape
+    ph, pw, Kr, Cin2 = x.shape
+    assert Cin == Cin2 and x.dtype == dy.dtype == torch.bfloat16 and x.is_contiguous() and dy.is_contiguous()
+    assert tuple(dy.shape) == (ph, pw, Kr, Cout)
+    if out is None:
+        out = torch.zeros(w_shape, device=x.device, dtype=torch.float32)
+    assert out.dtype == torch.float32 and out.is_contiguous() and tuple(out.shape) == tuple(w_shape)
+    ensure_workspace(x.device)
+
+    def launch():
+        return _L().cddmsl_conv_wgrad_planes(ptr(x), ptr(dy), ptr(out), ptr(scale), ph, pw, Kr, Cin, Cout, KH, KW, pad, stream_ptr())
+    e0 = PROFILE.begin(plan=launch) if PROFILE.on else None
+    check(launch(), "cddmsl_conv_wgrad_planes")
+    M = ph * pw * Kr
+    PROFILE.end(e0, _CONV_KERNEL.get(_L().cddmsl_last_kernel(), "conv_wgrad") if e0 is not None else "conv_wgrad",
+                2.0 * M * Cout * KH * KW * Cin, (M, Cout, KH * KW * Cin, KH, 0, 1),
+                nbytes=float(x.numel() * 2 + dy.numel() * 2 + out.numel() * 4))
+    return out
+
+
 def bottleneck64_ok(o1, w2, w3, wd=None, w1n=None):
     if not (o1.is_cuda and o1.dtype == torch.bfloat16 and o1.dim() == 4 and o1.is_contiguous() and o1.shape[3] == 64):
         return False
@@ -510,6 +566,27 @@
     return y
 
 
+@_timed("avgpool2_fwd")
+def avgpool2_fwd_planes(x):
+    require_cuda(x)
+    H, W, N, C = x.shape
+    assert x.is_contiguous()
+    y = torch.empty((N, H // 2, W // 2, C), device=x.device, dtype=x.dtype)
+    check(_L().cddmsl_avgpool2_fwd_planes(ptr(x), ptr(y), N, H, W, C, _dt(x), stream_ptr()), "cddmsl_avgpool2_fwd_planes")
+    return y
+
+
+@_timed("avgpool2_bwd")
+def avgpool2_bwd_planes(dy, in_shape, mask=None):
+    require_cuda(dy, mask)
+    H, W, N, C = in_shape
+    assert dy.is_contiguous() and tuple(dy.shape) == (N, H // 2, W // 2, C)
+    assert mask is None or (mask.is_contiguous() and tuple(mask.shape) == tuple(in_shape) and mask.dtype == dy.dtype)
+    dx = torch.empty(in_shape, device=dy.device, dtype=dy.dtype)
+    check(_L().cddmsl_avgpool2_bwd_planes(ptr(dy), ptr(mask), ptr(dx), N, H, W, C, _dt(dy), stream_ptr()), "cddmsl_avgpool2_bwd_planes")
+    return dx
+
+
 @_timed("avgpool2_bwd")
 def avgpool2_bwd(dy, in_shape, mask=None, add=None, emit8=None):
     require_cuda(dy, mask, add)
@@ -746,6 +823,37 @@
     if y8 is not None:
         y._fp8 = (y8, emit8[0].data_ptr())
     return yp if pooled_only else y
+
+
+@_timed("roi_align_forward")
+def roi_align_forward_affine_planes(x, rois, ph, pw, spatial_scale, sampling_ratio, aligned, scale=None, bias=None, relu=False, extra_rows=0):
+    require_cuda(x, rois)
+    assert rois.dim() == 2 and rois.size(1) == 5 and rois.dtype == torch.float32 and rois.is_contiguous()
+    assert (scale is None) == (bias is None) and x.dtype == torch.bfloat16
+    N, H, W, C = x.shape
+    K = rois.shape[0]
+    y = torch.empty((ph, pw, K + extra_rows, C), device=x.device, dtype=x.dtype)
+    assert scale is None or (scale.dtype == torch.float32 and scale.numel() == C and bias.numel() == C and scale.is_contiguous() and bias.is_contiguous())
+    check(_L().cddmsl_roi_align_forward_affine_planes(ptr(x), ptr(rois), ptr(y), ptr(scale), ptr(bias), int(relu), N, C, H, W, K, ph, pw,
+                                                       K + extra_rows, spatial_scale, sampling_ratio, int(aligned), stream_ptr()),
+          "cddmsl_roi_align_forward_affine_planes")
+    return y
+
+
+@_timed("roi_align_backward")
+def roi_align_backward_planes(dy, K, rois, roi_start, in_shape, spatial_scale, sampling_ratio, aligned):
+    require_cuda(dy, rois, roi_start)
+    N, H, W, C = in_shape
+    ph, pw, Kr, _ = dy.shape
+    assert roi_start.dtype == torch.int32 and roi_start.numel() == N + 1 and dy.is_contiguous() and K == rois.shape[0] and Kr >= K
+    dx = torch.empty(in_shape, device=dy.device, dtype=dy.dtype)
+    ay = workspace("roi_ay", max(K, 1) * H * ph * 4, dy.device)
+    ax = workspace("roi_ax", max(K, 1) * W * pw * 4, dy.device)
+    fp = workspace("roi_fp", max(K, 1) * 16, dy.device)
+    check(_L().cddmsl_roi_align_backward_planes(ptr(dy), ptr(rois), ptr(roi_start), ptr(dx), ptr(ay), ptr(ax), ptr(fp), N, C, H, W, K,
+                                                 ph, pw, Kr, spatial_scale, sampling_ratio, int(aligned), _dt(dy), stream_ptr()),
+          "cddmsl_roi_align_backward_planes")
+    return dx
 
 
 @_timed("roi_align_backward")
diff --git a/cddmsl_amd/layers.py b/cddmsl_amd/layers.py
--- a/cddmsl_amd/layers.py
+++ b/cddmsl_amd/layers.py
@@ -635,7 +635,14 @@
     return K * (out_size // 2) ** 2 > N * H * W
 
 
-def _roi_block0_forward(feat, rois, bp, out_size, scale, sr, extra, next_pw=None, on_map=None):
+def roi_planes_wanted(Kr, out_size, bp, dtype):
+    if os.environ.get("CDDMSL_ROI_PLANES", "") != "1" or dtype != torch.bfloat16 or bp.fp8 or bp.stride != 2:
+        return False
+    Cout, KH, KW, Cin = _ohwi(bp.w[1]).shape
+    return (KH, KW) == (3, 3) and hip.conv_planes_ok(out_size, out_size, Kr, Cin, Cout, KH, KW, 1)
+
+
+def _roi_block0_forward(feat, rois, bp, out_size, scale, sr, extra, next_pw=None, on_map=None, planes=None):
     T = feat.dtype
     (s1, b1), (s2, b2), (s3, b3), bnd = bp.bn
     w1, _ = bp.pw[0].get(T, False)
@@ -644,8 +651,13 @@
     N, H, W, _ = feat.shape
     z = hip.conv_fwd(feat, w1)
     o1_shape = (K + E, out_size, out_size, z.shape[-1])
-    e8 = fp8_emit_for(bp.pw[1], o1_shape, 1, f8) if E == 0 else None
-    o1 = hip.roi_align_forward_affine(z, rois, out_size, out_size, scale, sr, True, s1, b1, relu=True, extra_rows=E, emit8=e8)
+    if planes is None:
+        planes = roi_planes_wanted(K + E, out_size, bp, T)
+    if planes:
+        o1 = hip.roi_align_forward_affine_planes(z, rois, out_size, out_size, scale, sr, True, s1, b1, relu=True, extra_rows=E)
+    else:
+        e8 = fp8_emit_for(bp.pw[1], o1_shape, 1, f8) if E == 0 else None
+        o1 = hip.roi_align_forward_affine(z, rois, out_size, out_size, scale, sr, True, s1, b1, relu=True, extra_rows=E, emit8=e8)
     del z
     if on_map is None:
         on_map = roi_downsample_on_map(K, out_size, N, H, W)
@@ -662,11 +674,15 @@
         px = hip.roi_align_forward_affine(feat, rois, out_size, out_size, scale, sr, True, pooled_only=True, extra_rows=E)
         idn = None
     if E:
-        o1[K:].copy_(hip.conv_fwd(extra, w1, s1, b1, relu=True))
+        (o1[:, :, K:].permute(2, 0, 1, 3) if planes else o1[K:]).copy_(hip.conv_fwd(extra, w1, s1, b1, relu=True))
         if idn is None:
             px[K:].copy_(hip.avgpool2_fwd(extra))
-    o2 = conv_fwd_auto(o1, bp.pw[1], s2, b2, f8, relu=True, pad=1)
-    p2 = hip.avgpool2_fwd(o2)
+    if planes:
+        o2 = hip.conv_fwd_planes(o1, bp.pw[1].get(T, False)[0], s2, b2, relu=True, pad=1)
+        p2 = hip.avgpool2_fwd_planes(o2)
+    else:
+        o2 = conv_fwd_auto(o1, bp.pw[1], s2, b2, f8, relu=True, pad=1)
+        p2 = hip.avgpool2_fwd(o2)
     if idn is None:
         idn = conv_fwd_auto(px, bp.pw[3], bnd[0], bnd[1], f8)
     out_shape = (p2.shape[0], p2.shape[1], p2.shape[2], _ohwi(bp.w[2]).shape[0])
@@ -681,13 +697,14 @@
         feat = feat.contiguous()
         nxt = lambda i: blocks[i + 1].pw[0] if i + 1 < len(blocks) else None
         on_map = roi_downsample_on_map(rois.shape[0], out_size, feat.shape[0], feat.shape[1], feat.shape[2])
-        o1, o2, p2, px, cur, o1_8 = _roi_block0_forward(feat, rois, blocks[0], out_size, scale, sr, extra, nxt(0), on_map)
+        planes = roi_planes_wanted(rois.shape[0] + (0 if extra is None else extra.shape[0]), out_size, blocks[0], feat.dtype)
+        o1, o2, p2, px, cur, o1_8 = _roi_block0_forward(feat, rois, blocks[0], out_size, scale, sr, extra, nxt(0), on_map, planes)
         saved, o1_8s = [feat, rois, roi_start, extra, o1, o2, p2, px, cur], [None, o1_8, None]
         for bi, bp in enumerate(blocks[1:], start=1):
             cur, mids = _block_forward(cur, bp, True, None, nxt(bi))
             saved += [mids[0], mids[1], mids[2], mids[3], cur]
             o1_8s += list(mids[4])
-        ctx.blocks, ctx.meta = blocks, (out_size, scale, sr, out_grad_premasked, on_map)
+        ctx.blocks, ctx.meta = blocks, (out_size, scale, sr, out_grad_premasked, on_map, planes)
         ctx.save_for_backward(*saved, *o1_8s)
         return cur
 
@@ -695,7 +712,7 @@
     def backward(ctx, g):
         blocks = ctx.blocks
         saved, o1_8s = ctx.saved_tensors[:-3 * len(blocks)], ctx.saved_tensors[-3 * len(blocks):]
-        out_size, scale, sr, premasked, on_map = ctx.meta
+        out_size, scale, sr, premasked, on_map, planes = ctx.meta
         feat, rois, roi_start, extra = saved[:4]
         st = saved[4:]
         gs = g.contiguous() if premasked else hip.relu_bwd(g.contiguous(), st[-1])
@@ -714,9 +731,16 @@
         d2_slot = fp8_slot_of(bp.pw[1], "_fp8_g") if f8 else None
         hip.conv_wgrad(p2, gs, shp(w3p), s3, out=_ohwi(_grad_buf(w3p)))
         e8 = d2_slot.emit() if f8 and _fp8_dgrad_wanted(bp.pw[1], o2.shape, 1, f8) else None
-        dpre2 = hip.avgpool2_bwd(dgrad_auto(gs, bp.pw[2], f8, gs_slot), tuple(o2.shape), mask=o2, emit8=e8)
-        dpre1 = dgrad_auto(dpre2, bp.pw[1], f8, d2_slot, pad=1, relu_mask=o1)
-        wgrad_auto(o1, dpre2, bp.pw[1], s2, 1, _ohwi(_grad_buf(w2p)), f8, o1_8s[1], d2_slot)
+        if planes:
+            dpre2 = hip.avgpool2_bwd_planes(dgrad_auto(gs, bp.pw[2]), tuple(o2.shape), mask=o2)
+            dpre1 = hip.conv_fwd_planes(dpre2, bp.pw[1].get(T, True)[1], relu_mask=o1, pad=1)
+            hip.conv_wgrad_planes(o1, dpre2, shp(w2p), s2, pad=1, out=_ohwi(_grad_buf(w2p)))
+            dpre1_extra = dpre1[:, :, K:].permute(2, 0, 1, 3).contiguous() if E else None
+        else:
+            dpre2 = hip.avgpool2_bwd(dgrad_auto(gs, bp.pw[2], f8, gs_slot), tuple(o2.shape), mask=o2, emit8=e8)
+            dpre1 = dgrad_auto(dpre2, bp.pw[1], f8, d2_slot, pad=1, relu_mask=o1)
+            wgrad_auto(o1, dpre2, bp.pw[1], s2, 1, _ohwi(_grad_buf(w2p)), f8, o1_8s[1], d2_slot)
+            dpre1_extra = dpre1[K:] if E else None
         N, H, W, C = feat.shape
         _, w1d = bp.pw[0].get(T, True)
         dfeat = dextra = dzd = wdd = None
@@ -729,13 +753,16 @@
         else:
             hip.conv_wgrad(px, gs, shp(wdp), bnd[0], out=_ohwi(_grad_buf(wdp)))
             dxb = dgrad_auto(gs, bp.pw[3], f8, gs_slot)
-        dz = hip.roi_align_backward(dpre1[:K], rois, roi_start, (N, H, W, dpre1.shape[-1]), scale, sr, True)
+        if planes:
+            dz = hip.roi_align_backward_planes(dpre1, K, rois, roi_start, (N, H, W, dpre1.shape[-1]), scale, sr, True)
+        else:
+            dz = hip.roi_align_backward(dpre1[:K], rois, roi_start, (N, H, W, dpre1.shape[-1]), scale, sr, True)
         hip.conv_wgrad(feat, dz, shp(w1p), s1, out=_ohwi(_grad_buf(w1p)))
         if E:
-            hip.conv_wgrad(extra, dpre1[K:], shp(w1p), s1, out=_ohwi(_grad_buf(w1p)))
+            hip.conv_wgrad(extra, dpre1_extra, shp(w1p), s1, out=_ohwi(_grad_buf(w1p)))
             if ctx.needs_input_grad[9]:
                 dxe = hip.conv_fwd(gs[K:], wdd) if on_map else dxb[K:].contiguous()
-                dextra = hip.conv_fwd(dpre1[K:], w1d, residual=hip.avgpool2_bwd(dxe, tuple(extra.shape)))
+                dextra = hip.conv_fwd(dpre1_extra, w1d, residual=hip.avgpool2_bwd(dxe, tuple(extra.shape)))
         if ctx.needs_input_grad[0]:
             r = hip.conv_fwd(dzd, wdd) if on_map else hip.roi_align_backward(dxb[:K], rois, roi_start, (N, H, W, C), scale, sr, True, pooled=True)
             dfeat = hip.conv_fwd(dz, w1d, residual=r)
diff --git a/include/cddmsl_hip.h b/include/cddmsl_hip.h
--- a/include/cddmsl_hip.h
+++ b/include/cddmsl_hip.h
@@ -38,6 +38,12 @@
                        int relu, void* y8, const float* q8, float* amax8, void* stream);
 int cddmsl_fp8_dot_nt(const void* a, const void* b, float* c, const float* alpha, int R, int N, int K, int ldc, void* stream);
 int cddmsl_conv_wgrad_fp8_ok(int Cin, int Cout, int KH, int KW, int pad, int ldd);
+int cddmsl_conv_planes_ok(int ph, int pw, int Kr, int Cin, int Cout, int KH, int KW, int pad);
+int cddmsl_conv_fwd_planes(const void* x, const void* w, void* y, const float* scale, const float* bias, const void* residual,
+                           const void* relu_mask, int ph, int pw, int Kr, int Cin, int Cout, int KH, int KW, int pad, int relu,
+                           void* stream);
+int cddmsl_conv_wgrad_planes(const void* x, const void* dy, float* dw, const float* scale, int ph, int pw, int Kr, int Cin, int Cout,
+                             int KH, int KW, int pad, void* stream);
 int cddmsl_conv_wgrad_fp8(const void* x8, const void* dy8, float* dw, const float* scale, int Nimg, int Hi, int Wi, int Cin, int Cout,
                           int KH, int KW, int pad, int ldd, void* stream);
 
@@ -52,6 +58,12 @@
                                     float* amax8, void* stream);
 int cddmsl_roi_align_backward_pooled(const void* dy, const float* rois, const int* roi_start, void* dx, float* ws_ay,
                                      float* ws_ax, int* ws_fp, int N, int C, int H, int W, int K, int ph, int pw,
+                                     float spatial_scale, int sampling_ratio, int aligned, int dtype, void* stream);
+int cddmsl_roi_align_forward_affine_planes(const void* x, const float* rois, void* y, const float* scale, const float* bias,
+                                           int relu, int N, int C, int H, int W, int K, int ph, int pw, int Kr,
+                                           float spatial_scale, int sampling_ratio, int aligned, void* stream);
+int cddmsl_roi_align_backward_planes(const void* dy, const float* rois, const int* roi_start, void* dx, float* ws_ay,
+                                     float* ws_ax, int* ws_fp, int N, int C, int H, int W, int K, int ph, int pw, int Kr,
                                      float spatial_scale, int sampling_ratio, int aligned, int dtype, void* stream);
 int cddmsl_roi_align_nchw_anyorder(const void* input, const float* rois, void* output, int N, int C, int H, int W, int K, int ph, int pw,
                                    float spatial_scale, int sampling_ratio, int aligned, int dtype, void* temp, size_t* temp_bytes,
@@ -161,6 +173,8 @@
 int cddmsl_avgpool2_fwd(const void* x, void* y, int N, int H, int W, int C, int dtype, void* stream);
 int cddmsl_avgpool2_bwd(const void* dy, const void* mask, const void* add, void* dx, int N, int H, int W, int C, int dtype,
                         void* stream);
+int cddmsl_avgpool2_fwd_planes(const void* x, void* y, int N, int H, int W, int C, int dtype, void* stream);
+int cddmsl_avgpool2_bwd_planes(const void* dy, const void* mask, void* dx, int N, int H, int W, int C, int dtype, void* stream);
 int cddmsl_avgpool2_bwd_q8(const void* dy, const void* mask, const void* add, void* dx, int N, int H, int W, int C, void* y8,
                            const float* q8, float* amax8, void* stream);
 int cddmsl_maxpool3s2_fwd(const void* x, void* y, int N, int H, int W, int C, int dtype, void* stream);
```

Result: slower. 165.7 (-1.3%).
